# pnnl/ERT-Conditional-Diffusion-Model

Measured on AMD Instinct MI355X. Metric: denoising-steps/sec (64×64, batch 64) at 1/2/4/8 GPUs; conv HBM GB/s vs roofline, higher is better.
Workload: dtype f32

## Files before the change

ert-conditional-diffusion-model_amd/csrc/unet.h:

```cpp
#pragma once
#include <cstdlib>

#include "ertd_common.h"

#ifdef ERTD_DIAG
#define ERTD_KNOB(name, dflt) (::ertd::unet::diag_knob("ERTD_" name, (dflt)))
#else
#define ERTD_KNOB(name, dflt) (dflt)
#endif

namespace ertd {
namespace unet {

#ifdef ERTD_DIAG
inline int diag_knob(const char* name, int dflt) {
  const char* e = getenv(name);
  return e ? atoi(e) : dflt;
}
#endif

constexpr int NTHR = 256;
constexpr double GN_EPS = 1e-5;

enum Act { ACT_NONE = 0, ACT_GN_SILU = 1, ACT_GN = 2 };
enum Mode { MODE_S1 = 0, MODE_S2 = 1, MODE_UP = 2,
            MODE_UPP = 3 };

struct GnPartArgs {
  const float2* pa; int npa; int Ca;
  const float2* pb; int npb; int Cb;
  int HW, groups;
  const float* gamma; const float* beta;
  float2* out;
  float2* mr;
};

struct GnFold {
  GnPartArgs g;
  unsigned* cnt;
  int target;
  int B;
};

struct ConvArgs {
  const float* srcA;
  const float* srcB;
  int Ca, Cb;
  const float2* gn;
  const float* wpk;
  const float* bias;
  const float* ebias;
  int eb_stride;
  const float* res;
  float* out;
  int Cin, Cout;
  int Hs, Ws;
  int Ho, Wo;
  void* bimg;
  int bimg_ready;
  const float* wpk_wino;
  float* ksplit_buf;
  const float* wpk_wino4;
  float2* gnp;
  int split;
  GnFold fold;
  unsigned* zero_words;
  int zero_n;
  GnPartArgs gnc;
};

hipError_t launch_gn_finalize(const GnPartArgs& a, int B, hipStream_t s);
hipError_t launch_gn_partials(const float* x, int C, int HW, int np, float2* out, int B, hipStream_t s);
struct WinoRoute {
  enum Kernel { NONE,
                F2,
                F4,
                F4S,
                F4S_UP
  } kernel = NONE;
  int ksplit = 1;
  size_t kbuf_floats = 0;
  int items = 0, grid = 0;
  int gn_parts = 0;
  bool fold_ok = false;
  int fold_target = 0;
  int pack_kind = ERTD_PACK_DIRECT;
};
WinoRoute wino_route(int mode, int act, int Cin, int Ca, int Cout, int Wo, int B, bool have_f2_pack,
                     bool have_f4_pack, int cus);
bool wino_gnc_ok(const WinoRoute& r, int Cin, int Wo, const GnPartArgs& g);
int conv_gn_parts(int ks, int mode, int act, const ConvArgs& a, const WinoRoute& r);
int conv_bf16_gn_parts(int ks, int mode, int act, const ConvArgs& a, int B);

__device__ __forceinline__ float row16_sum(float v) {
  v += __int_as_float(__builtin_amdgcn_update_dpp(0, __float_as_int(v), 0xB1, 0xF, 0xF, false));
  v += __int_as_float(__builtin_amdgcn_update_dpp(0, __float_as_int(v), 0x4E, 0xF, 0xF, false));
  v += __int_as_float(__builtin_amdgcn_update_dpp(0, __float_as_int(v), 0x141, 0xF, 0xF, false));
  v += __int_as_float(__builtin_amdgcn_update_dpp(0, __float_as_int(v), 0x140, 0xF, 0xF, false));
  return v;
}

__device__ __forceinline__ void st_f2_wt(float2* p, float2 v) {
  unsigned* u = reinterpret_cast<unsigned*>(p);
  __hip_atomic_store(u, __float_as_uint(v.x), __ATOMIC_RELAXED, __HIP_MEMORY_SCOPE_AGENT);
  __hip_atomic_store(u + 1, __float_as_uint(v.y), __ATOMIC_RELAXED, __HIP_MEMORY_SCOPE_AGENT);
}
__device__ __forceinline__ float2 ld_f2_wt(const float2* p) {
  const unsigned* u = reinterpret_cast<const unsigned*>(p);
  return make_float2(__uint_as_float(__hip_atomic_load(u, __ATOMIC_RELAXED, __HIP_MEMORY_SCOPE_AGENT)),
                     __uint_as_float(__hip_atomic_load(u + 1, __ATOMIC_RELAXED, __HIP_MEMORY_SCOPE_AGENT)));
}
#ifndef FOLD_BATCH
#define FOLD_BATCH 4
#endif
constexpr int GN_LPG = 16;
struct GnGroupGeom {
  int c0, itemsA, items;
  const float2* pa;
  const float2* pb;
};
__device__ __forceinline__ GnGroupGeom gn_group_geom(const GnPartArgs& g, int b, int gi, bool live) {
  const int cpg = (g.Ca + g.Cb) / g.groups;
  GnGroupGeom q{};
  if (!live) return q;
  q.c0 = gi * cpg;
  const int nA = q.c0 < g.Ca ? (g.Ca - q.c0 < cpg ? g.Ca - q.c0 : cpg) : 0;
  q.itemsA = nA * g.npa;
  q.items = q.itemsA + (cpg - nA) * (g.Cb > 0 ? g.npb : 0);
  q.pa = g.pa + ((size_t)b * g.Ca + q.c0) * g.npa;
  q.pb = g.Cb > 0 ? g.pb + ((size_t)b * g.Cb + (q.c0 + nA - g.Ca)) * g.npb : nullptr;
  return q;
}
template <int CTRL>
__device__ __forceinline__ double dpp_f64(double v) {
  const unsigned long long u = __double_as_longlong(v);
  const int lo = __builtin_amdgcn_update_dpp(0, (int)(unsigned)u, CTRL, 0xF, 0xF, false);
  const int hi = __builtin_amdgcn_update_dpp(0, (int)(unsigned)(u >> 32), CTRL, 0xF, 0xF, false);
  return __longlong_as_double((long long)(((unsigned long long)(unsigned)hi << 32) | (unsigned)lo));
}
__device__ __forceinline__ double gn_lpg_sum(double v) {
  static_assert(GN_LPG == 16, "one DPP row per group");
  v += dpp_f64<0xB1>(v);
  v += dpp_f64<0x4E>(v);
  v += dpp_f64<0x141>(v);
  v += dpp_f64<0x140>(v);
  return v;
}
__device__ __forceinline__ double gn_part_q(float2 v, double n, double inv_n, double mean) {
  const double d = (double)v.x * inv_n - mean;
  return (double)v.y + n * (d * d);
}
__device__ __forceinline__ float2 gn_mean_rstd(double mean, double Q, double N) {
  double var = Q / N;
  var = var > 0.0 ? var : 0.0;
  return make_float2((float)mean, (float)(1.0 / sqrt(var + GN_EPS)));
}
template <bool WT>
__device__ __forceinline__ float2 gn_ld_part(const GnGroupGeom& q, int k) {
  return k < q.itemsA ? (WT ? ld_f2_wt(q.pa + k) : q.pa[k]) : q.pb[k - q.itemsA];
}
template <bool WT>
__device__ __forceinline__ void gn_group_finalize(const GnPartArgs& g, int b, int lane, int part,
                                                  int nparts, float2* orow = nullptr) {
  const int G = g.groups, C = g.Ca + g.Cb, cpg = C / G;
  const int gper = (G + nparts - 1) / nparts, gfirst = part * gper;
  const int gcnt = G - gfirst < gper ? G - gfirst : gper;
  if (gcnt <= 0) return;
  constexpr int LPG = GN_LPG;
  const double na = (double)(g.HW / g.npa), nb = g.Cb > 0 ? (double)(g.HW / g.npb) : 1.0;
  const double ina = 1.0 / na, inb = 1.0 / nb;
  const double N = (double)cpg * (double)g.HW;
  for (int gbase = 0; gbase < gcnt; gbase += 64 / LPG) {
    const int gl = gbase + lane / LPG, sub = lane % LPG;
    const bool live = gl < gcnt;
    const int gi = gfirst + gl;
    const GnGroupGeom q = gn_group_geom(g, b, gi, live);
    double S = 0.0;
    for (int k0 = sub; k0 < q.items; k0 += FOLD_BATCH * LPG) {
      float2 v[FOLD_BATCH];
#pragma unroll
      for (int j = 0; j < FOLD_BATCH; ++j) {
        const int k = k0 + j * LPG;
        v[j] = k < q.items ? gn_ld_part<WT>(q, k) : make_float2(0.f, 0.f);
      }
#pragma unroll
      for (int j = 0; j < FOLD_BATCH; ++j)
        if (k0 + j * LPG < q.items) S += (double)v[j].x;
    }
    S = gn_lpg_sum(S);
    const double mean = S / N;
    double Q = 0.0;
    for (int k0 = sub; k0 < q.items; k0 += FOLD_BATCH * LPG) {
      float2 v[FOLD_BATCH];
#pragma unroll
      for (int j = 0; j < FOLD_BATCH; ++j) {
        const int k = k0 + j * LPG;
        v[j] = k < q.items ? gn_ld_part<WT>(q, k) : make_float2(0.f, 0.f);
      }
#pragma unroll
      for (int j = 0; j < FOLD_BATCH; ++j) {
        const int k = k0 + j * LPG;
        if (k < q.items) Q += k < q.itemsA ? gn_part_q(v[j], na, ina, mean) : gn_part_q(v[j], nb, inb, mean);
      }
    }
    Q = gn_lpg_sum(Q);
    if (!live) continue;
    const float2 mr = gn_mean_rstd(mean, Q, N);
    if (g.mr && sub == 0) g.mr[(size_t)b * G + gi] = mr;
    for (int cl = sub; cl < cpg; cl += LPG) {
      const int c = q.c0 + cl;
      const float scale = mr.y * g.gamma[c];
      const float shift = -scale * mr.x + g.beta[c];
      if (orow) orow[c] = make_float2(scale, shift);
      else g.out[(size_t)b * C + c] = make_float2(scale, shift);
    }
  }
}
template <int JM, int KM>
__device__ __forceinline__ void gn_group_finalize_regs(const GnPartArgs& g, const int (&smp)[JM],
                                                       const int (&jg)[JM], const int (&row)[JM],
                                                       const bool (&jl)[JM], int lane, float2* tab) {
  constexpr int LPG = GN_LPG;
  const int G = g.groups, C = g.Ca + g.Cb, cpg = C / G, sub = lane % LPG;
  const double na = (double)(g.HW / g.npa), nb = g.Cb > 0 ? (double)(g.HW / g.npb) : 1.0;
  const double ina = 1.0 / na, inb = 1.0 / nb;
  const double N = (double)cpg * (double)g.HW;
  GnGroupGeom q[JM];
  float2 v[JM][KM];
  float ga[JM], be[JM];
  bool live[JM];
#pragma unroll
  for (int j = 0; j < JM; ++j) {
    const int gi = jg[j] * 4 + lane / LPG;
    live[j] = jl[j] && gi < G;
    q[j] = gn_group_geom(g, smp[j], gi, live[j]);
#pragma unroll
    for (int k = 0; k < KM; ++k) {
      const int kk = sub + LPG * k;
      v[j][k] = kk < q[j].items ? gn_ld_part<false>(q[j], kk) : make_float2(0.f, 0.f);
    }
    const bool ch = live[j] && sub < cpg;
    ga[j] = ch ? g.gamma[q[j].c0 + sub] : 0.f;
    be[j] = ch ? g.beta[q[j].c0 + sub] : 0.f;
  }
#pragma unroll
  for (int j = 0; j < JM; ++j) {
    double S = 0.0;
#pragma unroll
    for (int k = 0; k < KM; ++k)
      if (sub + LPG * k < q[j].items) S += (double)v[j][k].x;
    S = gn_lpg_sum(S);
    const double mean = S / N;
    double Q = 0.0;
#pragma unroll
    for (int k = 0; k < KM; ++k) {
      const int kk = sub + LPG * k;
      if (kk < q[j].items)
        Q += kk < q[j].itemsA ? gn_part_q(v[j][k], na, ina, mean) : gn_part_q(v[j][k], nb, inb, mean);
    }
    Q = gn_lpg_sum(Q);
    if (live[j] && sub < cpg) {
      const float2 mr = gn_mean_rstd(mean, Q, N);
      const float scale = mr.y * ga[j];
      const float shift = -scale * mr.x + be[j];
      tab[(size_t)row[j] * C + q[j].c0 + sub] = make_float2(scale, shift);
    }
  }
}
__device__ __forceinline__ void gn_fold_item_done(const GnFold& f, int b, int* lds_cnt, int nw, int lane) {
  asm volatile("s_waitcnt vmcnt(0)" ::: "memory");
  int old = 0;
  if (lane == 0) old = atomicAdd(lds_cnt, 1);
  old = __builtin_amdgcn_readfirstlane(old);
  if (old == nw - 1 && lane == 0) {
    *lds_cnt = 0;
    (void)__hip_atomic_fetch_add(f.cnt + b, 1u, __ATOMIC_RELAXED, __HIP_MEMORY_SCOPE_AGENT);
  }
}

struct ConvDispatch {
  int kernel = -1;
  WinoRoute route;
  int items = 0, grid = 0;
};
ConvDispatch conv_dispatch(int ks, int mode, int act, const ConvArgs& a, int B);
hipError_t launch_conv(int ks, int mode, int act, const ConvArgs& a, int B, hipStream_t s);
int conv_bf16_dispatch(int ks, int mode, int act, const ConvArgs& a);
hipError_t launch_conv_bf16(int ks, int mode, int act, const ConvArgs& a, int B, hipStream_t s);
size_t conv_packed_floats_bf16(int cin, int cout, int ks, bool split = false);
hipError_t launch_act_bf16(const ConvArgs& a, int act, bool up, int B, hipStream_t s);
size_t conv_bf16_image_bytes(int cin, int B, int H, int W, bool split = false);
hipError_t launch_pack_conv_bf16(const float* w, int cin, int cout, int ks, float* dst,
                                 hipStream_t s, bool split = false);
enum PackKind { PK_F32 = 0, PK_BF16 = 1, PK_SPLIT = 2 };
hipError_t launch_conv_out(int act, const ConvArgs& a, int B, int pk, hipStream_t s);
bool conv_in_ok(const ConvArgs& a, int ks, int mode, int act);
hipError_t launch_conv_in(const ConvArgs& a, int B, int pk, hipStream_t s);
hipError_t launch_conv_wino(int act, const ConvArgs& a, hipStream_t s, const WinoRoute& r);
hipError_t launch_conv_wino4(int act, const ConvArgs& a, hipStream_t s, const WinoRoute& r);
hipError_t launch_conv_wino4s(int act, const ConvArgs& a, hipStream_t s, const WinoRoute& r);
size_t conv_packed_floats_wino(int cin, int cout);
size_t conv_packed_floats_wino4(int cin, int cout);
hipError_t launch_pack_conv_wino4(const float* w, int cin, int cout, float* dst, hipStream_t s,
                                  bool flipT = false);
int wino4s_xs();
hipError_t launch_add_inplace(float* out, const float* part, size_t n, hipStream_t s);
hipError_t launch_pack_conv_wino(const float* w, int cin, int cout, float* dst, hipStream_t s,
                                 bool flipT = false);
bool conv1x1_ok(const ConvArgs& a, int act, int B);
hipError_t launch_conv1x1(const ConvArgs& a, int B, hipStream_t s);
bool skip_gemm_ok(const ConvArgs& a, int ks, int mode, int act, int B);
struct SkipGemmGeom {
  bool split = false;
  int mt = 0, nt = 0;
  int items = 0, grid = 0;
};
hipError_t launch_skip_gemm(const ConvArgs& a, int B, hipStream_t s, SkipGemmGeom* geom = nullptr);
size_t wgrad_wino_ws_floats(int Cin, int Cout, int B, int H, int ks, int mode);
hipError_t launch_wgrad_wino(const float* dy, const float* x, int Ca, const float* x2, int Cb, int B,
                             int H, int Cout, int mode, const float* gn, int act, float* dw,
                             int accumulate, float* ws, hipStream_t s, float* db = nullptr,
                             float* db2 = nullptr);
bool wgrad_wino_bias_ok(int Cin, int Cout, int B, int H, int ks, int mode);
size_t conv_packed_floats(int cin, int cout, int ks);
hipError_t launch_pack_conv(const float* w, int cin, int cout, int ks, float* dst, hipStream_t s,
                            bool flipT = false);
hipError_t launch_pack_batch(const ertd_pack_desc* d, int n, int blocks, hipStream_t s);
size_t conv_packed_floats_up(int cin, int cout);
hipError_t launch_pack_conv_up(const float* w, int cin, int cout, float* dst, hipStream_t s);

struct GnArgs {
  const float* srcA; const float* srcB; int Ca, Cb;
  int HW, groups;
  const float* gamma; const float* beta;
  float2* out;
  float2* mr;
};
hipError_t launch_gn_stats(const GnArgs& a, int B, hipStream_t s);
bool gn_act_bf16_fits(int C, int groups, int HW);
hipError_t launch_gn_act_bf16(const GnArgs& a, bool silu, void* bimg, int B, hipStream_t s,
                              bool split = false);

enum DenseIn { DIN_PLAIN = 0, DIN_SILU = 1, DIN_SINUSOID = 2 };
struct DenseArgs {
  const float* x; int x_stride;
  const int64_t* t;
  const int* t_dev;
  const float* freq;
  const float* wt;
  const float* bias;
  const float* add; int add_stride;
  int add_bcast;
  float* y; int y_stride;
  int K, O;
};
hipError_t launch_dense(int din, const DenseArgs& a, int B, hipStream_t s);
hipError_t launch_transpose(const float* w, int O, int K, float* dst, int dst_ld, hipStream_t s);

hipError_t launch_attention(const float* qkv, int C, int N, float* o, float* scratch, int B,
                            hipStream_t s);

struct UpdateArgs {
  float* x;
  const float* eps;
  const float* c1; const float* c2; const float* sigma;
  const float* noise;
  int num_steps;
  const int* t_dev;
  uint64_t seed; uint32_t member_offset;
  int P;
};
hipError_t launch_unet_update(const UpdateArgs& a, int B, hipStream_t s);
hipError_t launch_zero_insert(const float* x, int B, int C, int Ho, float* out, hipStream_t s);
hipError_t launch_sum_pool2(const float* x, int B, int C, int H, float* out, int accumulate,
                            hipStream_t s);
hipError_t launch_set_word(int* w, int v, hipStream_t s);
hipError_t launch_dec_word(int* w, hipStream_t s);
struct SolverUpdateArgs {
  float* x;
  const float* eps;
  float* d_prev;
  const float* coef;
  const float* noise;
  const int* words;
  int K;
  float clip;
  uint64_t seed; uint32_t member_offset;
  int P;
};
hipError_t launch_unet_solver_update(const SolverUpdateArgs& a, int B, hipStream_t s);
hipError_t launch_solver_set_words(int* words, const int* timesteps, int k, hipStream_t s);
hipError_t launch_solver_next_words(int* words, const int* timesteps, int K, hipStream_t s);

}
}
```

ert-conditional-diffusion-model_amd/csrc/unet_capi.hip:

```cpp
#include <cstdlib>
#include <cstring>
#include <algorithm>
#include <new>
#include <map>
#include <string>
#include <vector>

#include "unet.h"
#include "unet_pack.h"

using namespace ertd;
using namespace ertd::unet;

namespace {

struct Param {
  std::string name;
  std::vector<int> shape;
  size_t numel() const {
    size_t n = 1;
    for (int d : shape) n *= (size_t)d;
    return n;
  }
};
// ... 627 lines not shown
  w.chk(launch_encoder_strips(pk + w.L->enc, e.enc0_b, e.enc2_b, cond, cstride, w.B, Lc,
                              ERTD_PREC_FP32, f.partial, w.s));
  w.chk(launch_hoist_prep(e, pk + w.L->enc, f.partial, S, L2, w.B, f.Uscr, f.cond_emb, w.s));
  w.dense(DIN_PLAIN, f.cond_emb, H, nullptr, nullptr, nullptr, "cond_proj", H, temb(w.c), nullptr,
          0, f.cproj, temb(w.c));
  return w.err == hipSuccess ? ERTD_OK : (int)w.err;
}

void embed(Walk& w, const Fixed& f, const int64_t* t) {
  const int tb = temb(w.c);
  w.dense(DIN_SINUSOID, nullptr, 0, t, f.tdev, w.pk + w.L->off.at("freq"), "time_embed.0", w.c->ch,
          tb, nullptr, 0, f.e1, tb);
  w.dense(DIN_SILU, f.e1, tb, nullptr, nullptr, nullptr, "time_embed.2", tb, tb, f.cproj, tb, f.emb,
          tb);
  w.dense(DIN_SILU, f.emb, tb, nullptr, nullptr, nullptr, "", tb, w.L->ebtotal, nullptr, 0, f.ebias,
          w.L->ebtotal, w.pk + w.L->wall, w.pk + w.L->ball);
}

Layout layout_with_freq(const ertd_unet_config* c) {
  Layout L = layout_full(c);
  L.off["freq"] = L.total;
  L.total += a64((size_t)c->ch / 2);
  return L;
}

size_t ws_bytes_for(const ertd_unet_config* c, const Layout& L, int B, int Lc) {
  Walk w{c, &L, nullptr, nullptr, 0, B, nullptr, true};
  fixed(w, Lc);
  w.unet(nullptr, nullptr, nullptr);
  return w.used;
}

inline int rcode(hipError_t e) { return e == hipSuccess ? ERTD_OK : (int)e; }

struct SampleCall {
  const ertd_unet_config* c;
  const float* packed; const float* cond; long long cond_stride; int L; int B;
  int num_steps; int t_first; int n_run;
  const float* c1; const float* c2; const float* sigma; const float* noise;
  uint64_t seed; uint32_t member_offset; float* x; void* ws; size_t ws_bytes;

  int check() const {
    if (!cfg_ok(c) || !packed || !cond || !c1 || !c2 || !sigma || !x || !ws || B < 1 || L < 1 ||
        num_steps < 1 || t_first < 0 || t_first >= num_steps || n_run < 0 || n_run > t_first + 1)
      return ERTD_EINVAL;
    const Layout Lo = layout_with_freq(c);
    if (ws_bytes_for(c, Lo, B, L) > ws_bytes) return ERTD_ENOSPC;
    return ERTD_OK;
  }
  int head(hipStream_t s) const {
    const Layout Lo = layout_with_freq(c);
    Walk w{c, &Lo, packed, (char*)ws, 0, B, s, false};
    w.cap = ws_bytes;
    const Fixed f = fixed(w, L);
    const int r = prologue(w, f, cond, cond_stride, L);
    if (r != ERTD_OK) return r;
    w.chk(launch_set_word(f.tdev, t_first, s));
    return rcode(w.err);
  }
  int step(hipStream_t s, hipStream_t s2 = nullptr, hipEvent_t evf = nullptr,
           hipEvent_t evj = nullptr, hipEvent_t eve = nullptr, bool skip_side = true) const {
    const Layout Lo = layout_with_freq(c);
    Walk w{c, &Lo, packed, (char*)ws, 0, B, s, false};
    w.cap = ws_bytes;
    w.s2 = skip_side ? s2 : nullptr;
    w.evf = evf;
    w.evj = evj;
    const Fixed f = fixed(w, L);
    const int P = c->image * c->image;
    if (s2 && eve) {
      w.chk(hipEventRecord(evf, s));
      w.chk(hipStreamWaitEvent(s2, evf, 0));
      w.s = s2;
      embed(w, f, nullptr);
      w.s = s;
      w.chk(hipEventRecord(eve, s2));
      w.emb_join = eve;
    } else {
      embed(w, f, nullptr);
    }
    w.unet(x, f.ebias, f.eps);
    UpdateArgs u{x, f.eps, c1, c2, sigma, noise, num_steps, f.tdev, seed, member_offset, P};
    w.chk(launch_unet_update(u, B, s));
    w.chk(launch_dec_word(f.tdev, s));
    return rcode(w.err);
  }
};

struct SolverCall {
  const ertd_unet_config* c;
  const float* packed; const float* cond; long long cond_stride; int L; int B;
  int K; int k_first; int n_run;
  const int32_t* timesteps; const float* coef; float clip; const float* noise;
  uint64_t seed; uint32_t member_offset; float* x; float* d_prev; void* ws; size_t ws_bytes;

  int check(hipStream_t s) const {
    if (!cfg_ok(c) || !packed || !cond || !timesteps || !coef || !x || !d_prev || !ws || B < 1 ||
        L < 1 || K < 1 || k_first < 0 || n_run < 0 || n_run > K - k_first || !(clip >= 0.f))
      return ERTD_EINVAL;
    const Layout Lo = layout_with_freq(c);
    if (ws_bytes_for(c, Lo, B, L) > ws_bytes) return ERTD_ENOSPC;
    return solver_tables_ok(timesteps, coef, K, true, noise != nullptr, s);
  }
  int head(hipStream_t s) const {
    const Layout Lo = layout_with_freq(c);
    Walk w{c, &Lo, packed, (char*)ws, 0, B, s, false};
    w.cap = ws_bytes;
    const Fixed f = fixed(w, L);
    const int r = prologue(w, f, cond, cond_stride, L);
    if (r != ERTD_OK) return r;
    w.chk(launch_solver_set_words(f.tdev, timesteps, k_first, s));
    return rcode(w.err);
  }
  int step(hipStream_t s, hipStream_t s2 = nullptr, hipEvent_t evf = nullptr,
           hipEvent_t evj = nullptr, hipEvent_t eve = nullptr, bool skip_side = true) const {
    const Layout Lo = layout_with_freq(c);
    Walk w{c, &Lo, packed, (char*)ws, 0, B, s, false};
    w.cap = ws_bytes;
    w.s2 = skip_side ? s2 : nullptr;
    w.evf = evf;
    w.evj = evj;
    const Fixed f = fixed(w, L);
    const int P = c->image * c->image;
    if (s2 && eve) {
      w.chk(hipEventRecord(evf, s));
      w.chk(hipStreamWaitEvent(s2, evf, 0));
      w.s = s2;
      embed(w, f, nullptr);
      w.s = s;
      w.chk(hipEventRecord(eve, s2));
      w.emb_join = eve;
    } else {
      embed(w, f, nullptr);
    }
    w.unet(x, f.ebias, f.eps);
    SolverUpdateArgs u{x, f.eps, d_prev, coef, noise, f.tdev, K, clip, seed, member_offset, P};
    w.chk(launch_unet_solver_update(u, B, s));
    w.chk(launch_solver_next_words(f.tdev, timesteps, K, s));
    return rcode(w.err);
  }
};

}

struct ertd_unet_plan {
  ertd_unet_config cfg{};
  SampleCall call{};
  SolverCall scall{};
  int n_run = 0;
  hipStream_t stream = nullptr;
  hipStream_t side = nullptr;
  hipEvent_t evf = nullptr, evj = nullptr, eve = nullptr;
  hipGraph_t g_head = nullptr, g_step = nullptr;
  hipGraphExec_t x_head = nullptr, x_step = nullptr;
  hipGraph_t g_multi = nullptr;
  hipGraphExec_t x_multi = nullptr;
  int multi = 0;
  bool skip_side = false;
};

template <class Call>
static int capture_unet_plan(ertd_unet_plan* p, const Call& call, ertd_unet_plan** plan) {
  int r = ERTD_OK;
  hipError_t e = hipStreamCreateWithFlags(&p->stream, hipStreamNonBlocking);
  const int sv = ERTD_KNOB("UNET_SIDE", -1);
  const bool side = sv >= 0 ? sv != 0 : bf_prec(p->cfg.precision);
  const bool side_emb = ERTD_KNOB("UNET_SIDE_EMB", 0) != 0;
  p->skip_side = side;
  if (e == hipSuccess && (side || side_emb)) {
    e = hipStreamCreateWithFlags(&p->side, hipStreamNonBlocking);
    if (e == hipSuccess) e = hipEventCreateWithFlags(&p->evf, hipEventDisableTiming);
    if (e == hipSuccess) e = hipEventCreateWithFlags(&p->evj, hipEventDisableTiming);
    if (e == hipSuccess) e = hipEventCreateWithFlags(&p->eve, hipEventDisableTiming);
  }
  const int multi = ERTD_KNOB("UNET_MULTI", 8);
  const int ngraphs = multi > 1 && p->n_run >= 2 * multi ? 3 : 2;
  for (int k = 0; e == hipSuccess && k < ngraphs; ++k) {
    e = hipStreamBeginCapture(p->stream, hipStreamCaptureModeThreadLocal);
    if (e != hipSuccess) break;
    if (k == 0) {
      r = call.head(p->stream);
    } else {
      for (int i = 0; r == ERTD_OK && i < (k == 1 ? 1 : multi); ++i)
        r = call.step(p->stream, p->side, p->evf, p->evj, p->eve, p->skip_side);
    }
    hipGraph_t g = nullptr;
    e = hipStreamEndCapture(p->stream, &g);
    (k == 0 ? p->g_head : k == 1 ? p->g_step : p->g_multi) = g;
    if (r != ERTD_OK) break;
    if (e == hipSuccess)
      e = hipGraphInstantiate(k == 0 ? &p->x_head : k == 1 ? &p->x_step : &p->x_multi, g, nullptr, nullptr, 0);
    if (k == 2 && e == hipSuccess) p->multi = multi;
  }
  if (r != ERTD_OK || e != hipSuccess) {
    ertd_unet_plan_destroy(p);
    return r != ERTD_OK ? r : (int)e;
  }
  *plan = p;
  return ERTD_OK;
}

extern "C" {

}

namespace {
struct Conv2dWs {
  size_t pack_floats = 0;
  size_t kbuf_floats = 0;
  size_t bimg_bytes = 0;
  size_t total() const { return a64(pack_floats) * sizeof(float) + a64(kbuf_floats) * sizeof(float) +
                                (bimg_bytes + 255) / 256 * 256; }
};

bool conv2d_geom_ok(int cin, int cout, int ks, int precision, int B, int H, int mode) {
  return cin >= 1 && cout >= 1 && (ks == 1 || ks == 3) && B >= 1 && H >= 1 && mode >= MODE_S1 &&
         mode <= MODE_UP && !(ks == 1 && mode != MODE_S1) &&
         (precision == ERTD_PREC_FP32 || bf_prec(precision));
}

int conv2d_out_size(int H, int mode) { return mode == MODE_S2 ? H / 2 : (mode == MODE_UP ? 2 * H : H); }

WinoRoute conv2d_route(int cin, int ca, int cout, int ks, int mode, int act, int precision, int B, int H) {
  if (bf_prec(precision) || ks != 3) return WinoRoute{};
  return wino_route(mode, act, cin, ca, cout, conv2d_out_size(H, mode), B, conv_packed_floats_wino(cin, cout) > 0,
                    conv_packed_floats_wino4(cin, cout) > 0, device_cu_count());
}

Conv2dWs conv2d_ws(int cin, int ca, int cout, int ks, int precision, int B, int H, int mode, int act) {
  Conv2dWs w;
  const bool bf = bf_prec(precision), split = precision == ERTD_PREC_BF16X3;
  size_t f = bf ? conv_packed_floats_bf16(cin, cout, ks, split) : conv_packed_floats(cin, cout, ks);
  if (!bf && ks == 3 && conv_packed_floats_up(cin, cout) > f)
    f = conv_packed_floats_up(cin, cout);
  if (!bf && ks == 3)
    f = a64(f) + std::max(conv_packed_floats_wino(cin, cout), conv_packed_floats_wino4(cin, cout));
  w.pack_floats = f;
  const int Ho = conv2d_out_size(H, mode);
  w.kbuf_floats = conv2d_route(cin, ca, cout, ks, mode, act, precision, B, H).kbuf_floats;
  if (bf && ks == 3 && cout > 1 &&
      ((mode == MODE_S1 && act != ACT_NONE) || (mode == MODE_UP && act == ACT_NONE)))
    w.bimg_bytes = conv_bf16_image_bytes(cin, B, Ho, Ho, split);
  return w;
}

}

extern "C" {

size_t ertd_conv2d_workspace_bytes(int cin, int cout, int ks, int precision, int B, int H, int mode) {
  if (!conv2d_geom_ok(cin, cout, ks, precision, B, H, mode)) return 0;
  const Conv2dWs a = conv2d_ws(cin, cin, cout, ks, precision, B, H, mode, ACT_GN_SILU);
  const Conv2dWs b = conv2d_ws(cin, cin, cout, ks, precision, B, H, mode, ACT_NONE);
  return std::max(a.total(), b.total());
}

namespace {
ConvArgs conv2d_args(const float* x, int Ca, const float* x2, int Cb, int H, const float* bias, int Cout,
                     int ks, int mode, const float* gn, const float* ebias, int eb_stride, const float* res,
                     float* out, int precision, float* pk, const Conv2dWs& need, const WinoRoute& route) {
  const int Cin = Ca + Cb;
  ConvArgs a{};
  a.srcA = x; a.srcB = x2; a.Ca = Ca; a.Cb = Cb;
  a.gn = (const float2*)gn;
  a.wpk = pk; a.bias = bias; a.ebias = ebias; a.eb_stride = eb_stride; a.res = res; a.out = out;
  a.Cin = Cin; a.Cout = Cout; a.Hs = H; a.Ws = H;
  a.Ho = a.Wo = conv2d_out_size(H, mode);
  if (route.kernel != WinoRoute::NONE) {
    float* pw = pk + a64(std::max(conv_packed_floats(Cin, Cout, ks), conv_packed_floats_up(Cin, Cout)));
    if (route.pack_kind == ERTD_PACK_WINO4) a.wpk_wino4 = pw; else a.wpk_wino = pw;
    a.ksplit_buf = need.kbuf_floats ? pk + a64(need.pack_floats) : nullptr;
  }
  a.bimg = need.bimg_bytes ? (void*)(pk + a64(need.pack_floats) + a64(need.kbuf_floats)) : nullptr;
  a.split = precision == ERTD_PREC_BF16X3 ? 1 : 0;
  return a;
}

int conv2d_impl(const float* x, int Ca, const float* x2, int Cb, int B, int H, const float* w,
                const float* bias, int Cout, int ks, int mode, const float* gn, int act,
                const float* ebias, int eb_stride, const float* res, float* out, int precision,
                void* ws, size_t ws_bytes, void* stream, bool pack, float* gnp = nullptr, int gn_np = 0) {
  const int Cin = Ca + Cb;
  if (!x || (pack && !w) || !bias || !out || !ws || B < 1 || Ca < 1 || Cb < 0 || (Cb > 0 && !x2) ||
      !conv2d_geom_ok(Cin, Cout, ks, precision, B, H, mode) || act < ACT_NONE || act > ACT_GN ||
      (act != ACT_NONE && !gn))
    return ERTD_EINVAL;
  const Conv2dWs need = conv2d_ws(Cin, Ca, Cout, ks, precision, B, H, mode, act);
  if (need.total() > ws_bytes) return ERTD_ENOSPC;
  hipStream_t s = (hipStream_t)stream;
  float* pk = (float*)ws;
  const bool bf = bf_prec(precision), split = precision == ERTD_PREC_BF16X3;
  const WinoRoute route = conv2d_route(Cin, Ca, Cout, ks, mode, act, precision, B, H);
  const bool wino = route.kernel != WinoRoute::NONE, wino4 = route.pack_kind == ERTD_PACK_WINO4;
  if (gnp && (bf || gn_np < 1)) return ERTD_EINVAL;
  hipError_t e = hipSuccess;
  if (!wino && pack)
    e = bf ? launch_pack_conv_bf16(w, Cin, Cout, ks, pk, s, split)
        : (ks == 3 && mode == MODE_UP) ? launch_pack_conv_up(w, Cin, Cout, pk, s)
                                       : launch_pack_conv(w, Cin, Cout, ks, pk, s);
  if (e != hipSuccess) return (int)e;
  ConvArgs a = conv2d_args(x, Ca, x2, Cb, H, bias, Cout, ks, mode, gn, ebias, eb_stride, res, out, precision,
                           pk, need, route);
  if (wino && pack &&
      (e = wino4 ? launch_pack_conv_wino4(w, Cin, Cout, const_cast<float*>(a.wpk_wino4), s)
                 : launch_pack_conv_wino(w, Cin, Cout, const_cast<float*>(a.wpk_wino), s)) != hipSuccess)
    return (int)e;
  if (gnp) {
    if (conv_gn_parts(ks, mode, act, a, route) != gn_np) return ERTD_EINVAL;
    a.gnp = (float2*)gnp;
  }
  e = bf ? launch_conv_bf16(ks, mode, act, a, B, s) : launch_conv(ks, mode, act, a, B, s);
  return e == hipErrorInvalidValue ? ERTD_EINVAL : rcode(e);
}
}

int ertd_conv2d(const float* x, int Ca, const float* x2, int Cb, int B, int H, const float* w,
                const float* bias, int Cout, int ks, int mode, const float* gn, int act,
                const float* ebias, int eb_stride, const float* res, float* out, int precision,
                void* ws, size_t ws_bytes, void* stream) {
  return conv2d_impl(x, Ca, x2, Cb, B, H, w, bias, Cout, ks, mode, gn, act, ebias, eb_stride, res, out,
                     precision, ws, ws_bytes, stream, true);
}

int ertd_conv2d_run(const float* x, int Ca, const float* x2, int Cb, int B, int H, const float* bias,
                    int Cout, int ks, int mode, const float* gn, int act, const float* ebias,
                    int eb_stride, const float* res, float* out, int precision, void* ws,
                    size_t ws_bytes, void* stream) {
  return conv2d_impl(x, Ca, x2, Cb, B, H, nullptr, bias, Cout, ks, mode, gn, act, ebias, eb_stride, res,
                     out, precision, ws, ws_bytes, stream, false);
}

int ertd_conv2d_gn_parts(int Ca, int Cb, int Cout, int ks, int mode, int act, int precision, int B, int H) {
  const int Cin = Ca + Cb;
  if (Ca < 1 || Cb < 0 || !conv2d_geom_ok(Cin, Cout, ks, precision, B, H, mode) || bf_prec(precision) ||
      act < ACT_NONE || act > ACT_GN)
    return 0;
  ConvArgs q{};
  q.Ca = Ca; q.Cb = Cb; q.Cin = Cin; q.Cout = Cout;
  q.Hs = q.Ws = H;
  q.Ho = q.Wo = conv2d_out_size(H, mode);
  return conv_gn_parts(ks, mode, act, q, conv2d_route(Cin, Ca, Cout, ks, mode, act, precision, B, H));
}

int ertd_conv2d_route_info(int Ca, int Cb, int Cout, int ks, int mode, int act, int precision, int has_ebias,
                           int B, int H, ertd_route_info* out) {
  const int Cin = Ca + Cb;
  if (!out || Ca < 1 || Cb < 0 || !conv2d_geom_ok(Cin, Cout, ks, precision, B, H, mode) || act < ACT_NONE ||
      act > ACT_GN)
    return ERTD_EINVAL;
  float* const base = reinterpret_cast<float*>((uintptr_t)4096);
  const Conv2dWs need = conv2d_ws(Cin, Ca, Cout, ks, precision, B, H, mode, act);
  const WinoRoute route = conv2d_route(Cin, Ca, Cout, ks, mode, act, precision, B, H);
  const ConvArgs a = conv2d_args(base, Ca, Cb > 0 ? base : nullptr, Cb, H, base, Cout, ks, mode,
                                 act != ACT_NONE ? base : nullptr, (has_ebias & 1) ? base : nullptr, Cout,
                                 (has_ebias & 2) ? base : nullptr, base, precision, base, need, route);
  *out = ertd_route_info{};
  out->ksplit = 1;
  if (bf_prec(precision)) {
    out->kernel = conv_bf16_dispatch(ks, mode, act, a);
  } else {
    const ConvDispatch d = conv_dispatch(ks, mode, act, a, B);
    if (d.kernel < 0) return ERTD_EINVAL;
    out->kernel = d.kernel;
    out->items = d.items;
    out->grid = d.grid;
    if (d.route.kernel != WinoRoute::NONE) out->ksplit = d.route.ksplit;
  }
  out->gn_parts = ertd_conv2d_gn_parts(Ca, Cb, Cout, ks, mode, act, precision, B, H);
  return ERTD_OK;
}

int ertd_conv2d_gn(const float* x, int Ca, const float* x2, int Cb, int B, int H, const float* w,
                   const float* bias, int Cout, int ks, int mode, const float* gn, int act,
                   const float* ebias, int eb_stride, const float* res, float* out, int precision,
                   void* ws, size_t ws_bytes, float* gn_parts, int gn_np, void* stream) {
  if (!gn_parts) return ERTD_EINVAL;
  return conv2d_impl(x, Ca, x2, Cb, B, H, w, bias, Cout, ks, mode, gn, act, ebias, eb_stride, res, out,
                     precision, ws, ws_bytes, stream, true, gn_parts, gn_np);
}

int ertd_conv2d_run_gn(const float* x, int Ca, const float* x2, int Cb, int B, int H, const float* bias,
                       int Cout, int ks, int mode, const float* gn, int act, const float* ebias,
                       int eb_stride, const float* res, float* out, int precision, void* ws,
                       size_t ws_bytes, float* gn_parts, int gn_np, void* stream) {
  if (!gn_parts) return ERTD_EINVAL;
  return conv2d_impl(x, Ca, x2, Cb, B, H, nullptr, bias, Cout, ks, mode, gn, act, ebias, eb_stride, res,
                     out, precision, ws, ws_bytes, stream, false, gn_parts, gn_np);
}

size_t ertd_conv_input_grad_ws_bytes(int Cin, int Cout, int B, int H, int ks, int mode) {
  if (Cin < 1 || Cout < 1 || B < 1 || H < 1 || (ks != 1 && ks != 3) || mode < MODE_S1 ||
      mode > MODE_UP || (ks == 1 && mode != MODE_S1))
    return 0;
  size_t n = a64(std::max(conv_packed_floats(Cout, Cin, ks),
                          std::max(conv_packed_floats_wino(Cout, Cin), conv_packed_floats_wino4(Cout, Cin))));
  if (mode == MODE_S2) n += a64((size_t)B * Cout * H * H);
  if (mode == MODE_UP) n += a64((size_t)B * Cin * 4 * H * H);
  const int Hg = mode == MODE_UP ? 2 * H : H;
  if (ks == 3) n += a64((size_t)B * Cin * Hg * Hg);
  return n * sizeof(float);
}

}

namespace {
WinoRoute input_grad_route(int Cin, int Cout, int B, int H, int ks, int mode) {
  return conv2d_route(Cout, Cout, Cin, ks, MODE_S1, ACT_NONE, ERTD_PREC_FP32, B, mode == MODE_UP ? 2 * H : H);
}

int input_grad_impl(const float* dy, int B, int H, const float* w, int Cout, int Cin, int ks, int mode,
                    float* dx, int accumulate, void* ws, size_t ws_bytes, void* stream, bool pack) {
  const size_t need = ertd_conv_input_grad_ws_bytes(Cin, Cout, B, H, ks, mode);
  if (!dy || (pack && !w) || !dx || !ws || need == 0) return ERTD_EINVAL;
  if (need > ws_bytes) return ERTD_ENOSPC;
  hipStream_t s = (hipStream_t)stream;
  float* pk = (float*)ws;
  float* scratch = pk + a64(std::max(conv_packed_floats(Cout, Cin, ks),
                                     std::max(conv_packed_floats_wino(Cout, Cin),
                                              conv_packed_floats_wino4(Cout, Cin))));
  const int Hg = mode == MODE_UP ? 2 * H : H;
  const float* src = dy;
  if (mode == MODE_S2) {
    hipError_t e = launch_zero_insert(dy, B, Cout, H / 2, scratch, s);
    if (e != hipSuccess) return (int)e;
    src = scratch;
  }
  ConvArgs a{};
  a.srcA = src; a.Ca = Cout; a.Cb = 0;
  a.Cin = Cout; a.Cout = Cin;
  a.Hs = a.Ws = a.Ho = a.Wo = Hg;
  const WinoRoute route = input_grad_route(Cin, Cout, B, H, ks, mode);
  const bool wino4 = route.pack_kind == ERTD_PACK_WINO4, wino = route.kernel != WinoRoute::NONE;
  hipError_t e = hipSuccess;
  if (pack)
    e = wino4 ? launch_pack_conv_wino4(w, Cout, Cin, pk, s, true)
        : wino ? launch_pack_conv_wino(w, Cout, Cin, pk, s, true)
               : launch_pack_conv(w, Cout, Cin, ks, pk, s, true);
  if (e != hipSuccess) return (int)e;
  if (wino4) a.wpk_wino4 = pk; else if (wino) a.wpk_wino = pk; else a.wpk = pk;
  if (route.ksplit == 2) {
    const size_t sc = mode == MODE_S2 ? a64((size_t)B * Cout * H * H)
                      : (mode == MODE_UP ? a64((size_t)B * Cin * 4 * H * H) : 0);
    a.ksplit_buf = scratch + sc;
  }
  a.bias = nullptr;
  float* out = mode == MODE_UP ? scratch : dx;
  a.res = (mode != MODE_UP && accumulate) ? dx : nullptr;
  a.out = out;
  if ((e = launch_conv(ks, MODE_S1, ACT_NONE, a, B, s)) != hipSuccess) return rcode(e);
  if (mode == MODE_UP) return rcode(launch_sum_pool2(scratch, B, Cin, H, dx, accumulate, s));
  return ERTD_OK;
}

void fill_desc(ertd_pack_desc* d, const float* w, float* dst, int cin, int cout, int ks, int kind, int flip) {
  *d = ertd_pack_desc{};
  d->w = w; d->dst = dst; d->cin = cin; d->cout = cout; d->ks = ks; d->kind = kind; d->flip = flip;
  switch (kind) {
    case ERTD_PACK_DIRECT:
      d->total = (long long)conv_packed_floats(cin, cout, ks);
      d->nchunk = (cin + conv_ck(ks) - 1) / conv_ck(ks);
      break;
    case ERTD_PACK_UP:
      d->total = (long long)conv_packed_floats_up(cin, cout);
      d->nchunk = (cin + conv_ck(2) - 1) / conv_ck(2);
      break;
    case ERTD_PACK_WINO:
      d->total = (long long)conv_packed_floats_wino(cin, cout);
      d->nchunk = cin / WINO_KC;
      break;
    default:
      d->total = (long long)conv_packed_floats_wino4(cin, cout);
      d->nchunk = cin / WINO4_KC;
      break;
  }
}
}

extern "C" {

int ertd_conv_input_grad(const float* dy, int B, int H, const float* w, int Cout, int Cin, int ks,
                         int mode, float* dx, int accumulate, void* ws, size_t ws_bytes,
                         void* stream) {
  return input_grad_impl(dy, B, H, w, Cout, Cin, ks, mode, dx, accumulate, ws, ws_bytes, stream, true);
}

int ertd_conv_input_grad_run(const float* dy, int B, int H, int Cout, int Cin, int ks, int mode,
                             float* dx, int accumulate, void* ws, size_t ws_bytes, void* stream) {
  return input_grad_impl(dy, B, H, nullptr, Cout, Cin, ks, mode, dx, accumulate, ws, ws_bytes, stream,
                         false);
}

int ertd_conv_input_grad_pack_desc(int Cin, int Cout, int B, int H, int ks, int mode, const float* w,
                                   void* ws, ertd_pack_desc* out) {
  if (!w || !ws || !out || ertd_conv_input_grad_ws_bytes(Cin, Cout, B, H, ks, mode) == 0)
    return ERTD_EINVAL;
  fill_desc(out, w, (float*)ws, Cout, Cin, ks, input_grad_route(Cin, Cout, B, H, ks, mode).pack_kind, 1);
  return ERTD_OK;
}

int ertd_conv2d_pack_desc(int Cin, int Ca, int Cout, int ks, int mode, int precision, int B, int H,
                          const float* w, void* ws, ertd_pack_desc* out) {
  if (!w || !ws || !out || precision != ERTD_PREC_FP32 || Ca < 1 || Ca > Cin ||
      !conv2d_geom_ok(Cin, Cout, ks, precision, B, H, mode))
    return ERTD_EINVAL;
  float* pk = (float*)ws;
  const WinoRoute route = conv2d_route(Cin, Ca, Cout, ks, mode, ACT_NONE, precision, B, H);
  if (route.kernel != WinoRoute::NONE)
    pk += a64(std::max(conv_packed_floats(Cin, Cout, ks), conv_packed_floats_up(Cin, Cout)));
  fill_desc(out, w, pk, Cin, Cout, ks, route.pack_kind, 0);
  return ERTD_OK;
}

int ertd_conv_pack_batch_prepare(ertd_pack_desc* d, int n) {
  if (!d || n < 1) return ERTD_EINVAL;
  long long blocks = 0;
  for (int k = 0; k < n; ++k) {
    if (!d[k].w || !d[k].dst || d[k].total < 1 || d[k].kind < ERTD_PACK_DIRECT || d[k].kind > ERTD_PACK_WINO4)
      return ERTD_EINVAL;
    d[k].block0 = (int)blocks;
    blocks += (pack_work_items(d[k].kind, d[k].total) + 255) / 256;
    if (blocks > (1LL << 30)) return ERTD_EINVAL;
  }
  return (int)blocks;
}

int ertd_conv_pack_batch(const ertd_pack_desc* descs, int n, int blocks, void* stream) {
  if (!descs || n < 1 || blocks < 1) return ERTD_EINVAL;
  return rcode(launch_pack_batch(descs, n, blocks, (hipStream_t)stream));
}

int ertd_group_norm_stats(const float* x, int Ca, const float* x2, int Cb, int B, int HW,
                          int groups, const float* gamma, const float* beta, float* out,
                          void* stream) {
  const int C = Ca + Cb;
  if (!x || !gamma || !beta || !out || B < 1 || Ca < 1 || Cb < 0 || (Cb > 0 && !x2) ||
      groups < 1 || C % groups || HW < 4 || HW % 4)
    return ERTD_EINVAL;
  GnArgs g{x, x2, Ca, Cb, HW, groups, gamma, beta, (float2*)out};
  return rcode(launch_gn_stats(g, B, (hipStream_t)stream));
}

int ertd_group_norm_partials(const float* x, int C, int B, int HW, int np, float* parts, void* stream) {
  if (!x || !parts || C < 1 || B < 1 || np < 1 || HW != np * 256) return ERTD_EINVAL;
  return rcode(launch_gn_partials(x, C, HW, np, (float2*)parts, B, (hipStream_t)stream));
}

int ertd_group_norm_finalize(const float* pa, int npa, int Ca, const float* pb, int npb, int Cb, int B,
                             int HW, int groups, const float* gamma, const float* beta, float* out,
                             float* mr, void* stream) {
  const int C = Ca + Cb;
  if (!pa || !gamma || !beta || !out || B < 1 || Ca < 1 || Cb < 0 || npa < 1 || HW < 1 || groups < 1 ||
      C % groups || HW % npa || (Cb > 0 && (!pb || npb < 1 || HW % npb)))
    return ERTD_EINVAL;
  GnPartArgs g{(const float2*)pa, npa, Ca, (const float2*)pb, npb, Cb, HW, groups, gamma, beta,
               (float2*)out, (float2*)mr};
  return rcode(launch_gn_finalize(g, B, (hipStream_t)stream));
}

int ertd_group_norm_act_bf16(const float* x, int Ca, const float* x2, int Cb, int B, int H,
                             int groups, const float* gamma, const float* beta, float* out,
                             void* img, int silu, void* stream) {
  const int C = Ca + Cb;
  if (!x || !gamma || !beta || !out || !img || B < 1 || Ca < 1 || Cb < 0 || (Cb > 0 && !x2) ||
      groups < 1 || H < 1 || !gn_act_bf16_fits(C, groups, H * H))
    return ERTD_EINVAL;
  GnArgs g{x, x2, Ca, Cb, H * H, groups, gamma, beta, (float2*)out};
  return rcode(launch_gn_act_bf16(g, silu != 0, img, B, (hipStream_t)stream));
}

int ertd_act_bf16(const float* x, int Ca, const float* x2, int Cb, int B, int H, const float* ss,
                  int act, int up, void* img, void* stream) {
  if (!x || !img || B < 1 || Ca < 1 || Cb < 0 || (Cb > 0 && !x2) || H < 1 ||
      act < ACT_NONE || act > ACT_GN || (act != ACT_NONE && !ss) || (up && act != ACT_NONE))
    return ERTD_EINVAL;
  ConvArgs a{};
  a.srcA = x;
  a.srcB = x2;
  a.Ca = Ca;
  a.Cb = Cb;
  a.Cin = Ca + Cb;
  a.gn = (const float2*)ss;
  a.Hs = a.Ws = H;
  a.Ho = a.Wo = up ? 2 * H : H;
  a.bimg = img;
  return rcode(launch_act_bf16(a, act, up != 0, B, (hipStream_t)stream));
}

int ertd_unet_update(float* x, const float* eps, const float* c1, const float* c2,
                     const float* sigma, const float* noise, int num_steps, const int* t_dev,
                     uint64_t seed, uint32_t member_offset, int B, int P, void* stream) {
  if (!x || !eps || !c1 || !c2 || !sigma || !t_dev || B < 1 || P < 1 || (noise && num_steps < 1))
    return ERTD_EINVAL;
  UpdateArgs u{x, eps, c1, c2, sigma, noise, num_steps, t_dev, seed, member_offset, P};
  return rcode(launch_unet_update(u, B, (hipStream_t)stream));
}

int ertd_attention(const float* qkv, int B, int C, int N, float* out, void* stream) {
  if (!qkv || !out || B < 1 || N != 256 || C < 2 || C % 256) return ERTD_EINVAL;
  return rcode(launch_attention(qkv, C, N, out, nullptr, B, (hipStream_t)stream));
}

int ertd_unet_n_params(const ertd_unet_config* c) {
  if (!cfg_ok(c)) return ERTD_EINVAL;
  return (int)enumerate(c).size();
}

int ertd_unet_param_info(const ertd_unet_config* c, int idx, char* name, int name_len,
                         int64_t* shape, int* ndim) {
  if (!cfg_ok(c) || !name || name_len < 2 || !shape || !ndim) return ERTD_EINVAL;
  const std::vector<Param> P = enumerate(c);
  if (idx < 0 || idx >= (int)P.size()) return ERTD_EINVAL;
  const Param& p = P[idx];
  strncpy(name, p.name.c_str(), (size_t)name_len - 1);
  name[name_len - 1] = 0;
  *ndim = (int)p.shape.size();
  for (int i = 0; i < *ndim; ++i) shape[i] = p.shape[i];
  return ERTD_OK;
}

size_t ertd_unet_packed_floats(const ertd_unet_config* c) {
  if (!cfg_ok(c)) return 0;
  return layout_with_freq(c).total;
}

size_t ertd_unet_workspace_bytes(const ertd_unet_config* c, int B, int L) {
  if (!cfg_ok(c) || B < 1 || L < 1) return 0;
  const Layout Lo = layout_with_freq(c);
  return ws_bytes_for(c, Lo, B, L);
}

int ertd_unet_pack(const ertd_unet_config* c, const float* const* params, const float* freq,
                   float* packed, void* stream) {
  if (!cfg_ok(c) || !params || !freq || !packed) return ERTD_EINVAL;
  const Layout L = layout_with_freq(c);
  for (size_t i = 0; i < L.params.size(); ++i)
    if (!params[i]) return ERTD_EINVAL;
  hipStream_t s = (hipStream_t)stream;
  hipError_t e = hipMemsetAsync(packed + L.dummy, 0, DUMMY_FLOATS * sizeof(float), s);
  if (e != hipSuccess) return (int)e;
  const ertd_weights ew = enc_weights(L, packed, params);
  if ((e = launch_pack(ew, packed + L.enc, s)) != hipSuccess) return (int)e;
  const int tb = temb(c);
  for (size_t i = 0; i < L.params.size(); ++i) {
    const Param& p = L.params[i];
    const float* src = params[i];
    if (p.name.rfind("condition_encoder.", 0) == 0) {
      static const char* map[6] = {"enc.0.weight", "enc.0.bias", "enc.2.weight",
                                   "enc.2.bias", "enc.6.weight", "enc.6.bias"};
      e = hipMemcpyAsync(packed + L.off.at(map[i]), src, p.numel() * sizeof(float),
                         hipMemcpyDeviceToDevice, s);
    } else if (ends_with(p.name, ".emb.weight")) {
      const int col = L.eboff.at(p.name.substr(0, p.name.size() - 11));
      e = launch_transpose(src, p.shape[0], p.shape[1], packed + L.wall + col, L.ebtotal, s);
    } else if (ends_with(p.name, ".emb.bias")) {
      const int col = L.eboff.at(p.name.substr(0, p.name.size() - 9));
      e = hipMemcpyAsync(packed + L.ball + col, src, p.numel() * sizeof(float),
                         hipMemcpyDeviceToDevice, s);
    } else if (p.shape.size() == 4) {
      e = bf_prec(c->precision)
              ? launch_pack_conv_bf16(src, p.shape[1], p.shape[0], p.shape[2],
                                      packed + L.off.at(p.name), s, c->precision == ERTD_PREC_BF16X3)
              : (ends_with(p.name, ".upsample.weight")
                     ? launch_pack_conv_up(src, p.shape[1], p.shape[0], packed + L.off.at(p.name), s)
                     : launch_pack_conv(src, p.shape[1], p.shape[0], p.shape[2],
                                        packed + L.off.at(p.name), s));
      const auto itw = L.offw.find(p.name);
      if (e == hipSuccess && itw != L.offw.end())
        e = launch_pack_conv_wino(src, p.shape[1], p.shape[0], packed + itw->second, s);
      const auto itw4 = L.offw4.find(p.name);
      if (e == hipSuccess && itw4 != L.offw4.end())
        e = launch_pack_conv_wino4(src, p.shape[1], p.shape[0], packed + itw4->second, s);
    } else if (p.shape.size() == 2) {
      e = launch_transpose(src, p.shape[0], p.shape[1], packed + L.off.at(p.name), p.shape[0], s);
    } else {
      e = hipMemcpyAsync(packed + L.off.at(p.name), src, p.numel() * sizeof(float),
                         hipMemcpyDeviceToDevice, s);
    }
    if (e != hipSuccess) return (int)e;
  }
  (void)tb;
  e = hipMemcpyAsync(packed + L.off.at("freq"), freq, (size_t)c->ch / 2 * sizeof(float),
                     hipMemcpyDeviceToDevice, s);
  return rcode(e);
}

int ertd_unet_forward(const ertd_unet_config* c, const float* packed, const float* x,
                      const int64_t* t, const float* cond, long long cond_stride, int L, int B,
                      float* out, float* cond_emb_out, void* ws, size_t ws_bytes, void* stream) {
  if (!cfg_ok(c) || !packed || !x || !t || !cond || !out || !ws || B < 1 || L < 1)
    return ERTD_EINVAL;
  const Layout Lo = layout_with_freq(c);
  if (ws_bytes_for(c, Lo, B, L) > ws_bytes) return ERTD_ENOSPC;
  Walk w{c, &Lo, packed, (char*)ws, 0, B, (hipStream_t)stream, false};
  w.cap = ws_bytes;
  const Fixed f = fixed(w, L);
  int r = prologue(w, f, cond, cond_stride, L);
  if (r != ERTD_OK) return r;
  embed(w, f, t);
  w.unet(x, f.ebias, out);
  if (cond_emb_out && w.err == hipSuccess)
    w.chk(hipMemcpyAsync(cond_emb_out, f.cond_emb, (size_t)B * H * sizeof(float),
                         hipMemcpyDeviceToDevice, w.s));
  return rcode(w.err);
}

int ertd_unet_sample(const ertd_unet_config* c, const float* packed, const float* cond,
                     long long cond_stride, int L, int B, int num_steps, int t_first, int n_run,
                     const float* c1, const float* c2, const float* sigma, const float* noise,
                     uint64_t seed, uint32_t member_offset, float* x_inout, void* ws,
                     size_t ws_bytes, void* stream) {
  SampleCall sc{c, packed, cond, cond_stride, L, B, num_steps, t_first, n_run, c1, c2, sigma,
                noise, seed, member_offset, x_inout, ws, ws_bytes};
  int r = sc.check();
  if (r != ERTD_OK) return r;
  hipStream_t s = (hipStream_t)stream;
  if ((r = sc.head(s)) != ERTD_OK) return r;
  for (int i = 0; i < n_run; ++i)
    if ((r = sc.step(s)) != ERTD_OK) return r;
  return ERTD_OK;
}

int ertd_unet_sample_plan_create(const ertd_unet_config* c, const float* packed, const float* cond,
                                 long long cond_stride, int L, int B, int num_steps, int t_first,
                                 int n_run, const float* c1, const float* c2, const float* sigma,
                                 const float* noise, uint64_t seed, uint32_t member_offset,
                                 float* x_inout, void* ws, size_t ws_bytes,
                                 ertd_unet_plan** plan) {
  if (!plan) return ERTD_EINVAL;
  *plan = nullptr;
  ertd_unet_plan* p = new (std::nothrow) ertd_unet_plan();
  if (!p) return ERTD_EINVAL;
  p->call = SampleCall{c, packed, cond, cond_stride, L, B, num_steps, t_first, n_run, c1, c2,
                       sigma, noise, seed, member_offset, x_inout, ws, ws_bytes};
  p->cfg = *c;
  p->call.c = &p->cfg;
  p->n_run = n_run;
  int r = p->call.check();
  if (r != ERTD_OK) {
    delete p;
    return r;
  }
  return capture_unet_plan(p, p->call, plan);
}

int ertd_unet_sample_solver(const ertd_unet_config* c, const float* packed, const float* cond,
                            long long cond_stride, int L, int B, int K, int k_first, int n_run,
                            const int32_t* timesteps, const float* coef, float clip,
                            const float* noise, uint64_t seed, uint32_t member_offset,
                            float* x_inout, float* d_prev_inout, void* ws, size_t ws_bytes,
                            void* stream) {
  SolverCall sc{c, packed, cond, cond_stride, L, B, K, k_first, n_run, timesteps, coef, clip,
                noise, seed, member_offset, x_inout, d_prev_inout, ws, ws_bytes};
  hipStream_t s = (hipStream_t)stream;
  int r = sc.check(s);
  if (r != ERTD_OK) return r;
  if ((r = sc.head(s)) != ERTD_OK) return r;
  for (int i = 0; i < n_run; ++i)
    if ((r = sc.step(s)) != ERTD_OK) return r;
  return ERTD_OK;
}

int ertd_unet_sample_solver_plan_create(const ertd_unet_config* c, const float* packed,
                                        const float* cond, long long cond_stride, int L, int B,
                                        int K, int k_first, int n_run, const int32_t* timesteps,
                                        const float* coef, float clip, const float* noise,
                                        uint64_t seed, uint32_t member_offset, float* x_inout,
                                        float* d_prev_inout, void* ws, size_t ws_bytes,
                                        void* stream, ertd_unet_plan** plan) {
  if (!plan) return ERTD_EINVAL;
  *plan = nullptr;
  if (!c) return ERTD_EINVAL;
  ertd_unet_plan* p = new (std::nothrow) ertd_unet_plan();
  if (!p) return ERTD_EINVAL;
  p->scall = SolverCall{c, packed, cond, cond_stride, L, B, K, k_first, n_run, timesteps, coef,
                        clip, noise, seed, member_offset, x_inout, d_prev_inout, ws, ws_bytes};
  p->cfg = *c;
  p->scall.c = &p->cfg;
  p->n_run = n_run;
  const int r = p->scall.check((hipStream_t)stream);
  if (r != ERTD_OK) {
    delete p;
    return r;
  }
  return capture_unet_plan(p, p->scall, plan);
}

int ertd_unet_plan_launch_steps(ertd_unet_plan* p, int n_steps, void* stream) {
  if (!p || !p->x_head || !p->x_step || n_steps < 0 || n_steps > p->n_run) return ERTD_EINVAL;
  hipStream_t s = (hipStream_t)stream;
  hipError_t e = hipGraphLaunch(p->x_head, s);
  int i = 0;
  if (p->x_multi)
    for (; e == hipSuccess && i + p->multi <= n_steps; i += p->multi) e = hipGraphLaunch(p->x_multi, s);
  for (; e == hipSuccess && i < n_steps; ++i) e = hipGraphLaunch(p->x_step, s);
  return rcode(e);
}

int ertd_unet_plan_launch(ertd_unet_plan* p, void* stream) {
  if (!p) return ERTD_EINVAL;
  return ertd_unet_plan_launch_steps(p, p->n_run, stream);
}

int ertd_unet_plan_destroy(ertd_unet_plan* p) {
  if (!p) return ERTD_OK;
  if (p->x_head) (void)hipGraphExecDestroy(p->x_head);
  if (p->x_step) (void)hipGraphExecDestroy(p->x_step);
  if (p->x_multi) (void)hipGraphExecDestroy(p->x_multi);
  if (p->g_multi) (void)hipGraphDestroy(p->g_multi);
  if (p->g_head) (void)hipGraphDestroy(p->g_head);
  if (p->g_step) (void)hipGraphDestroy(p->g_step);
  if (p->stream) (void)hipStreamDestroy(p->stream);
  if (p->side) (void)hipStreamDestroy(p->side);
  if (p->evf) (void)hipEventDestroy(p->evf);
  if (p->evj) (void)hipEventDestroy(p->evj);
  if (p->eve) (void)hipEventDestroy(p->eve);
  delete p;
  return ERTD_OK;
}

}
```

ert-conditional-diffusion-model_amd/csrc/unet_conv_wino.hip:

```cpp
#include <cstdlib>

#include "unet.h"
#include "unet_pack.h"

namespace ertd {
namespace unet {

namespace {

constexpr int NMW = 8;
constexpr int NPW = 4;
constexpr int WT = 64 * (NMW + NPW);
constexpr int WKC = 8;
constexpr int WSP = WKC / 4;
constexpr int U_FL = 16 * 2 * WSP * 128;
constexpr int V_FL = 16 * WSP * 2 * 128;
constexpr int NUB = 3;
constexpr int NRS = 3;
constexpr size_t WLDS = (size_t)(NUB * U_FL + 2 * V_FL) * sizeof(float);
constexpr int XIF = WKC * 64;
#ifndef WINO_PPRIO
#define WINO_PPRIO 2
#endif
#ifndef WINO_PD
// ... 241 lines not shown
      for (int x = 0; x < PD; ++x) ld(x);
#pragma unroll
      for (int x = 0; x < 16; ++x) {
        if (x + PD < 16) ld(x + PD);
        const int r = x % (PD + 1);
#pragma unroll
        for (int st = 0; st < 2; ++st) {
          if constexpr (DBG & 8) {
            acc[x][0][0] += ra[r][st] * rb0[r][st];
            acc[x][1][0] += ra[r][st] * rb1[r][st];
          } else {
            acc[x][0] = __builtin_amdgcn_mfma_f32_16x16x4f32(ra[r][st], rb0[r][st], acc[x][0], 0, 0, 0);
            acc[x][1] = __builtin_amdgcn_mfma_f32_16x16x4f32(ra[r][st], rb1[r][st], acc[x][1], 0, 0, 0);
          }
        }
        if (x + PD < 16) __builtin_amdgcn_sched_group_barrier(0x100, 3, 0);
        __builtin_amdgcn_sched_group_barrier(0x008, 4, 0);
      }
#pragma unroll
      for (int x = 0; x < 16; ++x) asm volatile("" : "+v"(acc[x][0]), "+v"(acc[x][1]));
      if (dma) asm volatile("s_waitcnt vmcnt(4)" ::: "memory");
      else asm volatile("s_waitcnt vmcnt(0)" ::: "memory");
      __syncthreads();
    }

    if constexpr (DBG & 64) {
      if (il == nloc - 1)
        for (int x = 0; x < 16; ++x) a.out[(size_t)bid * 64 + lane] += acc[x][0][0] + acc[x][1][1];
      continue;
    }
    const int itg = bid + il * G;
    const Item itm = item_of(itg / ksp, ncog, NTBLK);
    const bool part2 = (itg % ksp) != 0;
    const bool has_eb = a.ebias && !part2, has_res = a.res && !part2, has_bias = a.bias && !part2;
    const unsigned smp = (unsigned)(a.Cout * HW * 4);
    const __amdgpu_buffer_rsrc_t ro = __builtin_amdgcn_make_buffer_rsrc(
        (part2 ? a.ksplit_buf : a.out) + (size_t)itm.b * a.Cout * HW, (short)0, smp, 0x00020000);
    const __amdgpu_buffer_rsrc_t rr = __builtin_amdgcn_make_buffer_rsrc(
        has_res ? const_cast<float*>(a.res) + (size_t)itm.b * a.Cout * HW : nullptr, (short)0, smp, 0x00020000);
    int ln;
    asm volatile("v_mbcnt_lo_u32_b32 %0, -1, 0\n\tv_mbcnt_hi_u32_b32 %0, -1, %0" : "=v"(ln));
    const int co0 = itm.cog * 64 + cb * 16 + 4 * (ln >> 4);
    int vo[2];
#pragma unroll
    for (int j = 0; j < 2; ++j) {
      const int tg = itm.tblk * 64 + (2 * tbp + j) * 16 + (ln & 15);
      const int ty = tg / TPR, tx = tg - ty * TPR;
      vo[j] = (co0 * HW + 2 * ty * WO + 2 * tx) * 4;
    }
    float bias[4], eb[4];
#pragma unroll
    for (int i = 0; i < 4; ++i) {
      bias[i] = has_bias ? a.bias[co0 + i] : 0.f;
      eb[i] = has_eb ? a.ebias[(size_t)itm.b * a.eb_stride + co0 + i] : 0.f;
    }
    auto out_tile = [&](const int j, f32x2 (&y)[4][2]) {
#pragma unroll
      for (int i = 0; i < 4; ++i) {
        float Pm[4][2];
#pragma unroll
        for (int r = 0; r < 4; ++r) {
          const float m0 = acc[4 * r + 0][j][i], m1 = acc[4 * r + 1][j][i];
          const float m2 = acc[4 * r + 2][j][i], m3 = acc[4 * r + 3][j][i];
          Pm[r][0] = (m0 + m1) + m2;
          Pm[r][1] = (m1 - m2) - m3;
        }
        y[i][0] = f32x2{(Pm[0][0] + Pm[1][0]) + Pm[2][0], (Pm[0][1] + Pm[1][1]) + Pm[2][1]} + bias[i];
        y[i][1] = f32x2{(Pm[1][0] - Pm[2][0]) - Pm[3][0], (Pm[1][1] - Pm[2][1]) - Pm[3][1]} + bias[i];
        if (has_eb) {
          y[i][0] = y[i][0] + eb[i];
          y[i][1] = y[i][1] + eb[i];
        }
      }
    };
    auto store_tile = [&](const int j, const f32x2 (&y)[4][2]) {
#pragma unroll
      for (int i = 0; i < 4; ++i)
#pragma unroll
        for (int r = 0; r < 2; ++r)
          __builtin_amdgcn_raw_buffer_store_b64(__builtin_bit_cast(__attribute__((ext_vector_type(2))) unsigned, y[i][r]),
                                                ro, vo[j] + r * WO * 4, i * HW * 4, 0);
    };
    f32x2 y[2][4][2];
    out_tile(0, y[0]);
    out_tile(1, y[1]);
    __builtin_amdgcn_sched_barrier(0);
    if (has_res) {
      f32x2 rv[2][4][2];
#pragma unroll
      for (int j = 0; j < 2; ++j)
#pragma unroll
        for (int i = 0; i < 4; ++i)
#pragma unroll
          for (int r = 0; r < 2; ++r)
            rv[j][i][r] = __builtin_bit_cast(
                f32x2, __builtin_amdgcn_raw_buffer_load_b64(rr, vo[j] + r * WO * 4, i * HW * 4, 0));
#pragma unroll
      for (int j = 0; j < 2; ++j)
#pragma unroll
        for (int i = 0; i < 4; ++i)
#pragma unroll
          for (int r = 0; r < 2; ++r) y[j][i][r] = y[j][i][r] + rv[j][i][r];
    }
    store_tile(0, y[0]);
    store_tile(1, y[1]);
    if (a.gnp && ksp == 1) {
      float2 pr[4];
#pragma unroll
      for (int i = 0; i < 4; ++i) {
        float sm = ((y[0][i][0][0] + y[0][i][0][1]) + (y[0][i][1][0] + y[0][i][1][1])) +
                   ((y[1][i][0][0] + y[1][i][0][1]) + (y[1][i][1][0] + y[1][i][1][1]));
        sm = row16_sum(sm);
        const float mu = sm * (1.0f / 128.0f);
        float q = 0.f;
#pragma unroll
        for (int j = 0; j < 2; ++j)
#pragma unroll
          for (int r = 0; r < 2; ++r)
#pragma unroll
            for (int x = 0; x < 2; ++x) {
              const float d = y[j][i][r][x] - mu;
              q = __builtin_fmaf(d, d, q);
            }
        pr[i] = make_float2(sm, row16_sum(q));
      }
      if ((ln & 15) == 0) {
        constexpr int np = TPR * TPR / 32;
        const int part = 2 * itm.tblk + tbp;
#pragma unroll
        for (int i = 0; i < 4; ++i) a.gnp[((size_t)itm.b * a.Cout + co0 + i) * np + part] = pr[i];
      }
    }
  }
}

#ifdef ERTD_DIAG
int wino_dbg() {
  static int v = [] {
    return ERTD_KNOB("WINO_DBG", 0);
  }();
  return v;
}
#endif

__global__ void add_inplace_kernel(float* __restrict__ out, const float* __restrict__ part, size_t n4) {
  const size_t i = (size_t)blockIdx.x * 256 + threadIdx.x;
  if (i >= n4) return;
  float4 o = reinterpret_cast<float4*>(out)[i];
  const float4 p = reinterpret_cast<const float4*>(part)[i];
  o.x = o.x + p.x; o.y = o.y + p.y; o.z = o.z + p.z; o.w = o.w + p.w;
  reinterpret_cast<float4*>(out)[i] = o;
}

int ksplit_items() {
  static int v = [] {
    return ERTD_KNOB("WINO_KSPLIT", 1);
  }();
  return v;
}

template <int WO, int ACT, int DBG>
hipError_t launch_wod(const ConvArgs& a, hipStream_t s, const WinoRoute& r) {
  static std::atomic<unsigned long long> attr{0};
  set_max_lds_once((const void*)conv_wino_kernel<WO, ACT, DBG>, (int)WLDS, attr);
  conv_wino_kernel<WO, ACT, DBG><<<r.grid, WT, WLDS, s>>>(a, r.items, r.ksplit);
  hipError_t e = hipGetLastError();
  if (e != hipSuccess || r.ksplit == 1) return e;
  return launch_add_inplace(a.out, a.ksplit_buf, r.kbuf_floats, s);
}

template <int WO, int ACT>
hipError_t launch_wo(const ConvArgs& a, hipStream_t s, const WinoRoute& r) {
#ifdef ERTD_DIAG
  if constexpr (WO == 64 && ACT == ACT_GN_SILU) {
    switch (wino_dbg()) {
      case 1: return launch_wod<WO, ACT, 1>(a, s, r);
      case 2: return launch_wod<WO, ACT, 2>(a, s, r);
      case 4: return launch_wod<WO, ACT, 4>(a, s, r);
      case 8: return launch_wod<WO, ACT, 8>(a, s, r);
      case 7: return launch_wod<WO, ACT, 7>(a, s, r);
      case 16: return launch_wod<WO, ACT, 16>(a, s, r);
      case 32: return launch_wod<WO, ACT, 32>(a, s, r);
      case 64: return launch_wod<WO, ACT, 64>(a, s, r);
      case 23: return launch_wod<WO, ACT, 23>(a, s, r);
      case 55: return launch_wod<WO, ACT, 55>(a, s, r);
      default: break;
    }
  }
#endif
  return launch_wod<WO, ACT, 0>(a, s, r);
}

template <int ACT>
hipError_t launch_act(const ConvArgs& a, hipStream_t s, const WinoRoute& r) {
  switch (a.Wo) {
    case 16: return launch_wo<16, ACT>(a, s, r);
    case 32: return launch_wo<32, ACT>(a, s, r);
    case 64: return launch_wo<64, ACT>(a, s, r);
    case 128: return launch_wo<128, ACT>(a, s, r);
    default: return hipErrorInvalidValue;
  }
}

__global__ void pack_wino_kernel(const float* __restrict__ w, int cin, int cout, int nchunk,
                                 size_t items, float* __restrict__ dst, bool flipT) {
  const size_t j = (size_t)blockIdx.x * blockDim.x + threadIdx.x;
  if (j >= items) return;
  pack_wino_tile(w, cin, cout, nchunk, j, flipT, dst);
}

}

hipError_t launch_add_inplace(float* out, const float* part, size_t n, hipStream_t s) {
  add_inplace_kernel<<<(unsigned)((n / 4 + 255) / 256), 256, 0, s>>>(out, part, n / 4);
  return hipGetLastError();
}

static int wino4_w16_env() {
  static int v = [] {
    return ERTD_KNOB("WINO4_W16", 0);
  }();
  return v;
}

static int wino4s_env() {
  static int v = [] {
    return ERTD_KNOB("WINO4S", 4);
  }();
  return v;
}

int wino4s_xs() {
  static const int v = [] {
    return ERTD_KNOB("WINO4S_XS", 2);
  }();
  return v;
}

static int wino4s_ks_env() {
  static const int v = [] {
    return ERTD_KNOB("WINO4S_KSPLIT", 1);
  }();
  return v;
}

static int wino4s_up_env() {
  static const int v = [] {
    return ERTD_KNOB("WINO4S_UP", 1);
  }();
  return v;
}

static bool chunks_split(int nchunk) { return nchunk % 2 == 0 && nchunk >= 4; }

WinoRoute wino_route(int mode, int act, int Cin, int Ca, int Cout, int Wo, int B, bool have_f2_pack,
                     bool have_f4_pack, int cus) {
  WinoRoute r;
  r.pack_kind = mode == MODE_UP ? ERTD_PACK_UP : ERTD_PACK_DIRECT;
  const bool up = mode == MODE_UP && act == ACT_NONE;
  if ((mode != MODE_S1 && !up) || wino_env() == 0 || Cout % 64 ||
      (Wo != 16 && Wo != 32 && Wo != 64 && Wo != 128))
    return r;
  const bool f2_geom = Cin % WKC == 0 && Ca % WKC == 0;
  const bool f4 = have_f4_pack && wino_env() == 1;
  const int ncog = Cout / 64, t4 = (Wo / 4) * (Wo / 4);
  int base = 0;
  bool split = false;

  const int s_items = t4 / 16 * B * ncog, e = wino4s_env();
  const bool s_split = wino4s_ks_env() && wino4s_xs() == 2 && Wo == 16 && Cin % 8 == 0 &&
                       chunks_split(Cin / 8) && s_items < cus && 2 * s_items >= cus;
  const bool s_level = e == 2 || (Wo != 16 ? (e == 3 || e == 4) : (e != 3 && (s_items >= cus || s_split)));
  const bool f4s = f4 && e != 0 && Cin % 8 == 0 && Ca % 2 == 0 && Wo != 128 && s_level &&
                   (!s_split || f2_geom);
  if (up) {
    if (!f4s || wino4s_up_env() == 0 || (Wo == 16 && s_items < cus)) return r;
    r.kernel = WinoRoute::F4S_UP;
    base = s_items;
  } else if (f4s && Ca % 4 == 0) {
    r.kernel = WinoRoute::F4S;
    base = s_items;
    split = s_split;
  } else if (f4 && Cin % 4 == 0 && Ca % 4 == 0 &&
             (Wo != 16 || (B % 2 == 0 && (wino4_w16_env() == 1 || t4 * B / 32 * ncog >= cus)))) {
    r.kernel = WinoRoute::F4;
    base = t4 * B / 32 * ncog;
    split = f2_geom && chunks_split(Cin / 4) && base < ksplit_items() * cus;
  } else if (have_f2_pack && f2_geom) {
    r.kernel = WinoRoute::F2;
    base = (Wo / 2) * (Wo / 2) / 64 * ncog * B;
    split = chunks_split(Cin / WKC) && base < ksplit_items() * cus;
  } else {
    return r;
  }
  const bool f2 = r.kernel == WinoRoute::F2, s = r.kernel == WinoRoute::F4S || r.kernel == WinoRoute::F4S_UP;
  r.ksplit = split ? 2 : 1;
  r.kbuf_floats = split ? (size_t)B * Cout * Wo * Wo : 0;
  r.items = base * r.ksplit;
  r.grid = r.items < cus ? r.items : cus;
  r.gn_parts = split ? 0 : (f2 ? (Wo / 2) * (Wo / 2) / 32 : t4 / 16);
  r.fold_ok = s && !split;
  r.fold_target = s ? t4 / 16 * ncog : 0;
  r.pack_kind = f2 ? ERTD_PACK_WINO : ERTD_PACK_WINO4;
  return r;
}

size_t conv_packed_floats_wino(int cin, int cout) {
  if (cin % WKC || cout % 64) return 0;
  return (size_t)16 * cout * cin;
}

hipError_t launch_pack_conv_wino(const float* w, int cin, int cout, float* dst, hipStream_t s,
                                 bool flipT) {
  const size_t total = conv_packed_floats_wino(cin, cout);
  if (!total) return hipErrorInvalidValue;
  const size_t items = total / 16;
  pack_wino_kernel<<<(unsigned)((items + 255) / 256), 256, 0, s>>>(w, cin, cout, cin / WKC, items, dst,
                                                                    flipT);
  return hipGetLastError();
}

hipError_t launch_conv_wino(int act, const ConvArgs& a, hipStream_t s, const WinoRoute& r) {
  if (r.ksplit == 2 && !a.ksplit_buf) return hipErrorInvalidValue;
  switch (r.kernel) {
    case WinoRoute::F4S:
    case WinoRoute::F4S_UP: return launch_conv_wino4s(act, a, s, r);
    case WinoRoute::F4: return launch_conv_wino4(act, a, s, r);
    case WinoRoute::F2: break;
    default: return hipErrorInvalidValue;
  }
  switch (act) {
    case ACT_NONE: return launch_act<ACT_NONE>(a, s, r);
    case ACT_GN_SILU: return launch_act<ACT_GN_SILU>(a, s, r);
    case ACT_GN: return launch_act<ACT_GN>(a, s, r);
    default: return hipErrorInvalidValue;
  }
}

}
}
```

ert-conditional-diffusion-model_amd/csrc/unet_conv_wino4.hip:

```cpp
#include <cstdlib>
#include <type_traits>

#include "unet.h"

namespace ertd {
namespace unet {

namespace {

constexpr int NMW = 8;
constexpr int NPW = 4;
constexpr int WT = 64 * (NMW + NPW);
constexpr int WKC = 4;
constexpr int NX = 36;
constexpr int U_FL = NX * 256;
constexpr int V_FL = NX * 128;
constexpr int NUB = 3;
constexpr int NRS = 3;
constexpr size_t WLDS = (size_t)(NUB * U_FL + 2 * V_FL) * sizeof(float);
constexpr int NDMA = U_FL / 256;
static_assert(NDMA == 4 * 5 + 4 * 4, "waves 0-3 issue 5 DMAs per chunk, waves 4-7 issue 4");
#ifndef WINO4_PPRIO
#define WINO4_PPRIO 2
#endif
#ifndef WINO4_PD
#define WINO4_PD 2
#endif
#ifndef WINO4_DMAI
#define WINO4_DMAI 1
#endif
using f32x4 = __attribute__((ext_vector_type(4))) float;
using f32x2 = __attribute__((ext_vector_type(2))) float;
using u32x4 = __attribute__((ext_vector_type(4))) unsigned;

constexpr double GD[6][3] = {{1.0, 0.0, 0.0},
                             {1.0 / 3, 1.0 / 3, 1.0 / 3},
                             {-1.0 / 3, 1.0 / 3, -1.0 / 3},
                             {-16.0 / 15, -8.0 / 15, -4.0 / 15},
                             {1.0 / 15, -2.0 / 15, 4.0 / 15},
                             {0.0, 0.0, 1.0}};

__device__ __forceinline__ f32x2 fmac(f32x2 x, float c, f32x2 s) {
  return __builtin_elementwise_fma(x, f32x2{c, c}, s);
}
__device__ __forceinline__ void bt6(const float (&d)[6], float (&o)[6]) {
  const float c = d[4] - d[2], e = d[3] - d[1];
  const float u = d[4] - d[1], v = d[4] + d[1];
  o[0] = __builtin_fmaf(1.5f, e, __builtin_fmaf(-2.f, d[2], d[0] + d[4]));
  o[1] = __builtin_fmaf(2.5f, d[3], __builtin_fmaf(0.5f, d[2], u));
  o[2] = __builtin_fmaf(0.5f, d[3], __builtin_fmaf(-2.5f, d[2], v));
  o[3] = __builtin_fmaf(2.f, e, c);
  o[4] = __builtin_fmaf(-0.5f, e, c);
  o[5] = __builtin_fmaf(1.5f, c, __builtin_fmaf(-2.f, d[3], d[1] + d[5]));
}
__device__ __forceinline__ void at6(const f32x2 (&m)[6], f32x2 (&y)[4]) {
  const f32x2 s = m[1] + m[2], d = m[1] - m[2];
  y[0] = (m[0] + s) + (m[3] + m[4]);
  y[1] = fmac(m[3], 0.5f, fmac(m[4], -2.f, d));
  y[2] = fmac(m[3], 0.25f, fmac(m[4], 4.f, s));
  y[3] = fmac(m[3], 0.125f, fmac(m[4], -8.f, d + m[5]));
}

__device__ __forceinline__ unsigned wlds_addr(const void* p) {
  return (unsigned)(uintptr_t)(const __attribute__((address_space(3))) char*)p;
}

#ifdef WINO4_STAMP
constexpr int NSS = 64;
constexpr int SPW = 2 + NSS * 5;
__device__ unsigned g_w4stamps[256 * 12 * SPW];
#define W4STAMP(ev, sl)                                                                  \
  do {                                                                                   \
    if (lane == 0 && (sl) < NSS)                                                         \
      stamps[wave * SPW + 2 + (sl) * 5 + (ev)] = (unsigned)__builtin_amdgcn_s_memtime(); \
  } while (0)
constexpr size_t WLDS_LAUNCH = WLDS + 12 * SPW * sizeof(unsigned);
#else
#define W4STAMP(ev, sl) \
  do {                  \
  } while (0)
constexpr size_t WLDS_LAUNCH = WLDS;
#endif

struct Item {
  int cog, blk;
};
__device__ __forceinline__ Item item_of(int it, int ncog) {
  Item r;
  r.cog = it % ncog;
  r.blk = it / ncog;
  return r;
}

template <int WO, int ACT, int DBG = 0>
__global__ __launch_bounds__(WT) void conv_wino4_kernel(ConvArgs a, int nitems, int ksp) {
  extern __shared__ __attribute__((aligned(16))) float smem[];
  float* ubuf = smem;
  float* vbuf = smem + NUB * U_FL;

  constexpr int TPR = WO / 4;
  constexpr int HW = WO * WO;
  constexpr int TS = TPR * TPR;
  static_assert(TPR >= 4 && (TS % 32 == 0 || 32 % TS == 0), "a 32-tile block is whole tile rows");
  const int tid = threadIdx.x;
  const int lane = tid & 63;
  const int wave = __builtin_amdgcn_readfirstlane(tid >> 6);
  const int Cin = a.Cin, Ca = a.Ca;
  const int nchunk = Cin / WKC;
  const int nck = nchunk / ksp;
  const int ncog = a.Cout / 64;
  const int bid = blockIdx.x, G = gridDim.x;
  const int nloc = bid < nitems ? (nitems - bid + G - 1) / G : 0;
  const int gtot = nloc * nck;
#ifdef WINO4_STAMP
  unsigned* stamps = reinterpret_cast<unsigned*>(smem + NUB * U_FL + 2 * V_FL);
  if (lane == 0) {
    stamps[wave * SPW] = (unsigned)__builtin_amdgcn_s_memrealtime();
    stamps[wave * SPW + 1] = (unsigned)__builtin_amdgcn_s_memtime();
  }
  auto stamp_flush = [&]() {
    __builtin_amdgcn_s_waitcnt(0);
    for (int i = lane; i < SPW; i += 64)
      g_w4stamps[((size_t)bid * 12 + wave) * SPW + i] = stamps[wave * SPW + i];
  };
#endif

  if (wave >= NMW) {
    __builtin_amdgcn_s_setprio(WINO4_PPRIO);
    const int q = wave - NMW;
    const int h = lane >> 5, t = lane & 31;
    const int vwoff = ((h * 18 + (t >> 4)) * 64 + q * 16 + (t & 15)) * 2;
    const int nbaddr = (lane + 31 - 62 * h) * 4;
    float2 raw[NRS][6];
    float2 gnv[NRS];
    f32x4 pad[NRS];
    int cur_g = 0, cur_k = 0, cur_k0 = 0, cur_b = 0, cur_il = 0;
    unsigned roff[6];
    unsigned soffA = 0, soffB = 0;
    f32x4 cur_pad;
    auto set_item = [&](int il) {
      const int it = bid + il * G;
      cur_k0 = (it % ksp) * nck;
      const Item itm = item_of(it / ksp, ncog);
      const int flat0 = itm.blk * 32;
      cur_b = flat0 / TS;
      const int tg = (flat0 + t) % TS;
      if constexpr (TS < 32) {
        const int ls = (flat0 + t) / TS - cur_b;
        soffA = (unsigned)(ls * Ca * HW * 4);
        soffB = (unsigned)(ls * a.Cb * HW * 4);
      }
      const int ty = tg / TPR, tx = tg - ty * TPR;
#pragma unroll
      for (int r = 0; r < 6; ++r) {
        const int iy = 4 * ty - 1 + r;
        roff[r] = (unsigned)(((iy >= 0 && iy < WO ? iy : 4 * ty) * WO + 4 * tx + 2 * h) * 4);
      }
      cur_pad = f32x4{ty > 0 ? 1.f : 0.f, ty < TPR - 1 ? 1.f : 0.f,
                      (h ? tx < TPR - 1 : tx > 0) ? 1.f : 0.f, 0.f};
    };
    const int glast = gtot - 1;
    auto load_next = [&](const int set) {
      const int cg = (cur_k0 + cur_k) * WKC + q;
      pad[set] = cur_pad;
      if constexpr (ACT != ACT_NONE) {
        if constexpr (TS < 32) gnv[set] = a.gn[(size_t)(cur_b + (t >= TS)) * Cin + cg];
        else gnv[set] = a.gn[(size_t)cur_b * Cin + cg];
      }
      const bool inA = cg < Ca;
      const float* p = inA ? a.srcA + ((size_t)cur_b * Ca + cg) * HW
                           : a.srcB + ((size_t)cur_b * a.Cb + (cg - Ca)) * HW;
      const unsigned soff = TS < 32 ? (inA ? soffA : soffB) : 0u;
      const int nrec = TS < 32 ? ((inA ? Ca : a.Cb) + 1) * HW * 4 : HW * 4;
      const __amdgpu_buffer_rsrc_t rs =
          __builtin_amdgcn_make_buffer_rsrc(const_cast<float*>(p), (short)0, nrec, 0x00020000);
#pragma unroll
      for (int r = 0; r < 6; ++r) {
        if constexpr (DBG & 2) {
          raw[set][r] = make_float2((float)(r + cur_k), (float)lane);
        } else {
          const auto v = __builtin_amdgcn_raw_buffer_load_b64(rs, (int)(roff[r] + soff), 0, 0);
          raw[set][r] = make_float2(__uint_as_float(v[0]), __uint_as_float(v[1]));
        }
      }
      if (cur_g < glast) {
        ++cur_g;
        if (++cur_k == nck) {
          cur_k = 0;
          set_item(++cur_il);
        }
      }
    };
    float act[2][3][6];
    auto act_stage = [&](const int set, const int ab) {
      if constexpr (DBG & 1) return;
#pragma unroll
      for (int r = 0; r < 6; ++r) {
        float2 m = raw[set][r];
        if constexpr (ACT != ACT_NONE) {
          m.x = __builtin_fmaf(m.x, gnv[set].x, gnv[set].y);
          m.y = __builtin_fmaf(m.y, gnv[set].x, gnv[set].y);
          if constexpr (ACT == ACT_GN_SILU) {
            m.x = m.x * __builtin_amdgcn_rcpf(1.0f + __expf(-m.x));
            m.y = m.y * __builtin_amdgcn_rcpf(1.0f + __expf(-m.y));
          }
        }
        if (r == 0 || r == 5) {
          const float fy = r == 0 ? pad[set].x : pad[set].y;
          m.x *= fy;
          m.y *= fy;
        }
        const float give = h ? m.y : m.x;
        const float nb = __int_as_float(__builtin_amdgcn_ds_bpermute(nbaddr, __float_as_int(give)));
        act[ab][0][r] = m.x;
        act[ab][1][r] = m.y;
        act[ab][2][r] = nb * pad[set].z;
      }
    };
    auto tr_stage = [&](const int ab, float* vb) {
      if constexpr (DBG & 1) return;
      float w[6][3];
#pragma unroll
      for (int c = 0; c < 3; ++c) {
        float o[6];
        bt6(act[ab][c], o);
#pragma unroll
        for (int i = 0; i < 6; ++i) w[i][c] = o[i];
      }
      float row[3][6];
#pragma unroll
      for (int aa = 0; aa < 3; ++aa)
#pragma unroll
        for (int c = 0; c < 3; ++c) {
          const auto sw = __builtin_amdgcn_permlane32_swap(__float_as_uint(w[aa][c]),
                                                           __float_as_uint(w[3 + aa][c]), false, false);
          const int jl = c == 0 ? 1 : (c == 1 ? 2 : 0);
          row[aa][jl] = __uint_as_float(sw[0]);
          row[aa][3 + c] = __uint_as_float(sw[1]);
        }
      float* o = vb + vwoff;
#pragma unroll
      for (int aa = 0; aa < 3; ++aa) {
        float vv[6];
        bt6(row[aa], vv);
#pragma unroll
        for (int jp = 0; jp < 6; jp += 2)
          *reinterpret_cast<f32x2*>(o + (aa * 3 + jp / 2) * 256) = f32x2{vv[jp], vv[jp + 1]};
      }
    };
    auto slot = [&](auto sa, auto ab, int g) {
      constexpr int SA = decltype(sa)::value, AB = decltype(ab)::value;
      W4STAMP(0, g);
      tr_stage(AB ^ 1, vbuf + ((g + 1) & 1) * V_FL);
      W4STAMP(1, g);
      act_stage(SA, AB);
      W4STAMP(4, g);
      load_next(SA);
      W4STAMP(2, g);
      __syncthreads();
      W4STAMP(3, g);
    };
    using I0 = std::integral_constant<int, 0>;
    using I1 = std::integral_constant<int, 1>;
    using I2 = std::integral_constant<int, 2>;
    if (gtot > 0) {
      set_item(0);
      load_next(0);
      load_next(1);
      load_next(2);
      act_stage(0, 0);
      tr_stage(0, vbuf);
      load_next(0);
      act_stage(1, 1);
      load_next(1);
    }
    __syncthreads();
    int g = 0;
    for (; g + 5 < gtot; g += 6) {
      slot(I2{}, I0{}, g);
      slot(I0{}, I1{}, g + 1);
      slot(I1{}, I0{}, g + 2);
      slot(I2{}, I1{}, g + 3);
      slot(I0{}, I0{}, g + 4);
      slot(I1{}, I1{}, g + 5);
    }
    if (g < gtot) slot(I2{}, I0{}, g);
    if (g + 1 < gtot) slot(I0{}, I1{}, g + 1);
    if (g + 2 < gtot) slot(I1{}, I0{}, g + 2);
    if (g + 3 < gtot) slot(I2{}, I1{}, g + 3);
    if (g + 4 < gtot) slot(I0{}, I0{}, g + 4);
#ifdef WINO4_STAMP
    stamp_flush();
#endif
    return;
  }

#ifdef WINO4_MPRIO
  __builtin_amdgcn_s_setprio(WINO4_MPRIO);
#endif
  const int cb = wave & 3, tb = wave >> 2;
  f32x4 acc[NX];
  const int ndma = wave < 4 ? 5 : 4;
  const int dfirst = wave < 4 ? wave * 5 : 20 + (wave - 4) * 4;
  int d_k = 0, d_il = 0;
  const float* d_src = a.wpk_wino4;
  auto d_item = [&](int il) {
    const int it = bid + il * G;
    d_src = a.wpk_wino4 + ((size_t)((it / ksp) % ncog) * nchunk + (size_t)(it % ksp) * nck) * U_FL;
  };
  if (nloc > 0) d_item(0);
  auto dma_one = [&](const int j, const int slot) {
    if constexpr (DBG & 4) return;
    int ln;
    asm volatile("v_mbcnt_lo_u32_b32 %0, -1, 0\n\tv_mbcnt_hi_u32_b32 %0, -1, %0" : "=v"(ln));
    const int ins = dfirst + j;
    const float* src = d_src + (size_t)d_k * U_FL + ins * 256 + ln * 4;
    const unsigned ldst = __builtin_amdgcn_readfirstlane(wlds_addr(ubuf + slot * U_FL + ins * 256));
    unsigned keep;
    asm volatile(
        "s_mov_b32 %0, m0\n\ts_mov_b32 m0, %2\n\ts_nop 0\n\t"
        "global_load_lds_dwordx4 %1, off\n\ts_mov_b32 m0, %0"
        : "=&s"(keep)
        : "v"(src), "s"(ldst)
        : "memory");
  };
  auto dma_advance = [&]() {
    if (++d_k == nck) {
      d_k = 0;
      if (++d_il < nloc) d_item(d_il);
    }
  };
  auto dma_all = [&](const int slot) {
#pragma unroll
    for (int j = 0; j < 5; ++j)
      if (j < 4 || wave < 4) dma_one(j, slot);
    dma_advance();
  };
  if (gtot > 0) dma_all(0);
  if (gtot > 1) dma_all(1);
  asm volatile("s_waitcnt vmcnt(0)" ::: "memory");
  __syncthreads();
  int su = 0, sd = 2;
  for (int il = 0; il < nloc; ++il) {
#pragma unroll
    for (int x = 0; x < NX; ++x) acc[x] = f32x4{};
    for (int k = 0; k < nck; ++k) {
      const int g = il * nck + k;
      const bool dma = g + 2 < gtot;
      W4STAMP(0, g);
#if !WINO4_DMAI
      if (dma) dma_all(sd);
#endif
      W4STAMP(1, g);
      int ln;
      asm volatile("v_mbcnt_lo_u32_b32 %0, -1, 0\n\tv_mbcnt_hi_u32_b32 %0, -1, %0" : "=v"(ln));
      const float* ub = ubuf + su * U_FL + (cb * 64 + ln) * 2;
      const float* vb = vbuf + (g & 1) * V_FL + (tb * 64 + ln) * 2;
      constexpr int PD = WINO4_PD;
      f32x2 ra[PD + 1], rb[PD + 1];
      auto ld = [&](const int xp) {
        const int r = xp % (PD + 1);
        if constexpr (DBG & 16) {
          ra[r] = f32x2{(float)(ln + xp), (float)k};
          rb[r] = f32x2{(float)(xp - ln), 1.f};
        } else {
          ra[r] = *reinterpret_cast<const f32x2*>(ub + xp * 512);
          rb[r] = *reinterpret_cast<const f32x2*>(vb + xp * 256);
        }
      };
#pragma unroll
      for (int xp = 0; xp < PD; ++xp) ld(xp);
#pragma unroll
      for (int xp = 0; xp < NX / 2; ++xp) {
        if (xp + PD < NX / 2) ld(xp + PD);
        const int r = xp % (PD + 1);
        if constexpr (DBG & 8) {
          acc[2 * xp][0] += ra[r].x * rb[r].x;
          acc[2 * xp + 1][0] += ra[r].y * rb[r].y;
        } else {
          acc[2 * xp] = __builtin_amdgcn_mfma_f32_16x16x4f32(ra[r].x, rb[r].x, acc[2 * xp], 0, 0, 0);
          acc[2 * xp + 1] = __builtin_amdgcn_mfma_f32_16x16x4f32(ra[r].y, rb[r].y, acc[2 * xp + 1], 0, 0, 0);
        }
        if (xp + PD < NX / 2) __builtin_amdgcn_sched_group_barrier(0x100, 2, 0);
        __builtin_amdgcn_sched_group_barrier(0x008, 2, 0);
#if WINO4_DMAI
        if (xp >= 1 && xp <= 5 && (xp <= 4 || wave < 4))
          if (dma) dma_one(xp - 1, sd);
#endif
      }
#if WINO4_DMAI
      if (dma) dma_advance();
#endif
      su = su == NUB - 1 ? 0 : su + 1;
      sd = sd == NUB - 1 ? 0 : sd + 1;
#pragma unroll
      for (int x = 0; x < NX; ++x) asm volatile("" : "+v"(acc[x]));
      W4STAMP(2, g);
      if (dma) {
        if (wave < 4) asm volatile("s_waitcnt vmcnt(5)" ::: "memory");
        else asm volatile("s_waitcnt vmcnt(4)" ::: "memory");
      } else {
        asm volatile("s_waitcnt vmcnt(0)" ::: "memory");
      }
      W4STAMP(4, g);
      __syncthreads();
      W4STAMP(3, g);
    }

    if constexpr (DBG & 32) {
      if (il == nloc - 1) {
        float sacc = 0.f;
        for (int x = 0; x < NX; ++x) sacc += acc[x][0] + acc[x][3];
        a.out[(size_t)bid * 64 + lane] = sacc;
      }
      continue;
    }
    const int itg = bid + il * G;
    const Item itm = item_of(itg / ksp, ncog);
    const int flatw = itm.blk * 32 + tb * 16;
    const int smpl = flatw / TS;
    const bool part2 = (itg % ksp) != 0;
    const bool has_eb = a.ebias && !part2, has_res = a.res && !part2, has_bias = a.bias && !part2;
    const unsigned smp = (unsigned)(a.Cout * HW * 4);
    const __amdgpu_buffer_rsrc_t ro = __builtin_amdgcn_make_buffer_rsrc(
        (part2 ? a.ksplit_buf : a.out) + (size_t)smpl * a.Cout * HW, (short)0, smp, 0x00020000);
    const __amdgpu_buffer_rsrc_t rr = __builtin_amdgcn_make_buffer_rsrc(
        has_res ? const_cast<float*>(a.res) + (size_t)smpl * a.Cout * HW : nullptr, (short)0, smp,
        0x00020000);
    f32x4 y[4][4];
#pragma unroll
    for (int pp = 0; pp < 2; ++pp) {
      f32x2 P[6][4];
#pragma unroll
      for (int i = 0; i < 6; ++i) {
        f32x2 m[6];
#pragma unroll
        for (int j = 0; j < 6; ++j) m[j] = f32x2{acc[6 * i + j][2 * pp], acc[6 * i + j][2 * pp + 1]};
        at6(m, P[i]);
      }
#pragma unroll
      for (int x = 0; x < 4; ++x) {
        f32x2 col[6], yc[4];
#pragma unroll
        for (int i = 0; i < 6; ++i) col[i] = P[i][x];
        at6(col, yc);
#pragma unroll
        for (int r = 0; r < 4; ++r) {
          y[2 * pp][r][x] = yc[r].x;
          y[2 * pp + 1][r][x] = yc[r].y;
        }
      }
    }
    int ln;
    asm volatile("v_mbcnt_lo_u32_b32 %0, -1, 0\n\tv_mbcnt_hi_u32_b32 %0, -1, %0" : "=v"(ln));
    const int co0 = itm.cog * 64 + cb * 16 + 4 * (ln >> 4);
    const int tg = flatw % TS + (ln & 15);
    const int ty = tg / TPR, tx = tg - ty * TPR;
    const int vo = (co0 * HW + 4 * ty * WO + 4 * tx) * 4;
#pragma unroll
    for (int i = 0; i < 4; ++i) {
      const float bi = has_bias ? a.bias[co0 + i] : 0.f;
      const float ei = has_eb ? a.ebias[(size_t)smpl * a.eb_stride + co0 + i] : 0.f;
#pragma unroll
      for (int r = 0; r < 4; ++r) {
        y[i][r] = y[i][r] + bi;
        if (has_eb) y[i][r] = y[i][r] + ei;
      }
    }
    __builtin_amdgcn_sched_barrier(0);
    if (has_res) {
      f32x4 rv[4][4];
#pragma unroll
      for (int i = 0; i < 4; ++i)
#pragma unroll
        for (int r = 0; r < 4; ++r)
          rv[i][r] = __builtin_bit_cast(f32x4, __builtin_amdgcn_raw_buffer_load_b128(rr, vo, i * HW * 4 + r * WO * 4, 0));
#pragma unroll
      for (int i = 0; i < 4; ++i)
#pragma unroll
        for (int r = 0; r < 4; ++r) y[i][r] = y[i][r] + rv[i][r];
    }
    if (a.gnp && ksp == 1) {
      float2 pr[4];
#pragma unroll
      for (int i = 0; i < 4; ++i) {
        float sm = 0.f;
#pragma unroll
        for (int r = 0; r < 4; ++r) sm += (y[i][r][0] + y[i][r][1]) + (y[i][r][2] + y[i][r][3]);
        sm = row16_sum(sm);
        const float mu = sm * (1.0f / 256.0f);
        float q = 0.f;
#pragma unroll
        for (int r = 0; r < 4; ++r)
#pragma unroll
          for (int x = 0; x < 4; ++x) {
            const float d = y[i][r][x] - mu;
            q = __builtin_fmaf(d, d, q);
          }
        pr[i] = make_float2(sm, row16_sum(q));
      }
      if ((ln & 15) == 0) {
        const int np = TS / 16, part = (flatw % TS) / 16;
#pragma unroll
        for (int i = 0; i < 4; ++i) a.gnp[((size_t)smpl * a.Cout + co0 + i) * np + part] = pr[i];
      }
    }
#pragma unroll
    for (int i = 0; i < 4; ++i)
#pragma unroll
      for (int r = 0; r < 4; ++r)
        __builtin_amdgcn_raw_buffer_store_b128(__builtin_bit_cast(u32x4, y[i][r]), ro, vo,
                                               i * HW * 4 + r * WO * 4, 0);
  }
#ifdef WINO4_STAMP
  stamp_flush();
#endif
}

__global__ void pack_wino4_kernel(const float* __restrict__ w, int cin, int cout, int nchunk,
                                  size_t total, float* __restrict__ dst, bool flipT) {
  const size_t i = (size_t)blockIdx.x * blockDim.x + threadIdx.x;
  if (i >= total) return;
  const int e = (int)(i & 1);
  const int c16 = (int)((i >> 1) & 15);
  const int kk = (int)((i >> 5) & 3);
  const int cb = (int)((i >> 7) & 3);
  size_t rest = i >> 9;
  const int xi = 2 * (int)(rest % (NX / 2)) + e;
  rest /= NX / 2;
  const int k = (int)(rest % nchunk);
  const int cog = (int)(rest / nchunk);
  const int co = cog * 64 + cb * 16 + c16;
  const int ci = k * WKC + kk;
  const int ri = xi / 6, rj = xi % 6;
  const float* g = flipT ? w + ((size_t)ci * cout + co) * 9 : w + ((size_t)co * cin + ci) * 9;
  double u = 0.0;
#pragma unroll
  for (int y = 0; y < 3; ++y) {
    double row = 0.0;
#pragma unroll
    for (int x = 0; x < 3; ++x) row += (double)(flipT ? g[8 - (y * 3 + x)] : g[y * 3 + x]) * GD[rj][x];
    u += GD[ri][y] * row;
  }
  dst[i] = (float)u;
}

template <int WO, int ACT, int DBG>
hipError_t launch_wo4d(const ConvArgs& a, hipStream_t s, const WinoRoute& r) {
  static std::atomic<unsigned long long> attr{0};
  set_max_lds_once((const void*)conv_wino4_kernel<WO, ACT, DBG>, (int)WLDS_LAUNCH, attr);
  conv_wino4_kernel<WO, ACT, DBG><<<r.grid, WT, WLDS_LAUNCH, s>>>(a, r.items, r.ksplit);
  hipError_t e = hipGetLastError();
  if (e != hipSuccess || r.ksplit == 1) return e;
  return launch_add_inplace(a.out, a.ksplit_buf, r.kbuf_floats, s);
}

#ifdef ERTD_DIAG
int wino4_dbg() {
  static int v = [] {
    return ERTD_KNOB("WINO4_DBG", 0);
  }();
  return v;
}
#endif

template <int WO, int ACT>
hipError_t launch_wo4(const ConvArgs& a, hipStream_t s, const WinoRoute& r) {
#ifdef ERTD_DIAG
  if constexpr (WO == 64 && ACT == ACT_GN_SILU) {
    switch (wino4_dbg()) {
      case 1: return launch_wo4d<WO, ACT, 1>(a, s, r);
      case 2: return launch_wo4d<WO, ACT, 2>(a, s, r);
      case 3: return launch_wo4d<WO, ACT, 3>(a, s, r);
      case 4: return launch_wo4d<WO, ACT, 4>(a, s, r);
      case 8: return launch_wo4d<WO, ACT, 8>(a, s, r);
      case 16: return launch_wo4d<WO, ACT, 16>(a, s, r);
      case 32: return launch_wo4d<WO, ACT, 32>(a, s, r);
      case 7: return launch_wo4d<WO, ACT, 7>(a, s, r);
      case 23: return launch_wo4d<WO, ACT, 23>(a, s, r);
      default: break;
    }
  }
#endif
  return launch_wo4d<WO, ACT, 0>(a, s, r);
}

template <int ACT>
hipError_t launch_act4(const ConvArgs& a, hipStream_t s, const WinoRoute& r) {
  switch (a.Wo) {
    case 16: return launch_wo4<16, ACT>(a, s, r);
    case 32: return launch_wo4<32, ACT>(a, s, r);
    case 64: return launch_wo4<64, ACT>(a, s, r);
    case 128: return launch_wo4<128, ACT>(a, s, r);
    default: return hipErrorInvalidValue;
  }
}

}

#ifdef WINO4_STAMP
extern "C" int ertd_diag_wino4_stamps(unsigned* host, size_t n) {
  const size_t cap = sizeof(g_w4stamps) / sizeof(unsigned);
  return (int)hipMemcpyFromSymbol(host, HIP_SYMBOL(g_w4stamps), (n < cap ? n : cap) * sizeof(unsigned), 0,
                                  hipMemcpyDeviceToHost);
}
#endif

size_t conv_packed_floats_wino4(int cin, int cout) {
  if (cin % WKC || cout % 64) return 0;
  return (size_t)NX * cout * cin;
}

hipError_t launch_pack_conv_wino4(const float* w, int cin, int cout, float* dst, hipStream_t s,
                                  bool flipT) {
  const size_t total = conv_packed_floats_wino4(cin, cout);
  if (!total) return hipErrorInvalidValue;
  pack_wino4_kernel<<<(unsigned)((total + 255) / 256), 256, 0, s>>>(w, cin, cout, cin / WKC, total, dst,
                                                                     flipT);
  return hipGetLastError();
}

hipError_t launch_conv_wino4(int act, const ConvArgs& a, hipStream_t s, const WinoRoute& r) {
  switch (act) {
    case ACT_NONE: return launch_act4<ACT_NONE>(a, s, r);
    case ACT_GN_SILU: return launch_act4<ACT_GN_SILU>(a, s, r);
    case ACT_GN: return launch_act4<ACT_GN>(a, s, r);
    default: return hipErrorInvalidValue;
  }
}

}
}
```

ert-conditional-diffusion-model_amd/csrc/unet_conv_wino4s.hip:

```cpp
#include <cstdlib>
#include <type_traits>

#include "unet.h"

namespace ertd {
namespace unet {

namespace {

constexpr int NMW = 4;
constexpr int NPW = 4;
constexpr int CCH = 8;
constexpr int NX = 36;
constexpr int VKS = 18 * 128;
constexpr int V_FL = 2 * VKS;
constexpr size_t WLDS = (size_t)2 * V_FL * sizeof(float);
constexpr int NRS = 3;
constexpr int GNC_JM = 4;
constexpr int GNC_KM = 6;
constexpr int GNC_TAB = 4096;
#ifndef WINO4S_PPRIO
#define WINO4S_PPRIO 2
#endif
#ifndef WINO4S_PD
#define WINO4S_PD 2
#endif
#ifndef WINO4S_MPRIO
#define WINO4S_MPRIO 1
#endif
#ifndef WINO4S_XCD
#define WINO4S_XCD 1
#endif
#ifndef WINO4S_XCDMAX
#define WINO4S_XCDMAX 2
#endif
#ifndef WINO4S_PACK
#define WINO4S_PACK 1
#endif
#ifndef WINO4S_HALO
#define WINO4S_HALO 1
#endif
#ifndef WINO4S_RPF
#define WINO4S_RPF 0
#endif
#ifndef WINO4S_ABL
#define WINO4S_ABL 0
#endif
using f32x4 = __attribute__((ext_vector_type(4))) float;
using f32x2 = __attribute__((ext_vector_type(2))) float;
using u32x4 = __attribute__((ext_vector_type(4))) unsigned;
using u32x2 = __attribute__((ext_vector_type(2))) unsigned;

__device__ __forceinline__ f32x2 fmac(f32x2 x, float c, f32x2 s) {
  return __builtin_elementwise_fma(x, f32x2{c, c}, s);
}
__device__ __forceinline__ void bt6(const float (&d)[6], float (&o)[6]) {
  const float c = d[4] - d[2], e = d[3] - d[1];
  const float u = d[4] - d[1], v = d[4] + d[1];
  o[0] = __builtin_fmaf(1.5f, e, __builtin_fmaf(-2.f, d[2], d[0] + d[4]));
  o[1] = __builtin_fmaf(2.5f, d[3], __builtin_fmaf(0.5f, d[2], u));
  o[2] = __builtin_fmaf(0.5f, d[3], __builtin_fmaf(-2.5f, d[2], v));
  o[3] = __builtin_fmaf(2.f, e, c);
  o[4] = __builtin_fmaf(-0.5f, e, c);
  o[5] = __builtin_fmaf(1.5f, c, __builtin_fmaf(-2.f, d[3], d[1] + d[5]));
}
__device__ __forceinline__ f32x2 pfma(f32x2 a, float c, f32x2 b) {
  return __builtin_elementwise_fma(a, f32x2{c, c}, b);
}
__device__ __forceinline__ void bt6p(const f32x2 (&d)[6], f32x2 (&o)[6]) {
  const f32x2 c = d[4] - d[2], e = d[3] - d[1];
  const f32x2 u = d[4] - d[1], v = d[4] + d[1];
  o[0] = pfma(e, 1.5f, pfma(d[2], -2.f, d[0] + d[4]));
  o[1] = pfma(d[3], 2.5f, pfma(d[2], 0.5f, u));
  o[2] = pfma(d[3], 0.5f, pfma(d[2], -2.5f, v));
  o[3] = pfma(e, 2.f, c);
  o[4] = pfma(e, -0.5f, c);
  o[5] = pfma(c, 1.5f, pfma(d[3], -2.f, d[1] + d[5]));
}
template <int N, bool SHL>
__device__ __forceinline__ f32x2 row_shift0(f32x2 v) {
  constexpr int ctrl = (SHL ? 0x100 : 0x110) + N;
  return f32x2{__int_as_float(__builtin_amdgcn_update_dpp(0, __float_as_int(v.x), ctrl, 0xf, 0xf, true)),
               __int_as_float(__builtin_amdgcn_update_dpp(0, __float_as_int(v.y), ctrl, 0xf, 0xf, true))};
}
template <int N, bool SHL>
__device__ __forceinline__ f32x2 row_shift_keep(f32x2 old, f32x2 v) {
  constexpr int ctrl = (SHL ? 0x100 : 0x110) + N;
  return f32x2{__int_as_float(__builtin_amdgcn_update_dpp(__float_as_int(old.x), __float_as_int(v.x), ctrl, 0xf, 0xf, false)),
               __int_as_float(__builtin_amdgcn_update_dpp(__float_as_int(old.y), __float_as_int(v.y), ctrl, 0xf, 0xf, false))};
}
__device__ __forceinline__ void at6(const f32x2 (&m)[6], f32x2 (&y)[4]) {
  const f32x2 s = m[1] + m[2], d = m[1] - m[2];
  y[0] = (m[0] + s) + (m[3] + m[4]);
  y[1] = fmac(m[3], 0.5f, fmac(m[4], -2.f, d));
  y[2] = fmac(m[3], 0.25f, fmac(m[4], 4.f, s));
  y[3] = fmac(m[3], 0.125f, fmac(m[4], -8.f, d + m[5]));
}

__device__ __forceinline__ void wino4s_fold_tail(const GnFold& f, int lane, int wave, int nmw) {
  for (int b = blockIdx.x; b < f.B; b += gridDim.x) {
    if (wave == 0 && lane == 0) {
      const unsigned* c = f.cnt + b;
      while (__hip_atomic_load(c, __ATOMIC_RELAXED, __HIP_MEMORY_SCOPE_AGENT) != (unsigned)f.target)
        __builtin_amdgcn_s_sleep(2);
      __hip_atomic_store(f.cnt + b, 0u, __ATOMIC_RELAXED, __HIP_MEMORY_SCOPE_AGENT);
    }
    __syncthreads();
    gn_group_finalize<true>(f.g, b, lane, wave, nmw);
  }
}

#ifdef WINO4S_STAMP
constexpr int S4_SPW = 64;
__device__ unsigned g_w4s_stamps[256 * 12 * S4_SPW];
#define W4S_STAMP(slot)                                                                            \
  do {                                                                                             \
    if (blockIdx.x < 256 && lane == 0)                                                             \
      g_w4s_stamps[(blockIdx.x * 12 + wave) * S4_SPW + (slot)] = (unsigned)__builtin_amdgcn_s_memtime(); \
  } while (0)
#define W4S_STAMP_ENTRY()                                                                          \
  do {                                                                                             \
    if (blockIdx.x < 256 && lane == 0) {                                                           \
      g_w4s_stamps[(blockIdx.x * 12 + wave) * S4_SPW] = (unsigned)__builtin_amdgcn_s_memrealtime(); \
      g_w4s_stamps[(blockIdx.x * 12 + wave) * S4_SPW + 1] = (unsigned)__builtin_amdgcn_s_memtime(); \
    }                                                                                              \
  } while (0)
#else
#define W4S_STAMP(slot) \
  do {                  \
  } while (0)
#define W4S_STAMP_ENTRY() \
  do {                    \
  } while (0)
#endif

struct Item {
  int cog, blk, half;
};
__device__ __forceinline__ Item item_of(int it, int ncog, int ksp) {
  Item r;
  r.half = it % ksp;
  const int pr = it / ksp;
  r.cog = pr % ncog;
  r.blk = pr / ncog;
  return r;
}

struct ItemWalk {
  int base, stride, ncog, ksp;
  __device__ __forceinline__ Item at(int il) const { return item_of(base + il * stride, ncog, ksp); }
};
__device__ __forceinline__ int itm_half(const ItemWalk& w, int il) { return w.at(il).half; }

template <int WO, int ACT, bool UP, int XS, bool FOLD, bool GNC>
__global__ __launch_bounds__(64 * (4 * XS + NPW)) void conv_wino4s_kernel(ConvArgs a, int nitems, int ksp, int cw) {
  static_assert(!GNC || (XS == 2 && !UP && ACT != ACT_NONE && !FOLD), "GNC: the xi-split GN+act kernel");
  extern __shared__ __attribute__((aligned(16))) float smem[];
  float* vbuf = smem;
  int* fold_items = nullptr;
  if constexpr (FOLD) {
    __shared__ int fold_lds;
    fold_items = &fold_lds;
    if (threadIdx.x == 0) fold_lds = 0;
  }

  constexpr int TPR = WO / 4;
  constexpr int HW = WO * WO;
  constexpr int TS = TPR * TPR;
  constexpr int WS = UP ? WO / 2 : WO;
  constexpr int HWS = WS * WS;
  static_assert(TS % 16 == 0 && TPR <= 16, "a 16-tile block is whole tile rows of one sample");
  const int tid = threadIdx.x;
  const int lane = tid & 63;
  const int wave = __builtin_amdgcn_readfirstlane(tid >> 6);
  W4S_STAMP_ENTRY();
  const int Cin = a.Cin, Ca = a.Ca;
  const int nchunk = Cin / CCH / ksp;
  const int ncog = a.Cout / 64;
  const int G = gridDim.x;
  const int bid = (WINO4S_XCD && G % 8 == 0 && ncog <= WINO4S_XCDMAX)
                      ? (int)(blockIdx.x % 8) * (G / 8) + (int)(blockIdx.x / 8) : (int)blockIdx.x;
  const ItemWalk wk = cw ? ItemWalk{bid * cw, 1, ncog, ksp} : ItemWalk{bid, G, ncog, ksp};
  const int nloc = cw ? (bid * cw < nitems ? min(cw, nitems - bid * cw) : 0)
                      : (bid < nitems ? (nitems - bid + G - 1) / G : 0);
  float2* const gtab = reinterpret_cast<float2*>(smem + 2 * V_FL + 4 * 2 * 8 * 256);
  const int gtot = nloc * nchunk;

  if (wave >= 4 * XS) {
    __builtin_amdgcn_s_setprio(WINO4S_PPRIO);
    const int q = wave - 4 * XS;
    const int chb = lane >> 5, h = (lane >> 4) & 1, t = lane & 15;
    const int cl = 2 * q + chb;
    const int vwoff = ((((cl >> 2) * 18 + 9 * h) * 4 + (cl & 3)) * 16 + t) * 2;
    const int nbaddr = (lane + 15 - 30 * h) * 4;
    const unsigned choff = (unsigned)(chb * HWS * 4);
    constexpr bool HALO = WINO4S_HALO && WINO4S_PACK && !UP && TPR <= 8;
    constexpr int NWR = HALO ? (TPR == 8 ? 5 : 4) : 6;
    float2 raw[NRS][NWR];
    float2 gnv[NRS];
    int gch[NRS];
    f32x4 pad[NRS];
    int cur_g = 0, cur_k = 0, cur_b = 0, cur_il = 0, cur_k0 = 0;
    unsigned roff[NWR];
    f32x4 cur_pad;
    auto set_item = [&](int il) {
      const Item itm = wk.at(il);
      cur_k0 = itm.half * nchunk;
      const int flat0 = itm.blk * 16;
      cur_b = flat0 / TS;
      const int tg = flat0 % TS + t;
      const int ty = tg / TPR, tx = tg - ty * TPR;
      if constexpr (UP) {
#pragma unroll
        for (int r = 0; r < 4; ++r) {
          const int sy = 2 * ty - 1 + r;
          roff[r] = (unsigned)(((sy >= 0 && sy < WS ? sy : 2 * ty) * WS + 2 * tx + h) * 4) + choff;
        }
      } else if constexpr (HALO) {
#pragma unroll
        for (int r = 0; r < 4; ++r) roff[r] = (unsigned)(((4 * ty + r) * WO + 4 * tx + 2 * h) * 4) + choff;
        if constexpr (TPR == 8) {
          const int iy = t < 8 ? 4 * ty - 1 : 4 * ty + 4;
          roff[4] = (unsigned)(((iy >= 0 && iy < WO ? iy : 4 * ty) * WO + 4 * tx + 2 * h) * 4) + choff;
        }
      } else {
#pragma unroll
        for (int r = 0; r < 6; ++r) {
          const int iy = 4 * ty - 1 + r;
          roff[r] = (unsigned)(((iy >= 0 && iy < WO ? iy : 4 * ty) * WO + 4 * tx + 2 * h) * 4) + choff;
        }
      }
      cur_pad = f32x4{ty > 0 ? 1.f : 0.f, ty < TPR - 1 ? 1.f : 0.f,
                      (h ? tx < TPR - 1 : tx > 0) ? 1.f : 0.f, 0.f};
    };
    const int glast = gtot - 1;
    auto load_next = [&](const int set) {
      const int cg = (cur_k0 + cur_k) * CCH + 2 * q;
      pad[set] = cur_pad;
      if constexpr (GNC) gch[set] = cur_il * Cin + cg + chb;
      else if constexpr (ACT != ACT_NONE) gnv[set] = a.gn[(size_t)cur_b * Cin + cg + chb];
      const bool inA = cg < Ca;
      const float* p = inA ? a.srcA + ((size_t)cur_b * Ca + cg) * HWS
                           : a.srcB + ((size_t)cur_b * a.Cb + (cg - Ca)) * HWS;
      const __amdgpu_buffer_rsrc_t rs =
          __builtin_amdgcn_make_buffer_rsrc(const_cast<float*>(p), (short)0, 2 * HWS * 4, 0x00020000);
      if constexpr (UP) {
        float v[4];
#pragma unroll
        for (int r = 0; r < 4; ++r) v[r] = __uint_as_float(__builtin_amdgcn_raw_buffer_load_b32(rs, (int)roff[r], 0, 0));
#pragma unroll
        for (int r = 0; r < 6; ++r) {
          const float u = v[(r + 1) >> 1];
          raw[set][r] = make_float2(u, u);
        }
      } else {
#pragma unroll
        for (int r = 0; r < NWR; ++r) {
          const auto v = __builtin_amdgcn_raw_buffer_load_b64(rs, (int)roff[r], 0, 0);
          raw[set][r] = make_float2(__uint_as_float(v[0]), __uint_as_float(v[1]));
        }
      }
      if (cur_g < glast) {
        ++cur_g;
        if (++cur_k == nchunk) {
          cur_k = 0;
          set_item(++cur_il);
        }
      }
    };
#if WINO4S_PACK
    f32x2 act2[2][6];
    float actn[2][6];
    auto act_stage = [&](const int set, const int ab) {
      if constexpr (GNC) gnv[set] = gtab[gch[set]];
      auto activate = [&](const float2 rw) {
        f32x2 v = f32x2{rw.x, rw.y};
        if constexpr (ACT != ACT_NONE) {
          v = __builtin_elementwise_fma(v, f32x2{gnv[set].x, gnv[set].x}, f32x2{gnv[set].y, gnv[set].y});
          if constexpr (ACT == ACT_GN_SILU) {
            f32x2 e = v * f32x2{-1.44269504088896340736f, -1.44269504088896340736f};
            e = f32x2{__builtin_amdgcn_exp2f(e.x), __builtin_amdgcn_exp2f(e.y)} + f32x2{1.0f, 1.0f};
            v = v * f32x2{__builtin_amdgcn_rcpf(e.x), __builtin_amdgcn_rcpf(e.y)};
          }
        }
        return v;
      };
      f32x2 m[6];
      if constexpr (HALO) {
#pragma unroll
        for (int r = 0; r < 4; ++r) m[1 + r] = activate(raw[set][r]);
        if constexpr (TPR == 8) {
          const f32x2 x = activate(raw[set][4]);
          m[0] = row_shift_keep<TPR, false>(x, m[4]);
          m[5] = row_shift_keep<TPR, true>(x, m[1]);
        } else {
          m[0] = row_shift0<TPR, false>(m[4]);
          m[5] = row_shift0<TPR, true>(m[1]);
        }
      } else {
#pragma unroll
        for (int r = 0; r < 6; ++r) m[r] = activate(raw[set][r]);
      }
      m[0] = m[0] * f32x2{pad[set].x, pad[set].x};
      m[5] = m[5] * f32x2{pad[set].y, pad[set].y};
      bt6p(m, act2[ab]);
#pragma unroll
      for (int i = 0; i < 6; ++i) {
        const float give = h ? act2[ab][i].y : act2[ab][i].x;
        const float nb = __int_as_float(__builtin_amdgcn_ds_bpermute(nbaddr, __float_as_int(give)));
        actn[ab][i] = nb * pad[set].z;
      }
    };
#else
    float act[2][3][6];
    auto act_stage = [&](const int set, const int ab) {
      if constexpr (GNC) gnv[set] = gtab[gch[set]];
      float cx[6], cy[6];
#pragma unroll
      for (int r = 0; r < 6; ++r) {
        float2 m = raw[set][r];
        if constexpr (ACT != ACT_NONE) {
          m.x = __builtin_fmaf(m.x, gnv[set].x, gnv[set].y);
          m.y = __builtin_fmaf(m.y, gnv[set].x, gnv[set].y);
          if constexpr (ACT == ACT_GN_SILU) {
            m.x = m.x * __builtin_amdgcn_rcpf(1.0f + __expf(-m.x));
            m.y = m.y * __builtin_amdgcn_rcpf(1.0f + __expf(-m.y));
          }
        }
        if (r == 0 || r == 5) {
          const float fy = r == 0 ? pad[set].x : pad[set].y;
          m.x *= fy;
          m.y *= fy;
        }
        cx[r] = m.x;
        cy[r] = m.y;
      }
      bt6(cx, act[ab][0]);
      bt6(cy, act[ab][1]);
#pragma unroll
      for (int i = 0; i < 6; ++i) {
        const float give = h ? act[ab][1][i] : act[ab][0][i];
        const float nb = __int_as_float(__builtin_amdgcn_ds_bpermute(nbaddr, __float_as_int(give)));
        act[ab][2][i] = nb * pad[set].z;
      }
    };
#endif
    auto tr_stage = [&](const int ab, float* vb) {
      float w[6][3];
#if WINO4S_PACK
#pragma unroll
      for (int i = 0; i < 6; ++i) {
        w[i][0] = act2[ab][i].x;
        w[i][1] = act2[ab][i].y;
        w[i][2] = actn[ab][i];
      }
#else
#pragma unroll
      for (int c = 0; c < 3; ++c)
#pragma unroll
        for (int i = 0; i < 6; ++i) w[i][c] = act[ab][c][i];
#endif
      float row[3][6];
#pragma unroll
      for (int aa = 0; aa < 3; ++aa)
#pragma unroll
        for (int c = 0; c < 3; ++c) {
          const auto sw = __builtin_amdgcn_permlane16_swap(__float_as_uint(w[aa][c]),
                                                           __float_as_uint(w[3 + aa][c]), false, false);
          const int jl = c == 0 ? 1 : (c == 1 ? 2 : 0);
          row[aa][jl] = __uint_as_float(sw[0]);
          row[aa][3 + c] = __uint_as_float(sw[1]);
        }
      float* o = vb + vwoff;
#pragma unroll
      for (int aa = 0; aa < 3; ++aa) {
        float vv[6];
        bt6(row[aa], vv);
#pragma unroll
        for (int jp = 0; jp < 6; jp += 2)
          *reinterpret_cast<f32x2*>(o + (aa * 3 + jp / 2) * 128) = f32x2{vv[jp], vv[jp + 1]};
      }
    };
    auto slot = [&](auto sa, auto ab, int g) {
      constexpr int SA = decltype(sa)::value, AB = decltype(ab)::value;
      if constexpr (!(WINO4S_ABL & 1)) {
        tr_stage(AB ^ 1, vbuf + ((g + 1) & 1) * V_FL);
        act_stage(SA, AB);
      }
      load_next(SA);
      if constexpr (!(WINO4S_ABL & 16)) __syncthreads();
    };
    using I0 = std::integral_constant<int, 0>;
    using I1 = std::integral_constant<int, 1>;
    using I2 = std::integral_constant<int, 2>;
    if (gtot > 0) {
      set_item(0);
      load_next(0);
      load_next(1);
      load_next(2);
    }
    if constexpr (GNC) {
      W4S_STAMP(25);
      __syncthreads();
      W4S_STAMP(26);
    }
    if (gtot > 0) {
      act_stage(0, 0);
      tr_stage(0, vbuf);
      load_next(0);
      act_stage(1, 1);
      load_next(1);
    }
    W4S_STAMP(3);
    __syncthreads();
    W4S_STAMP(2);
    int g = 0;
    for (; g + 5 < gtot; g += 6) {
      slot(I2{}, I0{}, g);
      slot(I0{}, I1{}, g + 1);
      slot(I1{}, I0{}, g + 2);
      slot(I2{}, I1{}, g + 3);
      slot(I0{}, I0{}, g + 4);
      slot(I1{}, I1{}, g + 5);
    }
    if (g < gtot) slot(I2{}, I0{}, g);
    if (g + 1 < gtot) slot(I0{}, I1{}, g + 1);
    if (g + 2 < gtot) slot(I1{}, I0{}, g + 2);
    if (g + 3 < gtot) slot(I2{}, I1{}, g + 3);
    if (g + 4 < gtot) slot(I0{}, I0{}, g + 4);
    W4S_STAMP(27);
    return;
  }

  if constexpr (XS == 1) {
  const int cb = wave;
  f32x4 acc[NX];
  const int nks = Cin / 4;
  const __amdgpu_buffer_rsrc_t ru = __builtin_amdgcn_make_buffer_rsrc(
      const_cast<float*>(a.wpk_wino4), (short)0, (int)((size_t)NX * a.Cout * Cin * 4), 0x00020000);
  int u_il = 0, u_ks = 0;
  int u_base = 0;
  auto u_item = [&](int il) {
    const Item itm = wk.at(il);
    u_base = itm.cog * nks * 36864;
  };
  auto u_advance = [&]() {
    if (++u_ks == nks) {
      if (u_il + 1 < nloc) {
        u_ks = 0;
        u_item(++u_il);
      } else {
        u_ks = nks - 1;
      }
    }
  };
  if (nloc > 0) u_item(0);
  f32x2 ub[2][18];
  const int uvoff = lane * 8 + cb * 512;
  auto u_load = [&](f32x2 (&u)[18], const int p) {
    if constexpr ((WINO4S_ABL & 32) != 0) {
      u[p] = u[p] + f32x2{1.f, 1.f};
      return;
    }
    const auto v = __builtin_amdgcn_raw_buffer_load_b64(
        ru, uvoff, (WINO4S_ABL & 2) ? p * 2048 : u_base + u_ks * 36864 + p * 2048, 0);
    u[p] = f32x2{__uint_as_float(v[0]), __uint_as_float(v[1])};
  };
  if (nloc > 0) {
#pragma unroll
    for (int p = 0; p < 18; ++p) u_load(ub[0], p);
    u_advance();
  }
  __syncthreads();
#ifndef WINO4S_XK
#define WINO4S_XK 1
#endif
  auto kstep = [&](const f32x2 (&u)[18], f32x2 (&nx)[18], const float* vs) {
    constexpr int PD = WINO4S_PD;
    f32x2 rb[PD + 1];
#pragma unroll
    for (int p = 0; p < PD; ++p) rb[p] = *reinterpret_cast<const f32x2*>(vs + p * 128);
#pragma unroll
    for (int p = 0; p < 18; ++p) {
      if (p + PD < 18) rb[(p + PD) % (PD + 1)] = *reinterpret_cast<const f32x2*>(vs + (p + PD) * 128);
      const int r = p % (PD + 1);
      if constexpr (WINO4S_ABL & 4) {
        acc[2 * p][0] = __builtin_fmaf(u[p].x, rb[r].x, acc[2 * p][0]);
        acc[2 * p + 1][0] = __builtin_fmaf(u[p].y, rb[r].y, acc[2 * p + 1][0]);
      } else {
        acc[2 * p] = __builtin_amdgcn_mfma_f32_16x16x4f32(u[p].x, rb[r].x, acc[2 * p], 0, 0, 0);
        acc[2 * p + 1] = __builtin_amdgcn_mfma_f32_16x16x4f32(u[p].y, rb[r].y, acc[2 * p + 1], 0, 0, 0);
      }
      u_load(nx, p);
      if (p + PD < 18) __builtin_amdgcn_sched_group_barrier(0x100, 1, 0);
      __builtin_amdgcn_sched_group_barrier(0x008, 2, 0);
      __builtin_amdgcn_sched_group_barrier(0x020, 1, 0);
    }
    u_advance();
  };
  auto chunk2 = [&](const float* vs) {
    constexpr int PD = WINO4S_PD;
    f32x2 rb[PD + 1];
#pragma unroll
    for (int q = 0; q < PD; ++q) rb[q] = *reinterpret_cast<const f32x2*>(vs + q * 128);
#pragma unroll
    for (int q = 0; q < 36; ++q) {
      const int st = q / 18, p = q % 18;
      const int qn = q + PD;
      if (qn < 36) rb[qn % (PD + 1)] = *reinterpret_cast<const f32x2*>(vs + (qn / 18) * VKS + (qn % 18) * 128);
      const int r = q % (PD + 1);
      const f32x2 u = st == 0 ? ub[0][p] : ub[1][p];
      acc[2 * p] = __builtin_amdgcn_mfma_f32_16x16x4f32(u.x, rb[r].x, acc[2 * p], 0, 0, 0);
      acc[2 * p + 1] = __builtin_amdgcn_mfma_f32_16x16x4f32(u.y, rb[r].y, acc[2 * p + 1], 0, 0, 0);
      if (st == 0) u_load(ub[1], p);
      else u_load(ub[0], p);
      if (qn < 36) __builtin_amdgcn_sched_group_barrier(0x100, 1, 0);
      __builtin_amdgcn_sched_group_barrier(0x008, 2, 0);
      __builtin_amdgcn_sched_group_barrier(0x020, 1, 0);
      if (p == 17) u_advance();
    }
  };
  for (int il = 0; il < nloc; ++il) {
#pragma unroll
    for (int x = 0; x < NX; ++x) acc[x] = f32x4{};
    for (int k = 0; k < nchunk; ++k) {
      const int g = il * nchunk + k;
      int ln;
      asm volatile("v_mbcnt_lo_u32_b32 %0, -1, 0\n\tv_mbcnt_hi_u32_b32 %0, -1, %0" : "=v"(ln));
      const float* vb = vbuf + (g & 1) * V_FL + ln * 2;
      if constexpr (WINO4S_XK && !(WINO4S_ABL & 4)) {
        chunk2(vb);
      } else {
        kstep(ub[0], ub[1], vb);
        kstep(ub[1], ub[0], vb + VKS);
      }
#pragma unroll
      for (int x = 0; x < NX; ++x) asm volatile("" : "+v"(acc[x]));
      if constexpr (!(WINO4S_ABL & 16)) __syncthreads();
    }

    if constexpr ((WINO4S_ABL & 8) != 0) {
      if (il == nloc - 1) {
        float sacc = 0.f;
        for (int x = 0; x < NX; ++x) sacc += acc[x][0] + acc[x][3];
        a.out[(size_t)bid * 64 + lane] = sacc;
      }
      continue;
    }
    const Item itm = wk.at(il);
    const int flatw = itm.blk * 16;
    const int smpl = flatw / TS;
    const bool has_eb = a.ebias != nullptr, has_res = a.res != nullptr, has_bias = a.bias != nullptr;
    const unsigned smp = (unsigned)(a.Cout * HW * 4);
    const __amdgpu_buffer_rsrc_t ro = __builtin_amdgcn_make_buffer_rsrc(
        a.out + (size_t)smpl * a.Cout * HW, (short)0, smp, 0x00020000);
    const __amdgpu_buffer_rsrc_t rr = __builtin_amdgcn_make_buffer_rsrc(
        has_res ? const_cast<float*>(a.res) + (size_t)smpl * a.Cout * HW : nullptr, (short)0, smp,
        0x00020000);
    f32x4 y[4][4];
#pragma unroll
    for (int pp = 0; pp < 2; ++pp) {
      f32x2 P[6][4];
#pragma unroll
      for (int i = 0; i < 6; ++i) {
        f32x2 m[6];
#pragma unroll
        for (int j = 0; j < 6; ++j) m[j] = f32x2{acc[6 * i + j][2 * pp], acc[6 * i + j][2 * pp + 1]};
        at6(m, P[i]);
      }
#pragma unroll
      for (int x = 0; x < 4; ++x) {
        f32x2 col[6], yc[4];
#pragma unroll
        for (int i = 0; i < 6; ++i) col[i] = P[i][x];
        at6(col, yc);
#pragma unroll
        for (int r = 0; r < 4; ++r) {
          y[2 * pp][r][x] = yc[r].x;
          y[2 * pp + 1][r][x] = yc[r].y;
        }
      }
    }
    int ln;
    asm volatile("v_mbcnt_lo_u32_b32 %0, -1, 0\n\tv_mbcnt_hi_u32_b32 %0, -1, %0" : "=v"(ln));
    const int co0 = itm.cog * 64 + cb * 16 + 4 * (ln >> 4);
    const int tg = flatw % TS + (ln & 15);
    const int ty = tg / TPR, tx = tg - ty * TPR;
    const int vo = (co0 * HW + 4 * ty * WO + 4 * tx) * 4;
#pragma unroll
    for (int i = 0; i < 4; ++i) {
      const float bi = has_bias ? a.bias[co0 + i] : 0.f;
      const float ei = has_eb ? a.ebias[(size_t)smpl * a.eb_stride + co0 + i] : 0.f;
#pragma unroll
      for (int r = 0; r < 4; ++r) {
        y[i][r] = y[i][r] + bi;
        if (has_eb) y[i][r] = y[i][r] + ei;
      }
    }
    __builtin_amdgcn_sched_barrier(0);
    if (has_res) {
      f32x4 rv[4][4];
#pragma unroll
      for (int i = 0; i < 4; ++i)
#pragma unroll
        for (int r = 0; r < 4; ++r)
          rv[i][r] = __builtin_bit_cast(f32x4, __builtin_amdgcn_raw_buffer_load_b128(rr, vo, i * HW * 4 + r * WO * 4, 0));
#pragma unroll
      for (int i = 0; i < 4; ++i)
#pragma unroll
        for (int r = 0; r < 4; ++r) y[i][r] = y[i][r] + rv[i][r];
    }
    if (a.gnp) {
      float2 pr[4];
#pragma unroll
      for (int i = 0; i < 4; ++i) {
        float sm = 0.f;
#pragma unroll
        for (int r = 0; r < 4; ++r) sm += (y[i][r][0] + y[i][r][1]) + (y[i][r][2] + y[i][r][3]);
        sm = row16_sum(sm);
        const float mu = sm * (1.0f / 256.0f);
        float qq = 0.f;
#pragma unroll
        for (int r = 0; r < 4; ++r)
#pragma unroll
          for (int x = 0; x < 4; ++x) {
            const float d = y[i][r][x] - mu;
            qq = __builtin_fmaf(d, d, qq);
          }
        pr[i] = make_float2(sm, row16_sum(qq));
      }
      if ((ln & 15) == 0) {
        const int np = TS / 16, part = (flatw % TS) / 16;
#pragma unroll
        for (int i = 0; i < 4; ++i) {
          float2* d = a.gnp + ((size_t)smpl * a.Cout + co0 + i) * np + part;
          if constexpr (FOLD) st_f2_wt(d, pr[i]);
          else *d = pr[i];
        }
      }
      if constexpr (FOLD) gn_fold_item_done(a.fold, smpl, fold_items, NMW, ln);
    }
#pragma unroll
    for (int i = 0; i < 4; ++i)
#pragma unroll
      for (int r = 0; r < 4; ++r)
        __builtin_amdgcn_raw_buffer_store_b128(__builtin_bit_cast(u32x4, y[i][r]), ro, vo,
                                               i * HW * 4 + r * WO * 4, 0);
  }
  if constexpr (FOLD) wino4s_fold_tail(a.fold, lane, wave, NMW);
  } else {
  constexpr int NP = 9;
  const int cb = wave & 3, xh = wave >> 2;
#if WINO4S_MPRIO
  if (xh) __builtin_amdgcn_s_setprio(WINO4S_MPRIO);
#endif
  float* xbuf = smem + 2 * V_FL;
  f32x4 acc[2 * NP];
  const int nks = Cin / 4;
  const __amdgpu_buffer_rsrc_t ru = __builtin_amdgcn_make_buffer_rsrc(
      const_cast<float*>(a.wpk_wino4), (short)0, (int)((size_t)NX * a.Cout * Cin * 4), 0x00020000);
  int u_il = 0, u_ks = 0, u_end = 0, u_base = 0;
  auto u_item = [&](int il) {
    const Item itm = wk.at(il);
    u_base = itm.cog * nks * 36864;
    u_ks = itm.half * nchunk * 2;
    u_end = u_ks + nchunk * 2;
  };
  auto u_advance = [&]() {
    if (++u_ks == u_end) {
      if (u_il + 1 < nloc) {
        u_item(++u_il);
      } else {
        u_ks = u_end - 1;
      }
    }
  };
  if (nloc > 0) u_item(0);
  f32x2 ub[2][NP];
  const int uvoff = lane * 8 + cb * 512;
  const int psoff = xh * NP * 2048;
  auto u_load = [&](f32x2 (&u)[NP], const int p) {
    const auto v = __builtin_amdgcn_raw_buffer_load_b64(ru, uvoff, u_base + u_ks * 36864 + psoff + p * 2048, 0);
    u[p] = f32x2{__uint_as_float(v[0]), __uint_as_float(v[1])};
  };
  if (nloc > 0) {
#pragma unroll
    for (int p = 0; p < NP; ++p) u_load(ub[0], p);
    u_advance();
  }
  if constexpr (GNC) {
    constexpr int JM = GNC_JM;
    const int ng4 = (a.gnc.groups + 3) / 4;
    int smp[JM], jg[JM], row[JM];
    bool jl[JM];
#pragma unroll
    for (int j = 0; j < JM; ++j) {
      const int job = wave + 4 * XS * j, il = job / ng4;
      jl[j] = il < nloc;
      row[j] = jl[j] ? il : 0;
      jg[j] = job - il * ng4;
      smp[j] = jl[j] ? wk.at(il).blk * 16 / TS : 0;
    }
    gn_group_finalize_regs<JM, GNC_KM>(a.gnc, smp, jg, row, jl, lane, gtab);
    W4S_STAMP(25);
    __syncthreads();
    W4S_STAMP(26);
  }
  __syncthreads();
  W4S_STAMP(2);
  auto chunk2 = [&](const float* vs) {
    constexpr int PD = WINO4S_PD;
    f32x2 rb[PD + 1];
#pragma unroll
    for (int q = 0; q < PD; ++q) rb[q] = *reinterpret_cast<const f32x2*>(vs + (xh * NP + q) * 128);
#pragma unroll
    for (int q = 0; q < 2 * NP; ++q) {
      const int st = q / NP, p = q % NP;
      const int qn = q + PD;
      if (qn < 2 * NP)
        rb[qn % (PD + 1)] = *reinterpret_cast<const f32x2*>(vs + (qn / NP) * VKS + (xh * NP + qn % NP) * 128);
      const int r = q % (PD + 1);
      const f32x2 u = st == 0 ? ub[0][p] : ub[1][p];
      acc[2 * p] = __builtin_amdgcn_mfma_f32_16x16x4f32(u.x, rb[r].x, acc[2 * p], 0, 0, 0);
      acc[2 * p + 1] = __builtin_amdgcn_mfma_f32_16x16x4f32(u.y, rb[r].y, acc[2 * p + 1], 0, 0, 0);
      if (st == 0) u_load(ub[1], p);
      else u_load(ub[0], p);
      if (qn < 2 * NP) __builtin_amdgcn_sched_group_barrier(0x100, 1, 0);
      __builtin_amdgcn_sched_group_barrier(0x008, 2, 0);
      __builtin_amdgcn_sched_group_barrier(0x020, 1, 0);
      if (p == NP - 1) u_advance();
    }
  };
  for (int il = 0; il < nloc; ++il) {
#pragma unroll
    for (int x = 0; x < 2 * NP; ++x) acc[x] = f32x4{};
    f32x2 own[4][4];
    if (il < 8) W4S_STAMP(3 + 3 * il);
    unsigned rpf[2] = {0u, 0u};
    for (int k = 0; k < nchunk; ++k) {
      const int g = il * nchunk + k;
      int ln;
      asm volatile("v_mbcnt_lo_u32_b32 %0, -1, 0\n\tv_mbcnt_hi_u32_b32 %0, -1, %0" : "=v"(ln));
#if WINO4S_RPF
      if (k == (nchunk > WINO4S_RPF ? nchunk - WINO4S_RPF : 0) && a.res && itm_half(wk, il) == 0) {
        const Item pit = wk.at(il);
        const int pflat = pit.blk * 16, psm = pflat / TS;
        const int pco = pit.cog * 64 + cb * 16 + 4 * (ln >> 4) + 2 * xh + ((ln >> 3) & 1);
        const int pr = (ln >> 1) & 3;
        const __amdgpu_buffer_rsrc_t rp = __builtin_amdgcn_make_buffer_rsrc(
            const_cast<float*>(a.res) + (size_t)psm * a.Cout * HW, (short)0, (unsigned)(a.Cout * HW * 4), 0x00020000);
#pragma unroll
        for (int h = 0; h < 2; ++h) {
          const int ptg = pflat % TS + (ln & 1) * 8 + h * 4;
          const int pty = ptg / TPR, ptx = ptg - pty * TPR;
          rpf[h] = __builtin_amdgcn_raw_buffer_load_b32(rp, (pco * HW + (4 * pty + pr) * WO + 4 * ptx) * 4, 0, 0);
        }
      }
#endif
      chunk2(vbuf + (g & 1) * V_FL + ln * 2);
#pragma unroll
      for (int x = 0; x < 2 * NP; ++x) asm volatile("" : "+v"(acc[x]));
      if (k == nchunk - 1) {
#pragma unroll
        for (int pp = 0; pp < 2; ++pp) {
          f32x2 P[3][4];
#pragma unroll
          for (int i = 0; i < 3; ++i) {
            f32x2 m[6];
#pragma unroll
            for (int j = 0; j < 6; ++j) m[j] = f32x2{acc[6 * i + j][2 * pp], acc[6 * i + j][2 * pp + 1]};
            at6(m, P[i]);
          }
          f32x2 Y[4][4];
#pragma unroll
          for (int x = 0; x < 4; ++x) {
            if (xh == 0) {
              const f32x2 s12 = P[1][x] + P[2][x], d12 = P[1][x] - P[2][x];
              Y[0][x] = P[0][x] + s12;
              Y[1][x] = d12;
              Y[2][x] = s12;
              Y[3][x] = d12;
            } else {
              Y[0][x] = P[0][x] + P[1][x];
              Y[1][x] = fmac(P[0][x], 0.5f, P[1][x] * f32x2{-2.f, -2.f});
              Y[2][x] = fmac(P[0][x], 0.25f, P[1][x] * f32x2{4.f, 4.f});
              Y[3][x] = fmac(P[0][x], 0.125f, fmac(P[1][x], -8.f, P[2][x]));
            }
          }
          if (pp == xh) {
#pragma unroll
            for (int r = 0; r < 4; ++r)
#pragma unroll
              for (int x = 0; x < 4; ++x) own[r][x] = Y[r][x];
          } else {
            float* xw = xbuf + ((cb * 2 + (xh ^ 1)) * 8) * 256 + lane * 4;
#pragma unroll
            for (int r = 0; r < 4; ++r)
#pragma unroll
              for (int x = 0; x < 4; x += 2)
                *reinterpret_cast<f32x4*>(xw + (r * 2 + x / 2) * 256) =
                    f32x4{Y[r][x].x, Y[r][x].y, Y[r][x + 1].x, Y[r][x + 1].y};
          }
        }
      }
      __syncthreads();
#ifdef WINO4S_STAMP
      if (g < 32) W4S_STAMP(28 + g);
#endif
    }
    if (il < 8) W4S_STAMP(4 + 3 * il);
    int ln;
    asm volatile("v_mbcnt_lo_u32_b32 %0, -1, 0\n\tv_mbcnt_hi_u32_b32 %0, -1, %0" : "=v"(ln));
    f32x4 y[2][4];
    {
      const float* xr = xbuf + ((cb * 2 + xh) * 8) * 256 + ln * 4;
#pragma unroll
      for (int r = 0; r < 4; ++r)
#pragma unroll
        for (int x = 0; x < 4; x += 2) {
          const f32x4 o = *reinterpret_cast<const f32x4*>(xr + (r * 2 + x / 2) * 256);
          const f32x2 q0 = own[r][x] + f32x2{o[0], o[1]}, q1 = own[r][x + 1] + f32x2{o[2], o[3]};
          y[0][r][x] = q0.x;
          y[1][r][x] = q0.y;
          y[0][r][x + 1] = q1.x;
          y[1][r][x + 1] = q1.y;
        }
    }
    const Item itm = wk.at(il);
    const int flatw = itm.blk * 16;
    const int smpl = flatw / TS;
    const bool part2 = itm.half != 0;
    const bool has_eb = !part2 && a.ebias != nullptr, has_res = !part2 && a.res != nullptr,
               has_bias = !part2 && a.bias != nullptr;
    const unsigned smp = (unsigned)(a.Cout * HW * 4);
    const __amdgpu_buffer_rsrc_t ro = __builtin_amdgcn_make_buffer_rsrc(
        (part2 ? a.ksplit_buf : a.out) + (size_t)smpl * a.Cout * HW, (short)0, smp, 0x00020000);
    const __amdgpu_buffer_rsrc_t rr = __builtin_amdgcn_make_buffer_rsrc(
        has_res ? const_cast<float*>(a.res) + (size_t)smpl * a.Cout * HW : nullptr, (short)0, smp,
        0x00020000);
    const int co0 = itm.cog * 64 + cb * 16 + 4 * (ln >> 4) + 2 * xh;
    const int tg = flatw % TS + (ln & 15);
    const int ty = tg / TPR, tx = tg - ty * TPR;
    const int vo = (co0 * HW + 4 * ty * WO + 4 * tx) * 4;
#pragma unroll
    for (int i = 0; i < 2; ++i) {
      const float bi = has_bias ? a.bias[co0 + i] : 0.f;
      const float ei = has_eb ? a.ebias[(size_t)smpl * a.eb_stride + co0 + i] : 0.f;
#pragma unroll
      for (int r = 0; r < 4; ++r) {
        y[i][r] = y[i][r] + bi;
        if (has_eb) y[i][r] = y[i][r] + ei;
      }
    }
    __builtin_amdgcn_sched_barrier(0);
    if (has_res) {
      f32x4 rv[2][4];
#pragma unroll
      for (int i = 0; i < 2; ++i)
#pragma unroll
        for (int r = 0; r < 4; ++r)
          rv[i][r] = __builtin_bit_cast(f32x4, __builtin_amdgcn_raw_buffer_load_b128(rr, vo, i * HW * 4 + r * WO * 4, 0));
#pragma unroll
      for (int i = 0; i < 2; ++i)
#pragma unroll
        for (int r = 0; r < 4; ++r) y[i][r] = y[i][r] + rv[i][r];
    }
    asm volatile("" ::"v"(rpf[0]), "v"(rpf[1]));
    if (a.gnp && !part2) {
      float2 pr[2];
#pragma unroll
      for (int i = 0; i < 2; ++i) {
        float sm = 0.f;
#pragma unroll
        for (int r = 0; r < 4; ++r) sm += (y[i][r][0] + y[i][r][1]) + (y[i][r][2] + y[i][r][3]);
        sm = row16_sum(sm);
        const float mu = sm * (1.0f / 256.0f);
        float qq = 0.f;
#pragma unroll
        for (int r = 0; r < 4; ++r)
#pragma unroll
          for (int x = 0; x < 4; ++x) {
            const float d = y[i][r][x] - mu;
            qq = __builtin_fmaf(d, d, qq);
          }
        pr[i] = make_float2(sm, row16_sum(qq));
      }
      if ((ln & 15) == 0) {
        const int np = TS / 16, part = (flatw % TS) / 16;
#pragma unroll
        for (int i = 0; i < 2; ++i) {
          float2* d = a.gnp + ((size_t)smpl * a.Cout + co0 + i) * np + part;
          if constexpr (FOLD) st_f2_wt(d, pr[i]);
          else *d = pr[i];
        }
      }
      if constexpr (FOLD) gn_fold_item_done(a.fold, smpl, fold_items, 4 * XS, ln);
    }
#pragma unroll
    for (int i = 0; i < 2; ++i)
#pragma unroll
      for (int r = 0; r < 4; ++r)
        __builtin_amdgcn_raw_buffer_store_b128(__builtin_bit_cast(u32x4, y[i][r]), ro, vo,
                                               i * HW * 4 + r * WO * 4, 0);
    if (il < 8) W4S_STAMP(5 + 3 * il);
  }
  W4S_STAMP(27);
  if constexpr (FOLD) wino4s_fold_tail(a.fold, lane, wave, 4 * XS);
  }

}

}

#ifdef WINO4S_STAMP
extern "C" int ertd_diag_wino4s_stamps(unsigned* host, size_t n) {
  const size_t cap = sizeof(g_w4s_stamps) / sizeof(unsigned);
  return (int)hipMemcpyFromSymbol(host, HIP_SYMBOL(g_w4s_stamps), (n < cap ? n : cap) * sizeof(unsigned), 0,
                                  hipMemcpyDeviceToHost);
}
extern "C" int ertd_diag_wino4s_stamps_clear() {
  static unsigned zero[256 * 12 * S4_SPW];
  return (int)hipMemcpyToSymbol(HIP_SYMBOL(g_w4s_stamps), zero, sizeof(zero), 0, hipMemcpyHostToDevice);
}
#endif

static int wino4s_cwalk_env() {
  static const int v = [] {
    return ERTD_KNOB("WINO4S_CWALK", 0);
  }();
  return v;
}

static int wino4s_cw_geom(int Cin, const WinoRoute& r) {
  if (r.ksplit != 1 || wino4s_xs() != 2 || Cin < 16 || r.grid < 1 || r.items % r.grid) return 0;
  const int cw = r.items / r.grid;
  return r.fold_target % cw == 0 ? cw : 0;
}

namespace {

int wino4s_cwalk(const ConvArgs& a, const WinoRoute& r) {
  if (wino4s_cwalk_env() == 0 || a.fold.cnt) return 0;
  return wino4s_cw_geom(a.Cin, r);
}

template <int WO, int ACT, bool UP, int XS>
hipError_t launch_wo4x(const ConvArgs& a, hipStream_t s, const WinoRoute& r) {
  constexpr size_t lds = WLDS + (XS == 2 ? (size_t)4 * 2 * 8 * 256 * sizeof(float) : 0);
  const int nitems = r.items, grid = r.grid, ksp = r.ksplit;
  if (ksp != 1 && (a.gnc.pa || a.fold.cnt || XS != 2)) return hipErrorInvalidValue;
  const int cw = wino4s_cwalk(a, r);
#ifdef ERTD_DIAG
  if (a.fold.cnt) {
    static std::atomic<unsigned long long> attr{0};
    set_max_lds_once((const void*)conv_wino4s_kernel<WO, ACT, UP, XS, true, false>, (int)lds, attr);
    conv_wino4s_kernel<WO, ACT, UP, XS, true, false><<<grid, 64 * (4 * XS + NPW), lds, s>>>(a, nitems, ksp, cw);
  } else
#else
  if (a.fold.cnt) return hipErrorInvalidValue;
#endif
  if constexpr (XS == 2 && !UP && ACT != ACT_NONE) {
    if (a.gnc.pa) {
      const int nlocmax = (nitems + grid - 1) / grid;
      const size_t ldsg = lds + (size_t)(cw ? cw : nlocmax) * a.Cin * sizeof(float2);
      static std::atomic<unsigned long long> attr{0};
      set_max_lds_once((const void*)conv_wino4s_kernel<WO, ACT, UP, XS, false, true>,
                       (int)(lds + GNC_TAB * sizeof(float2)), attr);
      conv_wino4s_kernel<WO, ACT, UP, XS, false, true><<<grid, 64 * (4 * XS + NPW), ldsg, s>>>(a, nitems, ksp, cw);
      return hipGetLastError();
    }
  }
  if (a.gnc.pa) return hipErrorInvalidValue;
  {
    static std::atomic<unsigned long long> attr{0};
    set_max_lds_once((const void*)conv_wino4s_kernel<WO, ACT, UP, XS, false, false>, (int)lds, attr);
    conv_wino4s_kernel<WO, ACT, UP, XS, false, false><<<grid, 64 * (4 * XS + NPW), lds, s>>>(a, nitems, ksp, cw);
  }
  hipError_t e = hipGetLastError();
  if (e != hipSuccess || ksp == 1) return e;
  return launch_add_inplace(a.out, a.ksplit_buf, r.kbuf_floats, s);
}

template <int WO, int ACT, bool UP>
hipError_t launch_wo4s(const ConvArgs& a, hipStream_t s, const WinoRoute& r) {
  if (wino4s_xs() == 2 && a.Cin >= 16) return launch_wo4x<WO, ACT, UP, 2>(a, s, r);
  return launch_wo4x<WO, ACT, UP, 1>(a, s, r);
}

template <int ACT, bool UP>
hipError_t launch_act4s(const ConvArgs& a, hipStream_t s, const WinoRoute& r) {
  switch (a.Wo) {
    case 16: return launch_wo4s<16, ACT, UP>(a, s, r);
    case 32: return launch_wo4s<32, ACT, UP>(a, s, r);
    case 64: return launch_wo4s<64, ACT, UP>(a, s, r);
    default: return hipErrorInvalidValue;
  }
}

}

bool wino_gnc_ok(const WinoRoute& r, int Cin, int Wo, const GnPartArgs& g) {
  static const int env = [] {
    return ERTD_KNOB("UNET_GNC", 3);
  }();
  if (r.kernel != WinoRoute::F4S || r.ksplit != 1) return false;
  if (!env || wino4s_xs() != 2 || Cin < 16) return false;
  if (!g.pa || g.groups < 1 || g.Ca + g.Cb != Cin || Cin % g.groups || g.npa < 1 ||
      (g.Cb > 0 && (!g.pb || g.npb < 1)) || g.HW != Wo * Wo || g.HW % g.npa ||
      (g.Cb > 0 && g.HW % g.npb))
    return false;
  const int nloc = wino4s_cwalk_env() ? wino4s_cw_geom(Cin, r) : (r.items + r.grid - 1) / r.grid;
  const int cpg = Cin / g.groups;
  const int np = g.npa > g.npb ? g.npa : g.npb;
  if (env == 2 && nloc > 1) return false;
  if (env == 3 && nloc > 2) return false;
  return nloc > 0 && nloc * ((g.groups + 3) / 4) <= 8 * GNC_JM && cpg <= GN_LPG &&
         cpg * np <= GN_LPG * GNC_KM && nloc * Cin <= GNC_TAB;
}

hipError_t launch_conv_wino4s(int act, const ConvArgs& a, hipStream_t s, const WinoRoute& r) {
  if (r.kernel == WinoRoute::F4S_UP)
    return act == ACT_NONE ? launch_act4s<ACT_NONE, true>(a, s, r) : hipErrorInvalidValue;
  if (r.kernel != WinoRoute::F4S) return hipErrorInvalidValue;
  switch (act) {
    case ACT_NONE: return launch_act4s<ACT_NONE, false>(a, s, r);
    case ACT_GN_SILU: return launch_act4s<ACT_GN_SILU, false>(a, s, r);
    case ACT_GN: return launch_act4s<ACT_GN, false>(a, s, r);
    default: return hipErrorInvalidValue;
  }
}

}
}
```

ert-conditional-diffusion-model_amd/csrc/unet_pack.h:

```cpp
#pragma once
#include "unet.h"

namespace ertd {
namespace unet {

__host__ __device__ constexpr int conv_ck(int ks) { return ks == 3 ? 4 : (ks == 2 ? 8 : 32); }
constexpr int WINO_KC = 8;
constexpr int WINO4_KC = 4;

__device__ __forceinline__ float pack_conv_elem(const float* __restrict__ w, int cin, int cout, int ks,
                                                int nchunk, size_t i, bool flipT) {
  const int ck = conv_ck(ks), ch = ck / 2;
  const int spc = ks == 3 ? 9 * ch : ch;
  const int e = (int)(i & 1);
  const int lane = (int)((i >> 1) & 63);
  size_t rest = i >> 7;
  const int sp = (int)(rest % (spc / 2));
  rest /= (spc / 2);
  const int k = (int)(rest % nchunk);
  const int tile = (int)(rest / nchunk);
  const int s = 2 * sp + e;
  const int hh = lane >> 5;
  const int co = tile * 32 + (lane & 31);
  int ci, ky, kx;
  if (ks == 3) { ci = k * ck + hh * ch + s / 9; ky = (s % 9) / 3; kx = s % 3; }
  else { ci = k * ck + hh * ch + s; ky = 0; kx = 0; }
  if (co >= cout || ci >= cin) return 0.f;
  return flipT ? w[(((size_t)ci * cout + co) * ks + (ks - 1 - ky)) * ks + (ks - 1 - kx)]
               : w[(((size_t)co * cin + ci) * ks + ky) * ks + kx];
}

__device__ __forceinline__ float pack_conv_up_elem(const float* __restrict__ w, int cin, int cout, int nchunk,
                                                   size_t per_class, size_t gi) {
  const int cls = (int)(gi / per_class);
  const size_t i = gi - (size_t)cls * per_class;
  const int pa = cls >> 1, pb = cls & 1;
  constexpr int ck = conv_ck(2), ch = ck / 2, spc = 4 * ch;
  const int e = (int)(i & 1);
  const int lane = (int)((i >> 1) & 63);
  size_t rest = i >> 7;
  const int sp = (int)(rest % (spc / 2));
  rest /= (spc / 2);
  const int k = (int)(rest % nchunk);
  const int tile = (int)(rest / nchunk);
  const int st = 2 * sp + e;
  const int co = tile * 32 + (lane & 31);
  const int ci = k * ck + (lane >> 5) * ch + st / 4;
  const int ty = (st % 4) / 2, tx = st % 2;
  float v = 0.f;
  if (co < cout && ci < cin) {
    const float* wk = w + ((size_t)co * cin + ci) * 9;
    const int y0 = (pa == 0) ? (ty == 0 ? 0 : 1) : (ty == 0 ? 0 : 2);
    const int y1 = (pa == 0) ? (ty == 0 ? 0 : 2) : (ty == 0 ? 1 : 2);
    const int x0 = (pb == 0) ? (tx == 0 ? 0 : 1) : (tx == 0 ? 0 : 2);
    const int x1 = (pb == 0) ? (tx == 0 ? 0 : 2) : (tx == 0 ? 1 : 2);
    for (int ky = y0; ky <= y1; ++ky)
      for (int kx = x0; kx <= x1; ++kx) v += wk[ky * 3 + kx];
  }
  return v;
}

__device__ __forceinline__ void pack_wino4_tile(const float* __restrict__ w, int cin, int cout, int nchunk,
                                                size_t j, bool flipT, float* __restrict__ dst) {
  constexpr double GD[6][3] = {{1.0, 0.0, 0.0},
                               {1.0 / 3, 1.0 / 3, 1.0 / 3},
                               {-1.0 / 3, 1.0 / 3, -1.0 / 3},
                               {-16.0 / 15, -8.0 / 15, -4.0 / 15},
                               {1.0 / 15, -2.0 / 15, 4.0 / 15},
                               {0.0, 0.0, 1.0}};
  const int c16 = (int)(j & 15);
  const int kk = (int)((j >> 4) & 3);
  const int cb = (int)((j >> 6) & 3);
  const size_t rest = j >> 8;
  const int k = (int)(rest % nchunk);
  const int cog = (int)(rest / nchunk);
  const int co = cog * 64 + cb * 16 + c16;
  const int ci = k * WINO4_KC + kk;
  const float* g = flipT ? w + ((size_t)ci * cout + co) * 9 : w + ((size_t)co * cin + ci) * 9;
  double gv[9];
#pragma unroll
  for (int q = 0; q < 9; ++q) gv[q] = (double)(flipT ? g[8 - q] : g[q]);
  double row[6][3];
#pragma unroll
  for (int rj = 0; rj < 6; ++rj)
#pragma unroll
    for (int y = 0; y < 3; ++y) {
      double r = 0.0;
#pragma unroll
      for (int x = 0; x < 3; ++x) r += gv[y * 3 + x] * GD[rj][x];
      row[rj][y] = r;
    }
  float2* o = reinterpret_cast<float2*>(dst) + ((((size_t)(cog * nchunk + k) * 18) * 4 + cb) * 4 + kk) * 16 + c16;
#pragma unroll
  for (int pp = 0; pp < 18; ++pp) {
    float uv[2];
#pragma unroll
    for (int e = 0; e < 2; ++e) {
      const int xi = 2 * pp + e, ri = xi / 6, rj = xi % 6;
      double u = 0.0;
#pragma unroll
      for (int y = 0; y < 3; ++y) u += GD[ri][y] * row[rj][y];
      uv[e] = (float)u;
    }
    o[(size_t)pp * 256] = make_float2(uv[0], uv[1]);
  }
}

__device__ __forceinline__ void pack_wino_tile(const float* __restrict__ w, int cin, int cout, int nchunk,
                                               size_t j, bool flipT, float* __restrict__ dst) {
  const double G[4][3] = {{1, 0, 0}, {0.5, 0.5, 0.5}, {0.5, -0.5, 0.5}, {0, 0, 1}};
  const int st = (int)(j & 1);
  const int c16 = (int)((j >> 1) & 15);
  const int kk = (int)((j >> 5) & 3);
  const int cb = (int)((j >> 7) & 3);
  const size_t rest = j >> 9;
  const int k = (int)(rest % nchunk);
  const int cog = (int)(rest / nchunk);
  const int co = cog * 64 + cb * 16 + c16;
  const int ci = k * WINO_KC + 2 * kk + st;
  const float* g = flipT ? w + ((size_t)ci * cout + co) * 9 : w + ((size_t)co * cin + ci) * 9;
  double gv[9];
#pragma unroll
  for (int q = 0; q < 9; ++q) gv[q] = (double)(flipT ? g[8 - q] : g[q]);
  double row[4][3];
#pragma unroll
  for (int rj = 0; rj < 4; ++rj)
#pragma unroll
    for (int y = 0; y < 3; ++y) {
      double r = 0.0;
#pragma unroll
      for (int x = 0; x < 3; ++x) r += gv[y * 3 + x] * G[rj][x];
      row[rj][y] = r;
    }
  float* o = dst + (((size_t)(cog * nchunk + k) * 16 * 4 + cb) * 4 + kk) * 32 + c16 * 2 + st;
#pragma unroll
  for (int xi = 0; xi < 16; ++xi) {
    const int ri = xi >> 2, rj = xi & 3;
    double u = 0.0;
#pragma unroll
    for (int y = 0; y < 3; ++y) u += G[ri][y] * row[rj][y];
    o[(size_t)xi * 512] = (float)u;
  }
}

__host__ __device__ inline long long pack_work_items(int kind, long long total) {
  return kind == 3 ? total / 36 : (kind == 2 ? total / 16 : total);
}

}
}
```

ert-conditional-diffusion-model_amd/csrc/unet_pack.hip:

```cpp
#include "unet_pack.h"

namespace ertd {
namespace unet {

namespace {

__global__ __launch_bounds__(256) void pack_batch_kernel(const ertd_pack_desc* __restrict__ d, int n) {
  const int b = blockIdx.x;
  int lo = 0, hi = n - 1;
  while (lo < hi) {
    const int mid = (lo + hi + 1) >> 1;
    if (d[mid].block0 <= b) lo = mid;
    else hi = mid - 1;
  }
  const ertd_pack_desc q = d[lo];
  const size_t i = (size_t)(b - q.block0) * 256 + threadIdx.x;
  if (i >= (size_t)pack_work_items(q.kind, q.total)) return;
  switch (q.kind) {
    case ERTD_PACK_DIRECT: q.dst[i] = pack_conv_elem(q.w, q.cin, q.cout, q.ks, q.nchunk, i, q.flip != 0); break;
    case ERTD_PACK_UP: q.dst[i] = pack_conv_up_elem(q.w, q.cin, q.cout, q.nchunk, (size_t)q.total / 4, i); break;
    case ERTD_PACK_WINO: pack_wino_tile(q.w, q.cin, q.cout, q.nchunk, i, q.flip != 0, q.dst); break;
    default: pack_wino4_tile(q.w, q.cin, q.cout, q.nchunk, i, q.flip != 0, q.dst); break;
  }
}

}

hipError_t launch_pack_batch(const ertd_pack_desc* d, int n, int blocks, hipStream_t s) {
  pack_batch_kernel<<<(unsigned)blocks, 256, 0, s>>>(d, n);
  return hipGetLastError();
}

}
}
```

ert-conditional-diffusion-model_amd/ertdiff/unet.py:

```python
from __future__ import annotations

import collections
import contextlib
import ctypes
import math
from typing import Dict, List, Optional, Sequence, Tuple, Union

import torch
import torch.nn as nn

from . import _lib
from .schedule import step_tables, timestep_frequencies


class ErtdUnetConfig(ctypes.Structure):
    _fields_ = [("image", ctypes.c_int), ("ch", ctypes.c_int), ("n_levels", ctypes.c_int),
                ("ch_mult", ctypes.c_int * 4), ("num_res", ctypes.c_int), ("attn", ctypes.c_int),
                ("groups", ctypes.c_int), ("precision", ctypes.c_int)]


CONFIGS: Dict[str, dict] = {
    "U1": dict(image=32, ch=32, ch_mult=(1, 2), num_res=2, attn=False),
    "U2": dict(image=64, ch=64, ch_mult=(1, 2, 4), num_res=2, attn=False),
    "U3": dict(image=64, ch=64, ch_mult=(1, 2, 4), num_res=2, attn=True),
    "U5": dict(image=128, ch=128, ch_mult=(1, 1, 2, 2), num_res=2, attn=True),
}


_PRECISIONS = {"fp32": 0, "bf16": 1, "bf16x3": 2}
_PRECISION_NAMES = {v: k for k, v in _PRECISIONS.items()}


def make_config(image=64, ch=64, ch_mult: Sequence[int] = (1, 2, 4), num_res=2, attn=False,
                groups=32, precision: str = "fp32") -> ErtdUnetConfig:
    m = list(ch_mult) + [0] * (4 - len(ch_mult))
    return ErtdUnetConfig(int(image), int(ch), len(ch_mult), (ctypes.c_int * 4)(*m), int(num_res),
                          int(bool(attn)), int(groups), _PRECISIONS[precision])


def param_layout(cfg: ErtdUnetConfig) -> List[Tuple[str, Tuple[int, ...]]]:
    lib = _lib.lib()
    n = lib.ertd_unet_n_params(ctypes.byref(cfg))
    if n < 0:
        raise RuntimeError("ertdiff: unsupported U-Net configuration")
    out = []
    name = ctypes.create_string_buffer(128)
    shape = (ctypes.c_int64 * 4)()
    nd = ctypes.c_int()
    for i in range(n):
        _lib.check(lib.ertd_unet_param_info(ctypes.byref(cfg), i, name, 128, shape,
                                            ctypes.byref(nd)), "unet_param_info")
        out.append((name.value.decode(), tuple(int(shape[j]) for j in range(nd.value))))
    return out


def unet_flops(image=64, ch=64, ch_mult: Sequence[int] = (1, 2, 4), num_res=2, attn=False,
               groups=32, batch: Optional[int] = None, cus: int = 256) -> Dict[str, int]:
    cfg = make_config(image, ch, ch_mult, num_res, attn, groups)
    layout = param_layout(cfg)
    conv = dense = ups = ups4 = wino = wino4 = 0
    res_of = {}
    r = image
    nl = len(ch_mult)
    for i in range(nl):
        res_of[f"down.{i}"] = r
        if i != nl - 1:
            r //= 2
    res_of["mid"] = r
    for i in reversed(range(nl)):
        res_of[f"up.{i}"] = image >> i

    def f4_items_fill(hw, cout):
        return batch is not None and (hw // 4) ** 2 // 16 * batch * (cout // 64) >= cus

    for name, shape in layout:
        if not name.endswith(".weight") or name.startswith("condition_encoder"):
            continue
        parts = name.split(".")
        if len(shape) == 4:
            if parts[0] in ("conv_in", "conv_out"):
                hw = image
            elif parts[0] == "mid":
                hw = res_of["mid"]
            else:
                hw = res_of[f"{parts[0]}.{parts[1]}"]
                if parts[2] == "downsample":
                    hw //= 2
                elif parts[2] == "upsample":
                    hw *= 2
            f = 2 * shape[0] * shape[1] * shape[2] * shape[3] * hw * hw
            conv += f
            if len(parts) > 2 and parts[2] == "upsample":
                if shape[1] % 8 == 0 and shape[0] % 64 == 0 and hw in (32, 64) or \
                        (hw == 16 and shape[1] % 8 == 0 and shape[0] % 64 == 0 and f4_items_fill(hw, shape[0])):
                    ups4 += f
                else:
                    ups += f
            if parts[-2] in ("conv1", "conv2") and shape[2] == 3 and shape[0] % 64 == 0:
                if (hw >= 32 and shape[1] % 4 == 0) or (hw == 16 and shape[1] % 8 == 0 and
                                                        f4_items_fill(hw, shape[0])):
                    wino4 += f
                elif shape[1] % 8 == 0:
                    wino += f
        elif len(shape) == 2:
            dense += 2 * shape[0] * shape[1]
    attn_f = 0
    if attn:
        C = ch * ch_mult[-1]
        N = res_of["mid"] ** 2
        attn_f = 2 * 2 * N * N * C
    enc = 6_308_736 + 14_426_112 + 2 * 64 * 128
    return {"conv": conv, "attention": attn_f, "dense": dense, "condition_encoder": enc,
            "total": conv + attn_f + dense + enc,
            "conv_winograd": wino + wino4 + ups4,
            "conv_winograd_f4": wino4 + ups4,
            "conv_executed_fp32": conv - ups * 5 // 9 - wino * 5 // 9 - (wino4 + ups4) * 3 // 4}


class ConditionalUNet(nn.Module):

    def __init__(self, image=64, ch=64, ch_mult: Sequence[int] = (1, 2, 4), num_res=2, attn=False,
                 groups=32, seed: Optional[int] = None, precision: str = "fp32"):
        super().__init__()
        self.spec = dict(image=image, ch=ch, ch_mult=tuple(ch_mult), num_res=num_res, attn=attn,
                         groups=groups)
        self.cfg = make_config(image, ch, ch_mult, num_res, attn, groups, precision)
        self.image = image
        self.param_dim = image * image
        self.layout = param_layout(self.cfg)
        g = torch.Generator().manual_seed(seed) if seed is not None else None
        shapes = dict(self.layout)
        for name, shape in self.layout:
            parts = name.split(".")
            mod = self
            for p in parts[:-1]:
                if not hasattr(mod, p) or not isinstance(getattr(mod, p), nn.Module):
                    mod.add_module(p, nn.Module())
                mod = getattr(mod, p)
            if ".norm" in name or name.startswith("norm_out"):
                val = torch.ones(shape) if parts[-1] == "weight" else torch.zeros(shape)
            else:
                wshape = shape if parts[-1] == "weight" else shapes[name[:-4] + "weight"]
                fan_in = int(math.prod(wshape[1:]))
                bound = 1.0 / math.sqrt(fan_in)
                val = (torch.rand(shape, generator=g) * 2 - 1) * bound
            mod.register_parameter(parts[-1], nn.Parameter(val))
        keys = list(self.state_dict().keys())
        if keys != [n for n, _ in self.layout]:
            raise RuntimeError("ertdiff: U-Net state_dict order differs from the library's")
        self._packed: Optional[torch.Tensor] = None
        self._packed_key = None
        self._ws: Dict = {}

    @classmethod
    def from_config(cls, name: str, seed: Optional[int] = None,
                    precision: str = "fp32") -> "ConditionalUNet":
        return cls(**CONFIGS[name], seed=seed, precision=precision)

    @property
    def precision(self) -> str:
        return _PRECISION_NAMES[self.cfg.precision]

    def set_precision(self, precision: str) -> None:
        self.cfg.precision = _PRECISIONS[precision]
        self._packed = None
        self._packed_key = None
        self._ws = {}

    def _params(self) -> List[torch.Tensor]:
        sd = dict(self.named_parameters())
        return [sd[n] for n, _ in self.layout]

    def packed_weights(self, dev: torch.device) -> torch.Tensor:
        ps = self._params()
        key = tuple((p.data_ptr(), p._version) for p in ps)
        if self._packed is None or self._packed_key != key or self._packed.device != dev:
            for (n, _), p in zip(self.layout, ps):
                if p.dtype != torch.float32 or not p.is_contiguous() or p.device != dev:
                    raise RuntimeError(f"ertdiff: parameter {n} must be contiguous float32 on {dev}")
            lib = _lib.lib()
            nf = lib.ertd_unet_packed_floats(ctypes.byref(self.cfg))
            if self._packed is None or self._packed.device != dev:
                self._packed = torch.empty(nf, dtype=torch.float32, device=dev)
            arr = (ctypes.c_void_p * len(ps))(*[p.data_ptr() for p in ps])
            freq = timestep_frequencies(self.spec["ch"], dev)
            with torch.cuda.device(dev):
                _lib.check(lib.ertd_unet_pack(ctypes.byref(self.cfg), arr, freq.data_ptr(),
                                              self._packed.data_ptr(), _lib.stream_of(dev)),
                           "unet_pack")
            self._packed_key = key
        return self._packed

    def workspace(self, dev: torch.device, B: int, L: int) -> torch.Tensor:
        n = _lib.lib().ertd_unet_workspace_bytes(ctypes.byref(self.cfg), B, L)
        if n == 0:
            raise RuntimeError("ertdiff: unsupported U-Net configuration")
        ws = self._ws.get(dev)
        if ws is None or ws.numel() < n:
            self._ws.pop(dev, None)
            ws = torch.empty(n, dtype=torch.uint8, device=dev)
            self._ws[dev] = ws
        return ws

    def forward(self, x: torch.Tensor, t: torch.Tensor, condition: torch.Tensor,
                return_cond_emb: bool = False):
        if (torch.is_grad_enabled() and not return_cond_emb and
                (x.requires_grad or any(p.requires_grad for p in self.parameters()))):
            if self.precision != "fp32":
                raise RuntimeError(
                    "ertdiff: the bf16-operand U-Net has no backward; call it under torch.no_grad() "
                    "for inference (sample_model does) or model.set_precision('fp32') to train")
            from .unet_train import UNetForwardFn
            dev = _lib.require_device(x, t, condition, self.conv_in.weight)
            self._check_call(x, t, condition)
            return UNetForwardFn.apply(self, _lib.f32c(x, "x"), t.to(device=dev, dtype=torch.int64)
                                       .contiguous(), _lib.f32c(condition, "condition"),
                                       *self._params())
        return self._infer(x, t, condition, return_cond_emb)

    def _check_call(self, x, t, cond):
        B = x.shape[0]
        if x.dim() != 2 or x.shape[1] != self.param_dim:
            raise RuntimeError(f"ertdiff: x must be (B, {self.param_dim}), got {tuple(x.shape)}")
        if cond.dim() != 3 or cond.shape[0] != B or cond.shape[1] != _lib.CIN:
            raise RuntimeError(f"ertdiff: condition must be (B, 14, L), got {tuple(cond.shape)}")
        if t.shape != (B,):
            raise RuntimeError(f"ertdiff: t must be (B,), got {tuple(t.shape)}")

    @torch.no_grad()
    def _infer(self, x: torch.Tensor, t: torch.Tensor, condition: torch.Tensor,
               return_cond_emb: bool = False):
        dev = _lib.require_device(x, t, condition, self.conv_in.weight)
        x = _lib.f32c(x, "x")
        cond = _lib.f32c(condition, "condition")
        B = x.shape[0]
        if x.dim() != 2 or x.shape[1] != self.param_dim:
            raise RuntimeError(f"ertdiff: x must be (B, {self.param_dim}), got {tuple(x.shape)}")
        if cond.dim() != 3 or cond.shape[0] != B or cond.shape[1] != _lib.CIN:
            raise RuntimeError(f"ertdiff: condition must be (B, 14, L), got {tuple(cond.shape)}")
        tt = t.to(torch.int64).contiguous()
        if tt.shape != (B,):
            raise RuntimeError(f"ertdiff: t must be (B,), got {tuple(t.shape)}")
        L = cond.shape[2]
        out = torch.empty(B, self.param_dim, dtype=torch.float32, device=dev)
        cemb = torch.empty(B, _lib.HIDDEN, dtype=torch.float32, device=dev) if return_cond_emb else None
        packed = self.packed_weights(dev)
        ws = self.workspace(dev, B, L)
        with torch.cuda.device(dev):
            _lib.check(_lib.lib().ertd_unet_forward(
                ctypes.byref(self.cfg), packed.data_ptr(), x.data_ptr(), tt.data_ptr(),
                cond.data_ptr(), _lib.CIN * L, L, B, out.data_ptr(), _lib.ptr(cemb), ws.data_ptr(),
                ws.numel(), _lib.stream_of(dev)), "unet_forward")
        return (out, cemb) if return_cond_emb else out


class _UPrepared:
    def __init__(self, model: ConditionalUNet, condition, T, betas, alphas, alpha_bar, num_steps,
                 temperature, shared_condition):
        dev = _lib.require_device(condition, model.conv_in.weight)
        self.dev = dev
        cond = _lib.f32c(condition, "condition")
        if cond.dim() == 2:
            cond = cond.unsqueeze(0)
        if cond.dim() != 3 or cond.shape[1] != _lib.CIN:
            raise RuntimeError(f"ertdiff: condition must be (B, 14, L), got {tuple(condition.shape)}")
        self.cond = cond
        self.L = cond.shape[2]
        self.stride = 0 if shared_condition else _lib.CIN * self.L
        self.num_steps = T if num_steps is None else int(num_steps)
        if not 1 <= self.num_steps <= T:
            raise RuntimeError(f"ertdiff: num_steps={self.num_steps} must be in [1, T={T}]")
        self.tables = step_tables(betas, alphas, alpha_bar, self.num_steps, temperature).to(dev)
        self.model = model
        self.packed = model.packed_weights(dev)

    def args(self, B, x, noise, seed, member_offset, t_first, n_run, ws):
        tb = self.tables
        return (ctypes.byref(self.model.cfg), self.packed.data_ptr(), self.cond.data_ptr(),
                self.stride, self.L, B, self.num_steps, t_first, n_run, tb[0].data_ptr(),
                tb[1].data_ptr(), tb[2].data_ptr(), _lib.ptr(noise), int(seed) & (2**64 - 1),
                int(member_offset) & 0xFFFFFFFF, x.data_ptr(), ws.data_ptr(), ws.numel())


@torch.no_grad()
def sample_unet(model: ConditionalUNet, condition, T, betas, alphas, alpha_bar, param_dim, device,
                num_steps=None, temperature=1.0, *, noise: Union[str, torch.Tensor] = "torch",
                seed: int = 0, member_offset: int = 0, shared_condition: bool = False,
                n_members: Optional[int] = None, precision: Optional[str] = None,
                mode: Optional[str] = None):
    from .sampler import draw_reference_noise, philox_normal
    if precision is not None and precision != model.precision:
        raise RuntimeError(f"ertdiff: precision={precision!r} but the U-Net runs {model.precision!r}; "
                           "call model.set_precision() first")
    if mode is not None:
        raise RuntimeError(f"ertdiff: mode={mode!r} applies to ConditionalDiffusionModel only")
    if model.param_dim != param_dim:
        raise RuntimeError(f"ertdiff: param_dim={param_dim} but the U-Net predicts {model.param_dim}")
    prep = _UPrepared(model, condition, T, betas, alphas, alpha_bar, num_steps, temperature,
                      shared_condition)
    n = prep.num_steps
    dev = prep.dev
    B = n_members if shared_condition else prep.cond.shape[0]
    inj = None
    if isinstance(noise, torch.Tensor):
        inj = _lib.f32c(noise, "noise")
        if inj.dim() != 3 or inj.shape[0] != n or inj.shape[2] != param_dim:
            raise RuntimeError(f"ertdiff: noise must be (num_steps={n}, B, {param_dim})")
        B = inj.shape[1]
        x = inj[0].clone()
    elif noise == "torch":
        if B is None:
            raise RuntimeError("ertdiff: shared_condition needs n_members")
        inj = draw_reference_noise(B, param_dim, n, device).to(dev)
        x = inj[0].clone()
    elif noise == "philox":
        x = philox_normal(B, param_dim, n, 1, seed, member_offset, dev)
    else:
        raise ValueError("noise must be 'torch', 'philox' or a tensor")
    if not shared_condition and prep.cond.shape[0] != B:
        raise RuntimeError(f"ertdiff: condition batch {prep.cond.shape[0]} != noise batch {B}")
    ws = model.workspace(dev, B, prep.L)
    with torch.cuda.device(dev):
        _lib.check(_lib.lib().ertd_unet_sample(*prep.args(B, x, inj, seed, member_offset, n - 1, n,
                                                          ws), _lib.stream_of(dev)), "unet_sample")
    return x


class UNetSamplerPlan:

    def __init__(self, model: ConditionalUNet, condition, T, betas, alphas, alpha_bar, *,
                 num_steps=None, t_first=None, n_run=None, temperature=1.0, seed=0,
                 member_offset=0, B=None, shared_condition=False,
                 noise: Optional[torch.Tensor] = None):
        self.prep = _UPrepared(model, condition, T, betas, alphas, alpha_bar, num_steps,
                               temperature, shared_condition)
        n = self.prep.num_steps
        dev = self.prep.dev
        self.dev = dev
        self.t_first = n - 1 if t_first is None else int(t_first)
        self.n_run = self.t_first + 1 if n_run is None else int(n_run)
        self.B = B if B is not None else self.prep.cond.shape[0]
        self.noise = None if noise is None else _lib.f32c(noise, "noise")
        self.x = torch.zeros(self.B, model.param_dim, dtype=torch.float32, device=dev)
        nbytes = _lib.lib().ertd_unet_workspace_bytes(ctypes.byref(model.cfg), self.B, self.prep.L)
        if nbytes == 0:
            raise RuntimeError("ertdiff: unsupported U-Net configuration")
        self.ws = torch.empty(nbytes, dtype=torch.uint8, device=dev)
        self._plan = ctypes.c_void_p()
        with torch.cuda.device(dev):
            _lib.check(_lib.lib().ertd_unet_sample_plan_create(
                *self.prep.args(self.B, self.x, self.noise, seed, member_offset, self.t_first,
                                self.n_run, self.ws), ctypes.byref(self._plan)),
                "unet_sample_plan_create")

    def launch(self, stream: Optional[torch.cuda.Stream] = None, n_steps: Optional[int] = None):
        s = (stream or torch.cuda.current_stream(self.dev)).cuda_stream
        with torch.cuda.device(self.dev):
            if n_steps is None:
                _lib.check(_lib.lib().ertd_unet_plan_launch(self._plan, s), "unet_plan_launch")
            else:
                _lib.check(_lib.lib().ertd_unet_plan_launch_steps(self._plan, int(n_steps), s),
                           "unet_plan_launch_steps")

    def close(self):
        if self._plan:
            _lib.lib().ertd_unet_plan_destroy(self._plan)
            self._plan = ctypes.c_void_p()

    def __del__(self):
        try:
            self.close()
        except Exception:
            pass


_MODES2D = {"same": 0, "down": 1, "up": 2}
_ACTS = {"none": 0, "gn_silu": 1, "gn": 2}


def conv2d(x: torch.Tensor, weight: torch.Tensor, bias: torch.Tensor, *, mode: str = "same",
           act: str = "none", gn: Optional[torch.Tensor] = None, x2: Optional[torch.Tensor] = None,
           ebias: Optional[torch.Tensor] = None, res: Optional[torch.Tensor] = None,
           precision: str = "fp32", out: Optional[torch.Tensor] = None) -> torch.Tensor:
    dev = _lib.require_device(x, weight, bias)
    x = _lib.f32c(x, "x")
    B, Ca, H, _ = x.shape
    Cb = 0 if x2 is None else x2.shape[1]
    Cout, Cin, ks, _ = weight.shape
    if Cin != Ca + Cb:
        raise RuntimeError("ertdiff: weight in-channels != input channels")
    Ho = H // 2 if mode == "down" else (2 * H if mode == "up" else H)
    if out is None:
        out = torch.empty(B, Cout, Ho, Ho, dtype=torch.float32, device=dev)
    elif (tuple(out.shape) != (B, Cout, Ho, Ho) or out.dtype != torch.float32 or out.device != dev
          or not out.is_contiguous()):
        raise RuntimeError("ertdiff: out must be a contiguous float32 (B, Cout, Ho, Ho) tensor on the device")
    prec = _PRECISIONS[precision]
    n = _lib.lib().ertd_conv2d_workspace_bytes(Cin, Cout, ks, prec, B, H, _MODES2D[mode])
    if n == 0:
        raise RuntimeError("ertdiff: unsupported conv2d geometry")
    ws = torch.empty(n, dtype=torch.uint8, device=dev)
    w = _lib.f32c(weight, "weight")
    bb = _lib.f32c(bias, "bias")
    eb = None if ebias is None else _lib.f32c(ebias, "ebias")
    with torch.cuda.device(dev):
        _lib.check(_lib.lib().ertd_conv2d(
            x.data_ptr(), Ca, _lib.ptr(None if x2 is None else _lib.f32c(x2, "x2")), Cb, B, H,
            w.data_ptr(), bb.data_ptr(), Cout, ks, _MODES2D[mode],
            _lib.ptr(None if gn is None else _lib.f32c(gn, "gn")), _ACTS[act], _lib.ptr(eb),
            0 if eb is None else eb.shape[1], _lib.ptr(None if res is None else _lib.f32c(res, "res")),
            out.data_ptr(), prec, ws.data_ptr(), ws.numel(), _lib.stream_of(dev)), "conv2d")
    return out


ConvRoute = collections.namedtuple("ConvRoute", "kernel ksplit items grid gn_parts")


def conv2d_route(Ca: int, Cb: int, Cout: int, ks: int, B: int, H: int, *, mode: str = "same",
                 act: str = "none", precision: str = "fp32", ebias: bool = False, res: bool = False,
# ... 54 lines not shown
```

Before: 261.5.

## Use upsample-specific Winograd F4 points to skip dead transform products

Adds a Cook-Toom point set (0, 1, 0.5, -0.5, -1) for the fused nearest-upsample F(4,3) Winograd kernel. Because the upsampled window repeats samples, one transform row and column is always zero, so the XS=2 upsample path skips those MFMA products, loads and transforms. It adds matching weight-pack matrices and specialised input and output transforms. This trades more code and template specialisation, with some numerical-conditioning risk from the new points, for fewer FLOPs in upsample convolutions.

```diff
diff --git a/ert-conditional-diffusion-model_amd/csrc/unet.h b/ert-conditional-diffusion-model_amd/csrc/unet.h
--- a/ert-conditional-diffusion-model_amd/csrc/unet.h
+++ b/ert-conditional-diffusion-model_amd/csrc/unet.h
@@ -85,6 +85,7 @@
   bool fold_ok = false;
   int fold_target = 0;
   int pack_kind = ERTD_PACK_DIRECT;
+  bool up_points = false;
 };
 WinoRoute wino_route(int mode, int act, int Cin, int Ca, int Cout, int Wo, int B, bool have_f2_pack,
                      bool have_f4_pack, int cus);
@@ -302,7 +303,7 @@
 size_t conv_packed_floats_wino(int cin, int cout);
 size_t conv_packed_floats_wino4(int cin, int cout);
 hipError_t launch_pack_conv_wino4(const float* w, int cin, int cout, float* dst, hipStream_t s,
-                                  bool flipT = false);
+                                  bool flipT = false, bool up = false);
 int wino4s_xs();
 hipError_t launch_add_inplace(float* out, const float* part, size_t n, hipStream_t s);
 hipError_t launch_pack_conv_wino(const float* w, int cin, int cout, float* dst, hipStream_t s,
diff --git a/ert-conditional-diffusion-model_amd/csrc/unet_capi.hip b/ert-conditional-diffusion-model_amd/csrc/unet_capi.hip
--- a/ert-conditional-diffusion-model_amd/csrc/unet_capi.hip
+++ b/ert-conditional-diffusion-model_amd/csrc/unet_capi.hip
@@ -953,7 +953,8 @@
   ConvArgs a = conv2d_args(x, Ca, x2, Cb, H, bias, Cout, ks, mode, gn, ebias, eb_stride, res, out, precision,
                            pk, need, route);
   if (wino && pack &&
-      (e = wino4 ? launch_pack_conv_wino4(w, Cin, Cout, const_cast<float*>(a.wpk_wino4), s)
+      (e = wino4 ? launch_pack_conv_wino4(w, Cin, Cout, const_cast<float*>(a.wpk_wino4), s, false,
+                                          route.up_points)
                  : launch_pack_conv_wino(w, Cin, Cout, const_cast<float*>(a.wpk_wino), s)) != hipSuccess)
     return (int)e;
   if (gnp) {
@@ -1103,9 +1104,12 @@
   return ERTD_OK;
 }
 
-void fill_desc(ertd_pack_desc* d, const float* w, float* dst, int cin, int cout, int ks, int kind, int flip) {
+void fill_desc(ertd_pack_desc* d, const float* w, float* dst, int cin, int cout, int ks, const WinoRoute& r,
+               int flip) {
+  const int kind = r.pack_kind;
   *d = ertd_pack_desc{};
   d->w = w; d->dst = dst; d->cin = cin; d->cout = cout; d->ks = ks; d->kind = kind; d->flip = flip;
+  d->reserved = r.up_points ? 1 : 0;
   switch (kind) {
     case ERTD_PACK_DIRECT:
       d->total = (long long)conv_packed_floats(cin, cout, ks);
@@ -1145,7 +1149,7 @@
                                    void* ws, ertd_pack_desc* out) {
   if (!w || !ws || !out || ertd_conv_input_grad_ws_bytes(Cin, Cout, B, H, ks, mode) == 0)
     return ERTD_EINVAL;
-  fill_desc(out, w, (float*)ws, Cout, Cin, ks, input_grad_route(Cin, Cout, B, H, ks, mode).pack_kind, 1);
+  fill_desc(out, w, (float*)ws, Cout, Cin, ks, input_grad_route(Cin, Cout, B, H, ks, mode), 1);
   return ERTD_OK;
 }
 
@@ -1158,7 +1162,7 @@
   const WinoRoute route = conv2d_route(Cin, Ca, Cout, ks, mode, ACT_NONE, precision, B, H);
   if (route.kernel != WinoRoute::NONE)
     pk += a64(std::max(conv_packed_floats(Cin, Cout, ks), conv_packed_floats_up(Cin, Cout)));
-  fill_desc(out, w, pk, Cin, Cout, ks, route.pack_kind, 0);
+  fill_desc(out, w, pk, Cin, Cout, ks, route, 0);
   return ERTD_OK;
 }
 
@@ -1320,7 +1324,8 @@
         e = launch_pack_conv_wino(src, p.shape[1], p.shape[0], packed + itw->second, s);
       const auto itw4 = L.offw4.find(p.name);
       if (e == hipSuccess && itw4 != L.offw4.end())
-        e = launch_pack_conv_wino4(src, p.shape[1], p.shape[0], packed + itw4->second, s);
+        e = launch_pack_conv_wino4(src, p.shape[1], p.shape[0], packed + itw4->second, s, false,
+                                   ends_with(p.name, ".upsample.weight"));
     } else if (p.shape.size() == 2) {
       e = launch_transpose(src, p.shape[0], p.shape[1], packed + L.off.at(p.name), p.shape[0], s);
     } else {
diff --git a/ert-conditional-diffusion-model_amd/csrc/unet_conv_wino.hip b/ert-conditional-diffusion-model_amd/csrc/unet_conv_wino.hip
--- a/ert-conditional-diffusion-model_amd/csrc/unet_conv_wino.hip
+++ b/ert-conditional-diffusion-model_amd/csrc/unet_conv_wino.hip
@@ -567,6 +567,7 @@
   r.fold_ok = s && !split;
   r.fold_target = s ? t4 / 16 * ncog : 0;
   r.pack_kind = f2 ? ERTD_PACK_WINO : ERTD_PACK_WINO4;
+  r.up_points = r.kernel == WinoRoute::F4S_UP;
   return r;
 }
 
diff --git a/ert-conditional-diffusion-model_amd/csrc/unet_conv_wino4.hip b/ert-conditional-diffusion-model_amd/csrc/unet_conv_wino4.hip
--- a/ert-conditional-diffusion-model_amd/csrc/unet_conv_wino4.hip
+++ b/ert-conditional-diffusion-model_amd/csrc/unet_conv_wino4.hip
@@ -39,6 +39,12 @@
                              {-16.0 / 15, -8.0 / 15, -4.0 / 15},
                              {1.0 / 15, -2.0 / 15, 4.0 / 15},
                              {0.0, 0.0, 1.0}};
+constexpr double GD_UP[6][3] = {{1.0, 0.0, 0.0},
+                                {2.0 / 3, 2.0 / 3, 2.0 / 3},
+                                {-8.0 / 3, -4.0 / 3, -2.0 / 3},
+                                {-8.0 / 3, 4.0 / 3, -2.0 / 3},
+                                {2.0 / 3, -2.0 / 3, 2.0 / 3},
+                                {0.0, 0.0, 1.0}};
 
 __device__ __forceinline__ f32x2 fmac(f32x2 x, float c, f32x2 s) {
   return __builtin_elementwise_fma(x, f32x2{c, c}, s);
@@ -518,9 +524,10 @@
 }
 
 __global__ void pack_wino4_kernel(const float* __restrict__ w, int cin, int cout, int nchunk,
-                                  size_t total, float* __restrict__ dst, bool flipT) {
+                                  size_t total, float* __restrict__ dst, bool flipT, bool up) {
   const size_t i = (size_t)blockIdx.x * blockDim.x + threadIdx.x;
   if (i >= total) return;
+  const double (&GD)[6][3] = up ? GD_UP : unet::GD;
   const int e = (int)(i & 1);
   const int c16 = (int)((i >> 1) & 15);
   const int kk = (int)((i >> 5) & 3);
@@ -612,11 +619,11 @@
 }
 
 hipError_t launch_pack_conv_wino4(const float* w, int cin, int cout, float* dst, hipStream_t s,
-                                  bool flipT) {
+                                  bool flipT, bool up) {
   const size_t total = conv_packed_floats_wino4(cin, cout);
   if (!total) return hipErrorInvalidValue;
   pack_wino4_kernel<<<(unsigned)((total + 255) / 256), 256, 0, s>>>(w, cin, cout, cin / WKC, total, dst,
-                                                                     flipT);
+                                                                     flipT, up);
   return hipGetLastError();
 }
 
diff --git a/ert-conditional-diffusion-model_amd/csrc/unet_conv_wino4s.hip b/ert-conditional-diffusion-model_amd/csrc/unet_conv_wino4s.hip
--- a/ert-conditional-diffusion-model_amd/csrc/unet_conv_wino4s.hip
+++ b/ert-conditional-diffusion-model_amd/csrc/unet_conv_wino4s.hip
@@ -76,6 +76,33 @@
   o[3] = pfma(e, 2.f, c);
   o[4] = pfma(e, -0.5f, c);
   o[5] = pfma(c, 1.5f, pfma(d[3], -2.f, d[1] + d[5]));
+}
+template <bool DEAD4>
+__device__ __forceinline__ void bt6u(const float (&d)[6], float (&o)[6]) {
+  const float c = d[4] - d[2], e = d[3] - d[1];
+  o[0] = __builtin_fmaf(4.f, d[4], __builtin_fmaf(-5.f, d[2], d[0]));
+  o[1] = __builtin_fmaf(-0.25f, d[1] + d[2], d[3] + d[4]);
+  o[2] = __builtin_fmaf(0.5f, e, c);
+  o[3] = __builtin_fmaf(-0.5f, e, c);
+  o[4] = DEAD4 ? 0.f : __builtin_fmaf(0.25f, d[1] - d[2], d[4] - d[3]);
+  o[5] = __builtin_fmaf(-1.25f, d[3], __builtin_fmaf(0.25f, d[1], d[5]));
+}
+template <bool DEAD4>
+__device__ __forceinline__ void bt6pu(const f32x2 (&d)[6], f32x2 (&o)[6]) {
+  const f32x2 c = d[4] - d[2], e = d[3] - d[1];
+  o[0] = pfma(d[4], 4.f, pfma(d[2], -5.f, d[0]));
+  o[1] = pfma(d[1] + d[2], -0.25f, d[3] + d[4]);
+  o[2] = pfma(e, 0.5f, c);
+  o[3] = pfma(e, -0.5f, c);
+  o[4] = DEAD4 ? f32x2{0.f, 0.f} : pfma(d[1] - d[2], 0.25f, d[4] - d[3]);
+  o[5] = pfma(d[3], -1.25f, pfma(d[1], 0.25f, d[5]));
+}
+__device__ __forceinline__ void at6u(const f32x2 (&m)[6], f32x2 (&y)[4]) {
+  const f32x2 s = m[2] + m[3], d = m[2] - m[3];
+  y[0] = (m[0] + m[1]) + s;
+  y[1] = fmac(d, 0.5f, m[1]);
+  y[2] = fmac(s, 0.25f, m[1]);
+  y[3] = fmac(d, 0.125f, m[1] + m[5]);
 }
 template <int N, bool SHL>
 __device__ __forceinline__ f32x2 row_shift0(f32x2 v) {
@@ -152,6 +179,8 @@
 };
 __device__ __forceinline__ int itm_half(const ItemWalk& w, int il) { return w.at(il).half; }
 
+constexpr int up25_pair(int xh, int l) { return xh && l >= 3 ? l + 3 : l; }
+
 template <int WO, int ACT, bool UP, int XS, bool FOLD, bool GNC>
 __global__ __launch_bounds__(64 * (4 * XS + NPW)) void conv_wino4s_kernel(ConvArgs a, int nitems, int ksp, int cw) {
   static_assert(!GNC || (XS == 2 && !UP && ACT != ACT_NONE && !FOLD), "GNC: the xi-split GN+act kernel");
@@ -169,6 +198,7 @@
   constexpr int TS = TPR * TPR;
   constexpr int WS = UP ? WO / 2 : WO;
   constexpr int HWS = WS * WS;
+  constexpr bool UP25 = UP && XS == 2;
   static_assert(TS % 16 == 0 && TPR <= 16, "a 16-tile block is whole tile rows of one sample");
   const int tid = threadIdx.x;
   const int lane = tid & 63;
@@ -303,9 +333,16 @@
       }
       m[0] = m[0] * f32x2{pad[set].x, pad[set].x};
       m[5] = m[5] * f32x2{pad[set].y, pad[set].y};
-      bt6p(m, act2[ab]);
+      if constexpr (UP) bt6pu<UP25>(m, act2[ab]);
+      else bt6p(m, act2[ab]);
 #pragma unroll
       for (int i = 0; i < 6; ++i) {
+        if constexpr (UP25) {
+          if (i == 4) {
+            actn[ab][i] = 0.f;
+            continue;
+          }
+        }
         const float give = h ? act2[ab][i].y : act2[ab][i].x;
         const float nb = __int_as_float(__builtin_amdgcn_ds_bpermute(nbaddr, __float_as_int(give)));
         actn[ab][i] = nb * pad[set].z;
@@ -335,8 +372,13 @@
         cx[r] = m.x;
         cy[r] = m.y;
       }
-      bt6(cx, act[ab][0]);
-      bt6(cy, act[ab][1]);
+      if constexpr (UP) {
+        bt6u<UP25>(cx, act[ab][0]);
+        bt6u<UP25>(cy, act[ab][1]);
+      } else {
+        bt6(cx, act[ab][0]);
+        bt6(cy, act[ab][1]);
+      }
 #pragma unroll
       for (int i = 0; i < 6; ++i) {
         const float give = h ? act[ab][1][i] : act[ab][0][i];
@@ -375,7 +417,11 @@
 #pragma unroll
       for (int aa = 0; aa < 3; ++aa) {
         float vv[6];
-        bt6(row[aa], vv);
+        if constexpr (UP) bt6u<UP25>(row[aa], vv);
+        else bt6(row[aa], vv);
+        if constexpr (UP25) {
+          if (aa == 1 && h) continue;
+        }
 #pragma unroll
         for (int jp = 0; jp < 6; jp += 2)
           *reinterpret_cast<f32x2*>(o + (aa * 3 + jp / 2) * 128) = f32x2{vv[jp], vv[jp + 1]};
@@ -566,14 +612,16 @@
         f32x2 m[6];
 #pragma unroll
         for (int j = 0; j < 6; ++j) m[j] = f32x2{acc[6 * i + j][2 * pp], acc[6 * i + j][2 * pp + 1]};
-        at6(m, P[i]);
+        if constexpr (UP) at6u(m, P[i]);
+        else at6(m, P[i]);
       }
 #pragma unroll
       for (int x = 0; x < 4; ++x) {
         f32x2 col[6], yc[4];
 #pragma unroll
         for (int i = 0; i < 6; ++i) col[i] = P[i][x];
-        at6(col, yc);
+        if constexpr (UP) at6u(col, yc);
+        else at6(col, yc);
 #pragma unroll
         for (int r = 0; r < 4; ++r) {
           y[2 * pp][r][x] = yc[r].x;
@@ -685,7 +733,12 @@
   };
   if (nloc > 0) {
 #pragma unroll
-    for (int p = 0; p < NP; ++p) u_load(ub[0], p);
+    for (int p = 0; p < NP; ++p) {
+      if constexpr (UP25) {
+        if (xh && p / 3 == 1) continue;
+      }
+      u_load(ub[0], p);
+    }
     u_advance();
   }
   if constexpr (GNC) {
@@ -731,12 +784,106 @@
       if (p == NP - 1) u_advance();
     }
   };
+  auto chunk2u = [&](auto xhc, const float* vs) {
+    constexpr int XH = decltype(xhc)::value;
+    constexpr int NL = XH ? NP - 3 : NP;
+    constexpr int PD = WINO4S_PD;
+    f32x2 rb[PD + 1];
+#pragma unroll
+    for (int q = 0; q < PD; ++q) rb[q] = *reinterpret_cast<const f32x2*>(vs + (XH * NP + up25_pair(XH, q)) * 128);
+#pragma unroll
+    for (int q = 0; q < 2 * NL; ++q) {
+      const int st = q / NL, p = up25_pair(XH, q % NL);
+      const int qn = q + PD;
+      if (qn < 2 * NL)
+        rb[qn % (PD + 1)] =
+            *reinterpret_cast<const f32x2*>(vs + (qn / NL) * VKS + (XH * NP + up25_pair(XH, qn % NL)) * 128);
+      const int r = q % (PD + 1);
+      const f32x2 u = st == 0 ? ub[0][p] : ub[1][p];
+      const bool both = p % 3 != 2;
+      if (both) acc[2 * p] = __builtin_amdgcn_mfma_f32_16x16x4f32(u.x, rb[r].x, acc[2 * p], 0, 0, 0);
+      acc[2 * p + 1] = __builtin_amdgcn_mfma_f32_16x16x4f32(u.y, rb[r].y, acc[2 * p + 1], 0, 0, 0);
+      if (st == 0) u_load(ub[1], p);
+      else u_load(ub[0], p);
+      if (qn < 2 * NL) __builtin_amdgcn_sched_group_barrier(0x100, 1, 0);
+      if (both) __builtin_amdgcn_sched_group_barrier(0x008, 2, 0);
+      else __builtin_amdgcn_sched_group_barrier(0x008, 1, 0);
+      __builtin_amdgcn_sched_group_barrier(0x020, 1, 0);
+      if (q % NL == NL - 1) u_advance();
+    }
+  };
   for (int il = 0; il < nloc; ++il) {
 #pragma unroll
     for (int x = 0; x < 2 * NP; ++x) acc[x] = f32x4{};
     f32x2 own[4][4];
+    auto tail_u = [&](auto xhc) {
+      constexpr int XH = decltype(xhc)::value;
+#pragma unroll
+      for (int pp = 0; pp < 2; ++pp) {
+        if (pp) __builtin_amdgcn_sched_barrier(0);
+        f32x2 P[3][4], Y[4][4];
+#pragma unroll
+        for (int i = 0; i < 3; ++i) {
+          if (XH && i == 1) continue;
+          f32x2 m[6];
+#pragma unroll
+          for (int j = 0; j < 6; ++j)
+            if (j != 4) m[j] = f32x2{acc[6 * i + j][2 * pp], acc[6 * i + j][2 * pp + 1]};
+          m[4] = f32x2{0.f, 0.f};
+          at6u(m, P[i]);
+        }
+#pragma unroll
+        for (int x = 0; x < 4; ++x) {
+          if constexpr (XH == 0) {
+            Y[0][x] = P[0][x] + (P[1][x] + P[2][x]);
+            Y[1][x] = fmac(P[2][x], 0.5f, P[1][x]);
+            Y[2][x] = fmac(P[2][x], 0.25f, P[1][x]);
+            Y[3][x] = fmac(P[2][x], 0.125f, P[1][x]);
+          } else {
+            Y[0][x] = P[0][x];
+            Y[1][x] = P[0][x] * f32x2{-0.5f, -0.5f};
+            Y[2][x] = P[0][x] * f32x2{0.25f, 0.25f};
+            Y[3][x] = fmac(P[0][x], -0.125f, P[2][x]);
+          }
+        }
+        if (pp == XH) {
+#pragma unroll
+          for (int r = 0; r < 4; ++r)
+#pragma unroll
+            for (int x = 0; x < 4; ++x) own[r][x] = Y[r][x];
+        } else {
+          float* xw = xbuf + ((cb * 2 + (XH ^ 1)) * 8) * 256 + lane * 4;
+#pragma unroll
+          for (int r = 0; r < 4; ++r)
+#pragma unroll
+            for (int x = 0; x < 4; x += 2)
+              *reinterpret_cast<f32x4*>(xw + (r * 2 + x / 2) * 256) =
+                  f32x4{Y[r][x].x, Y[r][x].y, Y[r][x + 1].x, Y[r][x + 1].y};
+        }
+      }
+    };
     if (il < 8) W4S_STAMP(3 + 3 * il);
     unsigned rpf[2] = {0u, 0u};
+    auto kloop_u = [&](auto xhc) {
+      for (int k = 0; k < nchunk; ++k) {
+        const int g = il * nchunk + k;
+        int ln;
+        asm volatile("v_mbcnt_lo_u32_b32 %0, -1, 0\n\tv_mbcnt_hi_u32_b32 %0, -1, %0" : "=v"(ln));
+        chunk2u(xhc, vbuf + (g & 1) * V_FL + ln * 2);
+#pragma unroll
+        for (int x = 0; x < 2 * NP; ++x)
+          if (x % 6 != 4) asm volatile("" : "+v"(acc[x]));
+        if (k == nchunk - 1) tail_u(xhc);
+        __syncthreads();
+#ifdef WINO4S_STAMP
+        if (g < 32) W4S_STAMP(28 + g);
+#endif
+      }
+    };
+    if constexpr (UP25) {
+      if (xh == 0) kloop_u(std::integral_constant<int, 0>{});
+      else kloop_u(std::integral_constant<int, 1>{});
+    } else {
     for (int k = 0; k < nchunk; ++k) {
       const int g = il * nchunk + k;
       int ln;
@@ -807,6 +954,7 @@
 #ifdef WINO4S_STAMP
       if (g < 32) W4S_STAMP(28 + g);
 #endif
+    }
     }
     if (il < 8) W4S_STAMP(4 + 3 * il);
     int ln;
diff --git a/ert-conditional-diffusion-model_amd/csrc/unet_pack.h b/ert-conditional-diffusion-model_amd/csrc/unet_pack.h
--- a/ert-conditional-diffusion-model_amd/csrc/unet_pack.h
+++ b/ert-conditional-diffusion-model_amd/csrc/unet_pack.h
@@ -61,13 +61,21 @@
 }
 
 __device__ __forceinline__ void pack_wino4_tile(const float* __restrict__ w, int cin, int cout, int nchunk,
-                                                size_t j, bool flipT, float* __restrict__ dst) {
-  constexpr double GD[6][3] = {{1.0, 0.0, 0.0},
-                               {1.0 / 3, 1.0 / 3, 1.0 / 3},
-                               {-1.0 / 3, 1.0 / 3, -1.0 / 3},
-                               {-16.0 / 15, -8.0 / 15, -4.0 / 15},
-                               {1.0 / 15, -2.0 / 15, 4.0 / 15},
-                               {0.0, 0.0, 1.0}};
+                                                size_t j, bool flipT, float* __restrict__ dst,
+                                                bool up = false) {
+  constexpr double GD_S1[6][3] = {{1.0, 0.0, 0.0},
+                                  {1.0 / 3, 1.0 / 3, 1.0 / 3},
+                                  {-1.0 / 3, 1.0 / 3, -1.0 / 3},
+                                  {-16.0 / 15, -8.0 / 15, -4.0 / 15},
+                                  {1.0 / 15, -2.0 / 15, 4.0 / 15},
+                                  {0.0, 0.0, 1.0}};
+  constexpr double GD_UP[6][3] = {{1.0, 0.0, 0.0},
+                                  {2.0 / 3, 2.0 / 3, 2.0 / 3},
+                                  {-8.0 / 3, -4.0 / 3, -2.0 / 3},
+                                  {-8.0 / 3, 4.0 / 3, -2.0 / 3},
+                                  {2.0 / 3, -2.0 / 3, 2.0 / 3},
+                                  {0.0, 0.0, 1.0}};
+  const double (&GD)[6][3] = up ? GD_UP : GD_S1;
   const int c16 = (int)(j & 15);
   const int kk = (int)((j >> 4) & 3);
   const int cb = (int)((j >> 6) & 3);
diff --git a/ert-conditional-diffusion-model_amd/csrc/unet_pack.hip b/ert-conditional-diffusion-model_amd/csrc/unet_pack.hip
--- a/ert-conditional-diffusion-model_amd/csrc/unet_pack.hip
+++ b/ert-conditional-diffusion-model_amd/csrc/unet_pack.hip
@@ -20,7 +20,7 @@
     case ERTD_PACK_DIRECT: q.dst[i] = pack_conv_elem(q.w, q.cin, q.cout, q.ks, q.nchunk, i, q.flip != 0); break;
     case ERTD_PACK_UP: q.dst[i] = pack_conv_up_elem(q.w, q.cin, q.cout, q.nchunk, (size_t)q.total / 4, i); break;
     case ERTD_PACK_WINO: pack_wino_tile(q.w, q.cin, q.cout, q.nchunk, i, q.flip != 0, q.dst); break;
-    default: pack_wino4_tile(q.w, q.cin, q.cout, q.nchunk, i, q.flip != 0, q.dst); break;
+    default: pack_wino4_tile(q.w, q.cin, q.cout, q.nchunk, i, q.flip != 0, q.dst, q.reserved == 1); break;
   }
 }
 
diff --git a/ert-conditional-diffusion-model_amd/ertdiff/unet.py b/ert-conditional-diffusion-model_amd/ertdiff/unet.py
--- a/ert-conditional-diffusion-model_amd/ertdiff/unet.py
+++ b/ert-conditional-diffusion-model_amd/ertdiff/unet.py
@@ -58,7 +58,7 @@
                groups=32, batch: Optional[int] = None, cus: int = 256) -> Dict[str, int]:
     cfg = make_config(image, ch, ch_mult, num_res, attn, groups)
     layout = param_layout(cfg)
-    conv = dense = ups = ups4 = wino = wino4 = 0
+    conv = dense = ups = ups4 = ups25 = wino = wino4 = 0
     res_of = {}
     r = image
     nl = len(ch_mult)
@@ -93,7 +93,10 @@
             if len(parts) > 2 and parts[2] == "upsample":
                 if shape[1] % 8 == 0 and shape[0] % 64 == 0 and hw in (32, 64) or \
                         (hw == 16 and shape[1] % 8 == 0 and shape[0] % 64 == 0 and f4_items_fill(hw, shape[0])):
-                    ups4 += f
+                    if shape[1] >= 16:
+                        ups25 += f
+                    else:
+                        ups4 += f
                 else:
                     ups += f
             if parts[-2] in ("conv1", "conv2") and shape[2] == 3 and shape[0] % 64 == 0:
@@ -112,9 +115,10 @@
     enc = 6_308_736 + 14_426_112 + 2 * 64 * 128
     return {"conv": conv, "attention": attn_f, "dense": dense, "condition_encoder": enc,
             "total": conv + attn_f + dense + enc,
-            "conv_winograd": wino + wino4 + ups4,
-            "conv_winograd_f4": wino4 + ups4,
-            "conv_executed_fp32": conv - ups * 5 // 9 - wino * 5 // 9 - (wino4 + ups4) * 3 // 4}
+            "conv_winograd": wino + wino4 + ups4 + ups25,
+            "conv_winograd_f4": wino4 + ups4 + ups25,
+            "conv_executed_fp32": conv - ups * 5 // 9 - wino * 5 // 9 - (wino4 + ups4) * 3 // 4
+                                  - ups25 * 119 // 144}
 
 
 class ConditionalUNet(nn.Module):
diff --git a/ert-conditional-diffusion-model_amd/ertdiff/wino_up.py b/ert-conditional-diffusion-model_amd/ertdiff/wino_up.py
--- /dev/null
+++ b/ert-conditional-diffusion-model_amd/ertdiff/wino_up.py
@@ -0,0 +1,104 @@
+from __future__ import annotations
+
+import numpy as np
+
+UP_POINTS = (0.0, 1.0, 0.5, -0.5, -1.0)
+UP_DEAD = 4
+PROJECT_POINTS = (0.0, 1.0, -1.0, 0.5, -2.0)
+
+
+def cook_toom(points, row0_scale=None):
+    a = np.asarray(points, dtype=np.float64)
+    n = len(a)
+    AT = np.zeros((4, n + 1))
+    G = np.zeros((n + 1, 3))
+    BT = np.zeros((n + 1, n + 1))
+    for i in range(n):
+        others = np.delete(a, i)
+        m = np.poly(others)[::-1]
+        N = np.prod(a[i] - others)
+        s = 1.0
+        if i == 0:
+            s = (1.0 / m[0]) if row0_scale is None else row0_scale
+        BT[i, :n] = m * s
+        G[i] = a[i] ** np.arange(3) / (N * s)
+        AT[:, i] = a[i] ** np.arange(4)
+    BT[n] = np.poly(a)[::-1]
+    G[n] = [0.0, 0.0, 1.0]
+    AT[3, n] = 1.0
+    return AT, G, BT
+
+
+BT_UP = np.array([[1, 0, -5, 0, 4, 0],
+                  [0, -.25, -.25, 1, 1, 0],
+                  [0, -.5, -1, .5, 1, 0],
+                  [0, .5, -1, -.5, 1, 0],
+                  [0, .25, -.25, -1, 1, 0],
+                  [0, .25, 0, -1.25, 0, 1]], dtype=np.float64)
+AT_UP = np.array([[1, 1, 1, 1, 1, 0],
+                  [0, 1, .5, -.5, -1, 0],
+                  [0, 1, .25, .25, 1, 0],
+                  [0, 1, .125, -.125, -1, 1]], dtype=np.float64)
+G_UP = np.array([[1, 0, 0],
+                 [2 / 3, 2 / 3, 2 / 3],
+                 [-8 / 3, -4 / 3, -2 / 3],
+                 [-8 / 3, 4 / 3, -2 / 3],
+                 [2 / 3, -2 / 3, 2 / 3],
+                 [0, 0, 1]], dtype=np.float64)
+
+_f = np.float32
+
+
+def _fma(a, b, c):
+    return (a.astype(np.float64) * np.float64(b) + c.astype(np.float64)).astype(_f) \
+        if np.isscalar(b) else (a.astype(np.float64) * b.astype(np.float64) + c.astype(np.float64)).astype(_f)
+
+
+def bt6u_f32(d):
+    d = [np.asarray(x, dtype=_f) for x in d]
+    c, e = d[4] - d[2], d[3] - d[1]
+    return [_fma(d[4], 4.0, _fma(d[2], -5.0, d[0])),
+            _fma(d[1] + d[2], -0.25, d[3] + d[4]),
+            _fma(e, 0.5, c),
+            _fma(e, -0.5, c),
+            _fma(d[1] - d[2], 0.25, d[4] - d[3]),
+            _fma(d[3], -1.25, _fma(d[1], 0.25, d[5]))]
+
+
+def at6u_f32(m, dead=True):
+    m = [np.asarray(x, dtype=_f) for x in m]
+    s, d = m[2] + m[3], m[2] - m[3]
+    y = [(m[0] + m[1]) + s, _fma(d, 0.5, m[1]), _fma(s, 0.25, m[1]), _fma(d, 0.125, m[1] + m[5])]
+    if not dead:
+        y = [y[0] + m[4], y[1] - m[4], y[2] + m[4], y[3] - m[4]]
+    return y
+
+
+def input_transform_f32(win):
+    rows = bt6u_f32([win[i] for i in range(6)])
+    V = [bt6u_f32([r[j] for j in range(6)]) for r in rows]
+    return V
+
+
+def conv_tile_f32(wins, U, live_only):
+    Cin = wins.shape[0]
+    M = np.zeros((6, 6), dtype=_f)
+    for c in range(Cin):
+        V = input_transform_f32(wins[c])
+        for i in range(6):
+            for j in range(6):
+                if live_only and (i == UP_DEAD or j == UP_DEAD):
+                    continue
+                M[i, j] = _fma(np.asarray(U[c, i, j], _f), np.asarray(V[i][j], _f), M[i, j])
+    P = [at6u_f32([M[i, j] for j in range(6)], dead=live_only) for i in range(6)]
+    Y = np.zeros((4, 4), dtype=_f)
+    for x in range(4):
+        col = at6u_f32([P[i][x] for i in range(6)], dead=live_only)
+        for r in range(4):
+            Y[r, x] = col[r]
+    return Y
+
+
+def up_window(src4):
+    m = [0, 1, 1, 2, 2, 3]
+    return np.asarray(src4)[..., m, :][..., :, m]
```

Result: faster. 267.5, median of 6 (+2.3%).
